# ComputationalRobotics/XM-code

Measured on AMD Instinct MI355X. Metric: BM iters/sec (tCG Hessian-vector iterations per second; ms_per_step = wall-clock-to-KKT of one staircase solve), higher is better.
Workload: dtype f64

## Files before the change

### include/xm_amd.h

```cpp
#ifndef XM_AMD_H
#define XM_AMD_H

#include <stddef.h>
#include <stdint.h>

#ifdef __cplusplus
extern "C" {
#endif

#define XM_OK              0
#define XM_ERR_IO         -1
#define XM_ERR_ARG        -2
#define XM_ERR_HIP        -3
#define XM_ERR_COMM       -4
#define XM_ERR_NOMEM      -5

#define XM_STATUS_NONE          0
#define XM_STATUS_CERTIFIED     1
#define XM_STATUS_MAX_RANK      2
#define XM_STATUS_LS_FAILED    -2

const char *xm_last_error(void);
const char *xm_version(void);
#define XM_ABI_REVISION 4
// ... 50 lines not shown
    uint32_t struct_size;
    int64_t n;
    int32_t storage;
    int32_t q_on_device;
    const double *q;
    int64_t ldq;
    int64_t nb;
    const int64_t *rowptr;
    const int32_t *colidx;
    const double *blocks;
    int64_t nobs, n_landmarks;
    const int32_t *obs_cam, *obs_lm;
    const double *obs_p, *obs_w;
    int64_t q_row0;
    int64_t ne;
    const int32_t *edge_i, *edge_j;
    const double *edge_w, *edge_M;
    int32_t n_gpus;
    int32_t gpu_map;
    const xm_tuning_t *tuning;
} xm_problem_t;

#define XM_MODE_SOLVE    0
#define XM_MODE_RANK3    1
#define XM_MODE_REBUTTLE 2

#define XM_FLAG_VERBOSE        1u
#define XM_FLAG_FIX_STALE_SR   2u
#define XM_FLAG_PROFILE_QW     4u
#define XM_FLAG_HOST_STEPPED   8u
#define XM_FLAG_MODEL_RECURRENCE 32u
#define XM_FLAG_HOST_OUTER    64u
#define XM_FLAG_DEVICE_OUTER 128u
#define XM_FLAG_WARM_R        16u

#define XM_RETRACT_QR    0
#define XM_RETRACT_POLAR 1

typedef struct {
    uint32_t struct_size;
    uint32_t max_rank;
    double tol, lam, max_time;
    int32_t mode;
    uint32_t flags;
    const double *s_ini;
    int32_t trace_cap;
    double *trace;
    const double *R_ini;
    int32_t retraction;
    int32_t sum_grouping;
} xm_options_t;

typedef struct {
    uint32_t struct_size;
    double *R;
    double *s;
    int32_t rank;
    int32_t status;
    double primal, dual, min_eig, gap;
    int64_t tcg_iters;
    int64_t outer_iters;
    int64_t qw_products;
    int64_t lanczos_iters;
    double seconds;
    double tr_seconds;
    double cert_seconds;
// ... 312 lines not shown
    int32_t irls_iterations;
    int32_t reserved;
    int64_t pcg_iterations;
    int64_t pcg_capped;
    int64_t pairs;
    int64_t registered;
    int64_t fixed_image;
    int64_t cams_heavy;
    int64_t max_incidences;
    double seconds_index;
    double seconds_kernels;
    double seconds_download;
} xm_vgr_result_t;
int xm_view_graph_rotations(int64_t n, const uint8_t *registered , const double *rot0, int64_t npairs, const int32_t *pi,
                            const int32_t *pj, const double *Rrel, const uint8_t *valid_in , const xm_vgr_options_t *opt,
                            double *rot_out, double *angle_axis_out, double *residual, double *weight, double *step_trace,
                            xm_vgr_result_t *res);
typedef struct {
    uint32_t struct_size;
    uint32_t reserved;
    const double *angle_axis, *x, *weight_in;
    double *rot, *residual, *gauge, *weight, *rhs, *diagonal, *product, *angle_axis_out, *step;
} xm_vgr_probe_t;
int xm_view_graph_rotations_probe(int64_t n, const uint8_t *registered, const double *rot0, int64_t npairs, const int32_t *pi,
                                  const int32_t *pj, const double *Rrel, const uint8_t *valid_in, const xm_vgr_options_t *opt,
                                  xm_vgr_probe_t *probe);
int xm_view_graph_rotations_limits(int64_t out[4]);
int xm_ctx_recover_tp(xm_ctx_t *ctx, const double *rot, const double *scale, double *t, double *p);
int xm_ctx_dense_q(xm_ctx_t *ctx, double *q, int64_t ldq);
int xm_create_matrix(int64_t n, int64_t m, int64_t nobs, const int32_t *cam, const int32_t *lm, const double *p, const double *w, double *Q,
                     int64_t ldq, double *Abar );
int xm_schur_dense_limits(int64_t out[3]);
int xm_ctx_schur_info(xm_ctx_t *ctx, int *uses_cg, int64_t stats[3], double *last_relres);
int xm_ctx_schur_precond_info(xm_ctx_t *ctx, int *kind, int64_t *aggregates, int *block);

#define XM_BA_FIX_ROTATIONS 1u
#define XM_BA_NONMONOTONIC  2u
#define XM_BA_DENSE_SCHUR   16u
#define XM_BA_PRECOND_TWO_LEVEL 32u
#define XM_BA_PRECOND_BLOCKS    64u
#define XM_BA_AGG_CAMS          16
#define XM_BA_MAX_AGGREGATES    4096
#define XM_BA_DENSE_MAX_ROWS 32768
#define XM_BA_LOSS_TRIVIAL  0
#define XM_BA_LOSS_HUBER    1
#define XM_BA_LOSS_SOFT_L1  2
#define XM_BA_LOSS_CAUCHY   3
#define XM_BA_LOSS_ARCTAN   4
#define XM_BA_OPTIONS_SIZE_V1 64u
#define XM_BA_NO_CONVERGENCE       0
#define XM_BA_CONVERGED_FUNCTION   1
#define XM_BA_CONVERGED_GRADIENT   2
#define XM_BA_CONVERGED_PARAMETER  3
#define XM_BA_MAX_ITERATIONS       4
#define XM_BA_TIME_LIMIT           5
#define XM_BA_NO_PROGRESS          6
typedef struct {
    uint32_t struct_size;
    int32_t max_iters;
    double max_time, eta, function_tol, gradient_tol, parameter_tol;
    uint32_t flags;
    int32_t trace_cap;
    double *trace;
    int32_t loss;
    int32_t max_nonmonotonic;
    double loss_scale;
// ... 312 lines not shown
```

### xm-code_amd/csrc/xm_capi.hip

```cpp
#include <algorithm>
#include <cmath>
#include <cstddef>
#include <cstdlib>
#include <cstring>
#include <fstream>
#include <mutex>
#include <vector>

#include "xm_ba.h"
#include "xm_gp.h"
#include "xm_clean.h"
#include "xm_trackfilter.h"
#include "xm_prune.h"
#include "xm_lift.h"
#include "xm_tracks.h"
#include "xm_tracks_split.h"
#include "xm_viewgraph.h"
#include "xm_vgcalib.h"
#include "xm_rotavg.h"
#include "xm_pair.h"
#include "xm_schur.h"
#include "xm_sell.h"
#include "xm_symw.h"
#include "xm_solver.h"
// ... 273 lines not shown
    XM_TRY
    if (!Q || ldq < 3 * n) throw xm::Error(XM_ERR_ARG, "xm_create_matrix: null Q or ldq < 3n");
    if (n > xm::kSchurDenseQMaxCams) throw xm::Error(XM_ERR_ARG, "xm_create_matrix: more than " + std::to_string(xm::kSchurDenseQMaxCams) + " cameras");
    require_device();
    hipStream_t st = nullptr;
    XM_HIP_CHECK(hipStreamCreateWithFlags(&st, hipStreamNonBlocking));
    double *dq = nullptr;
    try {
        xm::SchurSettings sc;
        sc.solver = 1;
        xm::SchurOp op(n, m, nobs, cam, lm, p, w, st, nullptr, sc);
        if (op.names_a_pair_twice()) throw xm::Error(XM_ERR_ARG, "xm_create_matrix: the observation list names a (camera, landmark) pair twice");
        const int64_t ld = xm_dense_ld(n);
        XM_HIP_CHECK(hipMalloc((void **)&dq, (size_t)3 * n * (size_t)ld * sizeof(double)));
        XM_HIP_CHECK(hipMemsetAsync(dq, 0, (size_t)3 * n * (size_t)ld * sizeof(double), st));
        op.build_dense_q(dq, ld, Abar, st);
        XM_HIP_CHECK(hipMemcpy2DAsync(Q, (size_t)ldq * sizeof(double), dq, (size_t)ld * sizeof(double), (size_t)3 * n * sizeof(double), (size_t)3 * n,
                                      hipMemcpyDeviceToHost, st));
        XM_HIP_CHECK(hipStreamSynchronize(st));
    } catch (...) {
        if (dq) (void)hipFree(dq);
        (void)hipStreamDestroy(st);
        throw;
    }
    (void)hipFree(dq);
    (void)hipStreamDestroy(st);
    return XM_OK;
    XM_CATCH
}
int xm_schur_dense_limits(int64_t out[3]) {
    XM_TRY
    if (!out) throw xm::Error(XM_ERR_ARG, "xm_schur_dense_limits: null output");
    out[0] = xm::kSchurDenseQWinCams; out[1] = xm::kSchurAbarPanel; out[2] = xm::kSchurDenseQMaxCams;
    return XM_OK;
    XM_CATCH
}
int xm_ctx_schur_info(xm_ctx_t *ctx, int *uses_cg, int64_t stats[3], double *last_relres) {
    XM_TRY
    if (!ctx || !ctx->impl || !uses_cg) throw xm::Error(XM_ERR_ARG, "xm_ctx_schur_info: single-GPU context and a non-null output needed");
    int64_t st[3] = {0, 0, 0};
    double rr = 0.0;
    *uses_cg = ctx->impl->schur_info(st, &rr) ? 1 : 0;
    if (stats) { stats[0] = st[0]; stats[1] = st[1]; stats[2] = st[2]; }
    if (last_relres) *last_relres = rr;
    return XM_OK;
    XM_CATCH
}
int xm_ctx_schur_precond_info(xm_ctx_t *ctx, int *kind, int64_t *aggregates, int *block) {
    XM_TRY
    if (!ctx || !ctx->impl || !kind) throw xm::Error(XM_ERR_ARG, "xm_ctx_schur_precond_info: single-GPU context and a non-null output needed");
    int64_t na = 0;
    int b = 0;
    *kind = ctx->impl->schur_precond(&na, &b);
    if (aggregates) *aggregates = na;
    if (block) *block = b;
    return XM_OK;
    XM_CATCH
}
int xm_ctx_bundle_adjust(xm_ctx_t *ctx, const xm_ba_options_t *opt, double *rot, double *t, double *p, xm_ba_result_t *res) {
    XM_TRY
    if (!ctx || !opt || !res || !rot || !t || !p) throw xm::Error(XM_ERR_ARG, "xm_ctx_bundle_adjust: null argument");
    static_assert(offsetof(xm_ba_options_t, loss) == XM_BA_OPTIONS_SIZE_V1, "the first version of xm_ba_options_t ends at trace");
    if (opt->struct_size != sizeof(xm_ba_options_t) && opt->struct_size != XM_BA_OPTIONS_SIZE_V1)
        throw xm::Error(XM_ERR_ARG, "xm_ctx_bundle_adjust: xm_ba_options_t.struct_size is neither sizeof(xm_ba_options_t) nor XM_BA_OPTIONS_SIZE_V1");
    if (res->struct_size != sizeof(xm_ba_result_t)) throw xm::Error(XM_ERR_ARG, "xm_ctx_bundle_adjust: xm_ba_result_t.struct_size is not sizeof(xm_ba_result_t)");
    if (ctx->team || !ctx->impl) throw xm::Error(XM_ERR_ARG, "xm_ctx_bundle_adjust: single-GPU contexts only (not n_gpus > 1)");
// ... 1611 lines not shown
```

### xm-code_amd/csrc/xm_common.h

```cpp
#pragma once

#include <hip/hip_runtime.h>

#include <algorithm>
#include <cstdint>
#include <cstdio>
#include <stdexcept>
#include <string>
#include <vector>

namespace xm {

struct Error : std::runtime_error {
    int code;
    Error(int c, const std::string &m) : std::runtime_error(m), code(c) {}
};

#define XM_HIP_CHECK(expr)                                                                            \
    do {                                                                                              \
        hipError_t _e = (expr);                                                                       \
        if (_e != hipSuccess)                                                                         \
            throw ::xm::Error(-3, std::string("HIP error: ") + hipGetErrorString(_e) + " at " +       \
                                      __FILE__ + ":" + std::to_string(__LINE__) + " (" #expr ")");    \
    } while (0)
// ... 147 lines not shown
    const OuterScal *os_cur;
    OuterScal *os_next;
    const double *parts;
    double *partsB_out;
    int nA, nB;
    const double *HpR, *Hps;
    double *R, *s;
    double *Rc, *sc;
    double *pR;
    const double *ps_cur;
    double *ps_next;
    double *vR, *vs, *HvR, *Hvs, *rR;
    const double *rs_cur;
    double *rs_next;
    double *Wloc, *Wpad;
    PointPtrs cur, cand;
    const double *partsA;
    double *partsM;
    int nM;
    double delta_bar, gradtol;
    int max_outer;
    double *trace;
    int trace_cap;
    const int *stop_req;
    unsigned long long *hprog;
    unsigned int run;
    int slot, grp;
};
void launch_outer_step(int o, int polar, const OuterStepArgs &A, int grid, hipStream_t st);

struct TcgParity {
    TcgScal *scal_cur, *scal_next;
    double *ps_cur, *ps_next, *rs_cur, *rs_next;
    size_t chunk, b_off;
    double *pcur;
    double *parts;
    double *Bout;
    double *partsB_out;
};

struct TcgInitArgs {
    int nloc;
    const double *rgR, *rgs, *R, *s;
    double *rR, *rs, *pR, *ps, *vR, *vs, *HvR, *Hvs;
    double *Wloc, *Wpad;
    TcgScal *scal0;
    double rr, delta;
    unsigned long long *hstat;
    int seq;
    const SpecCtl *spec;
};
struct CgStepArgs {
    int nloc;
    TcgParity v;
    int nA, nB, world;
    const double *HpR, *Hps, *R, *s;
    double *pR, *vR, *vs, *HvR, *Hvs, *rR;
    double *Wloc, *Wpad;
    unsigned long long *hstat;
    int64_t mat;
    double *Afull, *Wfull;
    int grouping;
    PeerXchg xchg;
};

void launch_qw_dense(int o, int epi, const double *Q, int64_t ld, const double *W, double alpha, const CamArgs &a,
                     hipStream_t st);
void launch_qw_bsr3(int o, int epi, const int64_t *rowptr, const int32_t *colidx, const double *blocks, const double *W,
                    double alpha, const CamArgs &a, hipStream_t st, int64_t nb = 0, const int4 *rowinfo = nullptr);
int64_t sell_resident_bytes(int64_t stream, int64_t other);
void bsr_build_rowinfo(const int64_t *rowptr_host, int nloc, std::vector<int4> &out);
int qw_grid(int nloc);
void launch_qw_dense_split(int o, int epi, const double *Q, int64_t ld, const double *W, double alpha, const CamArgs &a, hipStream_t st);
int qw_dense_tile_cols();
int qw_dense_split_k(int nloc, int64_t ld);
int bsr_grid(int nloc);
void qw_bench_nt(int nt);
void symv_bench_k(int k, int kf);
int symv_trace_slots();
struct SymvPlan { int K, Kf, ysplit, nchunks, gx, gy; };
void symv_plan_get(int nloc, int64_t ld, int out[4]);
struct SymvWork {
    int nloc = 0, o = 0;
    int64_t ld = 0;
    SymvPlan plan{};
    DevBuf<double> prow, pcol;
    void ensure(int nloc, int64_t ld, int o);
    void release();
    explicit operator bool() const { return pcol.p != nullptr; }
};
void launch_qw_sym_traced(int o, const double *Q, int64_t ld, const double *W, const CamArgs &a, SymvWork &work, unsigned long long *trace, hipStream_t st);
void launch_qw_sym(int o, int epi, const double *Q, int64_t ld, const double *W, double alpha, const CamArgs &a, SymvWork &work, hipStream_t st,
                   int rev = 0);
void launch_asym(const double *Q, int64_t ld, int64_t m, double *out, int grid, hipStream_t st);
void launch_dense_to_f32(const double *src, float *dst, int64_t rows, int64_t ld, unsigned int *bad, hipStream_t st);
void launch_qw_dense_f32(int o, int epi, const float *Qf, const double *Qd, int64_t ld, const double *W, double alpha, const CamArgs &a, hipStream_t st);
void launch_qw_sym_f32(int o, int epi, const float *Qf, const double *Qd, int64_t ld, const double *W, double alpha, const CamArgs &a, SymvWork &work,
                       hipStream_t st, int rev = 0);

void launch_symhash(const double *Q, int64_t ld, int64_t row0, int64_t nrows, int64_t m, unsigned long long *out, int grid, hipStream_t st);

void launch_transpose_pad(const double *src_colmajor, int64_t lds, int64_t rows, int64_t cols, double *dst, int64_t ldd,
                          hipStream_t st);
void launch_dense_from_bsr(const int64_t *rowptr, const int32_t *colidx, const double *blocks, int64_t nloc, int64_t cam0,
                           double *dst, int64_t ldd, hipStream_t st);

int flat_grid(int64_t elems);
void launch_scale_rows(int o, int nloc, const double *R, const double *s, double *Wloc, hipStream_t st);
void launch_tcg_init(int o, const TcgInitArgs &a, hipStream_t st);
void launch_cg_step(int o, const CgStepArgs &a, hipStream_t st);
struct OuterArgs { double loss, delta, delta_bar, gradtol; int shrink_count, last_iter; };
void launch_outer_finalize(const double *partsA, int nA_loc, int world, const double *partsM, int nM, const TcgScal *scal, double *hres,
                           unsigned long long seq, int grouping, hipStream_t st, const OuterArgs *oa = nullptr, SpecCtl *spec_out = nullptr);
void launch_retract(int o, int nloc, int cam0, const double *R, const double *s, const double *D, const double *ds, double t,
                    double *Rout, double *sout, double *Wloc, hipStream_t st, int polar = 0);
int retract_grid(int nloc);
void launch_retract_model(int o, int nloc, int cam0, const double *R, const double *s, const double *vR, const double *vs, double *Rout, double *sout,
                          double *Wloc, double *Wpad, const double *HvR, const double *Hvs, const double *rgR, const double *rgs, double *parts,
                          hipStream_t st, int polar);
void launch_cert_prepare(int o, int nloc, int cam0, double lam, const double *QsR, const double *R, const double *s,
                         double *Lam, double *dz, double *parts, hipStream_t st);
void launch_recover_gram(int64_t n, int r, const double *R, const double *s, double *parts, int grid, hipStream_t st);
void launch_recover_project(int64_t n, int r, const double *R, const double *s, const double *V, double *rot, double *scale, int *negcount,
                            hipStream_t st, int variant = 0);
void launch_negate(double *x, int64_t len, hipStream_t st);
int dots_multi_segments(int64_t len);
// ... 47 lines not shown
```

### xm-code_amd/csrc/xm_device.h

```cpp
#pragma once

#include "xm_common.h"

namespace xm {

template <int CTRL, int ROW_MASK>
__device__ __forceinline__ double dpp_mov(double v) {
    int lo = __double2loint(v), hi = __double2hiint(v);
    lo = __builtin_amdgcn_update_dpp(0, lo, CTRL, ROW_MASK, 0xf, false);
    hi = __builtin_amdgcn_update_dpp(0, hi, CTRL, ROW_MASK, 0xf, false);
    return __hiloint2double(hi, lo);
}
__device__ __forceinline__ double wave_sum(double v) {
    v += dpp_mov<0xb1, 0xf>(v);
    v += dpp_mov<0x4e, 0xf>(v);
    v += dpp_mov<0x124, 0xf>(v);
    v += dpp_mov<0x128, 0xf>(v);
    v += dpp_mov<0x142, 0xa>(v);
    v += dpp_mov<0x143, 0xc>(v);
    const int lo = __builtin_amdgcn_readlane(__double2loint(v), 63), hi = __builtin_amdgcn_readlane(__double2hiint(v), 63);
    return __hiloint2double(hi, lo);
}

template <int GW>
// ... 30 lines not shown
    __syncthreads();
    return (sh[0] + sh[1]) + (sh[2] + sh[3]);
}

__device__ __forceinline__ int sum_perm(int i, int count, int grp) {
    if (grp == 1) return count - 1 - i;
    if (grp == 2) { const int h = (count + 1) >> 1; return (i < h) ? 2 * i : 2 * (i - h) + 1; }
    return i;
}
__device__ __forceinline__ double sum_partials256(const double *p, int count, double *sh, int grp = 0) {
    double v = 0.0;
    for (int i = threadIdx.x; i < count; i += 256) v += p[sum_perm(i, count, grp)];
    return block_sum256(v, sh);
}

__device__ __forceinline__ void sum_partials256_x4(const double *p0, const double *p1, const double *p2, int count, const double *p3,
                                                   int count3, double *sh16, double (&out)[4], int grp = 0) {
    double v[4] = {0.0, 0.0, 0.0, 0.0};
    for (int i = threadIdx.x; i < count; i += 256) { const int j = sum_perm(i, count, grp); v[0] += p0[j]; v[1] += p1[j]; v[2] += p2[j]; }
    for (int i = threadIdx.x; i < count3; i += 256) v[3] += p3[sum_perm(i, count3, grp)];
#pragma unroll
    for (int k = 0; k < 4; ++k) v[k] = wave_sum(v[k]);
    __syncthreads();
    if ((threadIdx.x & 63) == 0) {
#pragma unroll
        for (int k = 0; k < 4; ++k) sh16[k * 4 + (threadIdx.x >> 6)] = v[k];
    }
    __syncthreads();
#pragma unroll
    for (int k = 0; k < 4; ++k) out[k] = (sh16[k * 4] + sh16[k * 4 + 1]) + (sh16[k * 4 + 2] + sh16[k * 4 + 3]);
}

constexpr int kPre = 4;
struct PartialsPre { double v[4][kPre]; };
__device__ __forceinline__ void sum_partials_prefetch(const double *p0, const double *p1, const double *p2, int count, const double *p3, int count3,
                                                      PartialsPre &pre, int grp) {
#pragma unroll
    for (int r = 0; r < kPre; ++r) {
        const int i = threadIdx.x + 256 * r;
        const int j = (i < count) ? sum_perm(i, count, grp) : 0, j3 = (i < count3) ? sum_perm(i, count3, grp) : 0;
        pre.v[0][r] = (i < count) ? p0[j] : 0.0; pre.v[1][r] = (i < count) ? p1[j] : 0.0; pre.v[2][r] = (i < count) ? p2[j] : 0.0;
        pre.v[3][r] = (i < count3) ? p3[j3] : 0.0;
    }
}
__device__ __forceinline__ void sum_partials256_x4_pre(const double *p0, const double *p1, const double *p2, int count, const double *p3,
                                                       int count3, bool use3, const PartialsPre &pre, double *sh16, double (&out)[4], int grp = 0) {
    double v[4] = {0.0, 0.0, 0.0, 0.0};
#pragma unroll
    for (int r = 0; r < kPre; ++r) {
        const int i = threadIdx.x + 256 * r;
        if (i < count) { v[0] += pre.v[0][r]; v[1] += pre.v[1][r]; v[2] += pre.v[2][r]; }
        if (use3 && i < count3) v[3] += pre.v[3][r];
    }
    for (int i = threadIdx.x + 256 * kPre; i < count; i += 256) { const int j = sum_perm(i, count, grp); v[0] += p0[j]; v[1] += p1[j]; v[2] += p2[j]; }
    if (use3)
        for (int i = threadIdx.x + 256 * kPre; i < count3; i += 256) v[3] += p3[sum_perm(i, count3, grp)];
#pragma unroll
    for (int k = 0; k < 4; ++k) v[k] = wave_sum(v[k]);
    __syncthreads();
    if ((threadIdx.x & 63) == 0) {
#pragma unroll
        for (int k = 0; k < 4; ++k) sh16[k * 4 + (threadIdx.x >> 6)] = v[k];
    }
    __syncthreads();
#pragma unroll
    for (int k = 0; k < 4; ++k) out[k] = (sh16[k * 4] + sh16[k * 4 + 1]) + (sh16[k * 4 + 2] + sh16[k * 4 + 3]);
}

#pragma clang fp contract(off)
struct Col3 {
    double v[3];
};
template <int O>
__device__ __forceinline__ Col3 load_col(const double *base, int cam, int lane) {
    constexpr int OP = pitch_of(O);
    Col3 c;
    const double *p = base + (size_t)cam * 3 * OP + lane;
#pragma unroll
    for (int a = 0; a < 3; ++a) c.v[a] = (lane < O) ? p[a * OP] : 0.0;
    return c;
}
template <int O>
__device__ __forceinline__ void store_col(const Col3 &c, double *base, int cam, int lane) {
    constexpr int OP = pitch_of(O);
    double *p = base + (size_t)cam * 3 * OP + lane;
    if (lane < O) {
#pragma unroll
        for (int a = 0; a < 3; ++a) p[a * OP] = c.v[a];
    }
// ... 198 lines not shown
```

### xm-code_amd/csrc/xm_kernels.hip

```cpp
#include <algorithm>
#include <cmath>
#include <cstdlib>
#include <cstring>
#include <type_traits>

#include "xm_common.h"
#include "xm_device.h"
#include "xm_symv_step.h"

namespace xm {

__device__ __forceinline__ double2 nt_load16(const double2 *p) {
    typedef double d2v __attribute__((ext_vector_type(2)));
    const d2v v = __builtin_nontemporal_load(reinterpret_cast<const d2v *>(p));
    return make_double2(v.x, v.y);
}

template <int O, int EPI, int NSUB, bool SPLIT = false>
__global__ __launch_bounds__(256) void qw_dense_kernel(const double *__restrict__ Q, int64_t ld,
                                                        const double *__restrict__ W, double alpha, CamArgs a) {
    constexpr int OP = pitch_of(O);
    int role = EPI;
    constexpr int TILE = NSUB * 128;
    constexpr int TILE2 = TILE * OP / 2;
// ... 229 lines not shown
            const double t = wave_sum(acc[r][k]);
            if (lane == k) h.v[r] = t;
        }
    if (active && lane < O) {
        double *ps = a.ksum + ((size_t)y * a.nloc + cam) * 3 * OP + lane;
#pragma unroll
        for (int r = 0; r < 3; ++r) __hip_atomic_store(ps + r * OP, h.v[r], __ATOMIC_RELAXED, __HIP_MEMORY_SCOPE_AGENT);
    }
    asm volatile("s_waitcnt vmcnt(0)" ::: "memory");
    __syncthreads();
    if (threadIdx.x == 0) {
        const unsigned int old = __hip_atomic_fetch_add(a.kcount + blockIdx.x, 1u, __ATOMIC_RELAXED, __HIP_MEMORY_SCOPE_AGENT);
        s_last = (old + 1 == (unsigned int)KS);
        if (s_last) __hip_atomic_store(a.kcount + blockIdx.x, 0u, __ATOMIC_RELAXED, __HIP_MEMORY_SCOPE_AGENT);
    }
    __syncthreads();
    if (!s_last) return;
    EpiOps eops;
    epi_prefetch<O, EPI>(eops, cam, lane, active, a);
    h.v[0] = h.v[1] = h.v[2] = 0.0;
    if (active && lane < O) {
        for (int s = 0; s < KS; ++s) {
            const double *ps = a.ksum + ((size_t)s * a.nloc + cam) * 3 * OP + lane;
#pragma unroll
            for (int r = 0; r < 3; ++r) h.v[r] += __hip_atomic_load(ps + r * OP, __ATOMIC_RELAXED, __HIP_MEMORY_SCOPE_AGENT);
        }
#pragma unroll
        for (int r = 0; r < 3; ++r) h.v[r] *= alpha;
    }
    qw_tail<O, EPI, 64, kQwWaves>(cam, lane, wave, active, h, a, eops, red);
}

constexpr int kSvTraceSlots = 24;
template <int O, bool TRACE = false>
__global__ __launch_bounds__(256) void qw_symv_kernel(const double *__restrict__ Q, int64_t ld, const double *__restrict__ W, int nloc, int Kc, int Kf, int ysplit, int nt_step0,
                                                        const TcgScal *__restrict__ scal, double *__restrict__ Prow,
                                                        double *__restrict__ Pcol, unsigned long long *__restrict__ trace, int rev, int by_phase) {
    constexpr int OP = pitch_of(O), V = 6 * O;
    __shared__ __attribute__((aligned(16))) double lds[4][V * 64];
    const int lane = threadIdx.x & 63, wave = __builtin_amdgcn_readfirstlane(threadIdx.x >> 6);
    unsigned long long *tr = nullptr;
    if constexpr (TRACE) {
        tr = trace + ((size_t)(blockIdx.y * gridDim.x + blockIdx.x) * 4 + wave) * kSvTraceSlots;
        if (lane == 0) {
            unsigned int hw, xcc;
            asm volatile("s_getreg_b32 %0, hwreg(HW_REG_HW_ID)" : "=s"(hw));
            asm volatile("s_getreg_b32 %0, hwreg(HW_REG_XCC_ID)" : "=s"(xcc));
            tr[0] = wall_clock64();
            tr[kSvTraceSlots - 1] = ((unsigned long long)xcc << 32) | hw;
        }
    }
    const SymvChunk ch = symv_chunk(blockIdx.x, blockIdx.y, nloc, ld, Kc, Kf, ysplit, wave);
    if (ch.empty) return;
    const int nrows = 3 * nloc, jb = ch.jb, je = ch.je;
    const bool half1 = ch.c0 + 128 < ld;
    double *L = lds[wave];
    const int64_t cA = ch.c0 + 2 * lane, cB = half1 ? cA + 128 : cA;

    double wc[2][2][O], ca[2][2][O];
    struct Slot { double2 q[6][2]; double wl; } slot[2];

    int nrun = 0;
    auto run = [&](int j, auto sl) __attribute__((always_inline)) {
        const Slot &b = slot[decltype(sl)::value];
        const int64_t r0 = (int64_t)6 * j;
        auto qat = [&](int r, int h, int e) __attribute__((always_inline)) { return e ? b.q[r][h].y : b.q[r][h].x; };
        auto wrow = [&](int r, double (&wr)[O]) __attribute__((always_inline)) { symv_wrow_read<O>(b.wl, r, r0 + r < nrows, wr); };
        double *prow = Prow + ((size_t)ch.s * (size_t)ch.R + (size_t)r0) * O;
        double mr[2] = {1.0, 1.0}, mc[2] = {1.0, 1.0};
        if (j < ch.jfull) symv_step<O, false>(qat, mr, mc, wrow, wc, ca, L, lane, prow);
        else {
#pragma unroll
            for (int h = 0; h < 2; ++h) {
                mr[h] = (cA + 128 * h >= r0) ? 1.0 : 0.0;
                mc[h] = (cA + 128 * h >= r0 + 6) ? 1.0 : 0.0;
            }
            symv_step<O, true>(qat, mr, mc, wrow, wc, ca, L, lane, prow);
        }
        if constexpr (TRACE) {
            if (lane == 0 && 2 + nrun < kSvTraceSlots - 3) tr[2 + nrun] = wall_clock64();
            ++nrun;
        }
    };
    auto sweep = [&](auto ntag) __attribute__((always_inline)) -> bool {
        constexpr bool NT = decltype(ntag)::value;
        auto load = [&](int j, auto sl) __attribute__((always_inline)) {
            Slot &b = slot[decltype(sl)::value];
            b.wl = symv_wrow_request<O>(W, j, nrows, lane);
            const int64_t r0 = (int64_t)6 * j;
#pragma unroll
            for (int r = 0; r < 6; ++r) {
                const int64_t rr = (r0 + r < nrows) ? r0 + r : nrows - 1;
                const double *row = Q + (size_t)rr * (size_t)ld;
#pragma unroll
                for (int h = 0; h < 2; ++h) {
                    const double2 *qp = reinterpret_cast<const double2 *>(row + (h ? cB : cA));
                    if (NT) b.q[r][h] = nt_load16(qp);
                    else b.q[r][h] = *qp;
                }
            }
        };
        if (jb < je) load(symv_walk_at(jb, je, rev, 0), std::integral_constant<int, 0>{});
#pragma unroll
        for (int h = 0; h < 2; ++h)
#pragma unroll
            for (int e = 0; e < 2; ++e)
#pragma unroll
                for (int k = 0; k < O; ++k) {
                    const double t = W[(size_t)((h ? cB : cA) + e) * OP + k];
                    wc[h][e][k] = (h == 0 || half1) ? t : 0.0;
                    ca[h][e][k] = 0.0;
                }
        if (scal != nullptr) {
            if (by_phase ? (scal->phase >= PH_STOP) : (scal->status != 0)) return false;
        }
        if constexpr (TRACE) { if (lane == 0) tr[1] = wall_clock64(); }
        symv_walk(jb, je, rev, load, run);
        return true;
    };
    const bool alive = (jb >= nt_step0) ? sweep(std::true_type{}) : sweep(std::false_type{});
    if (!alive) return;
    if constexpr (TRACE) { if (lane == 0) tr[kSvTraceSlots - 3] = wall_clock64(); }

    symv_colsum<O>(ca, lds, wave, lane, wave == 0 || half1, Pcol + ((size_t)ch.sc * (size_t)ld + (size_t)(cA + 128 * wave)) * O);
    if constexpr (TRACE) { if (lane == 0) tr[kSvTraceSlots - 2] = wall_clock64(); }
}

template <int O, int EPI>
__global__ __launch_bounds__(256) void symv_reduce_kernel(const double *__restrict__ Prow, const double *__restrict__ Pcol, int64_t ld,
                                                           int nstrips, int Kc, int Kf, int ysplit, double alpha, CamArgs a) {
    int role = (EPI == EPI_AUTO) ? (int)EPI_HESS : EPI;
    constexpr int NE = 3 * O;
    static_assert(NE <= 16, "a record must fit a 16-lane group");
    __shared__ double red[kQwWaves][3];
    const int lane = threadIdx.x & 63, wave = __builtin_amdgcn_readfirstlane(threadIdx.x >> 6);
    const int cam = blockIdx.x * kQwWaves + wave;
    const bool active = cam < a.nloc;
    EpiOps eops;
    epi_prefetch<O, EPI == EPI_AUTO ? EPI_HESS : EPI>(eops, cam, lane, active, a);
    const int e = lane & 15, g = lane >> 4;
    const bool eok = e < NE;
    const int camc = active ? cam : 0;
    const int64_t R = (int64_t)6 * ((a.nloc + 1) >> 1);
    const int s_lo = (6 * (camc >> 1)) / kSvStrip;
    const int nrow = nstrips - s_lo;
    auto ncol_of = [&](int c) -> int {
        const int sc_ = c / kSvStrip, row = min(sc_, nstrips - 1 - sc_);
        const int K = (row >= ysplit) ? Kf : Kc;
        return (c >= 6) ? (c - 6) / (6 * K) + 1 : 0;
    };
    const int ncol_l = ncol_of(3 * camc + (eok ? e / O : 0));
    const int ncol = max(ncol_of(3 * camc), ncol_of(3 * camc + 2));
    const int nrec = nrow + ncol;
    const int tot = active ? nrec : 0, tot_l = active ? nrow + ncol_l : 0;
    const size_t eo = (size_t)camc * 3 * O + (eok ? e : 0);
    auto fetch = [&](int i) -> double {
        const int ic = min(i, nrec - 1);
        const double *p = (ic < nrow) ? Prow + (size_t)(s_lo + ic) * (size_t)R * O : Pcol + (size_t)(ic - nrow) * (size_t)ld * O;
// ... 338 lines not shown
template <int O>
__global__ __launch_bounds__(256) void tcg_init_kernel(int nloc, const double *__restrict__ rgR, const double *__restrict__ rgs,
                                                        const double *__restrict__ R, const double *__restrict__ s,
                                                        double *rR, double *rs, double *pR, double *ps, double *vR, double *vs,
                                                        double *HvR, double *Hvs, double *Wloc, TcgScal *scal0, double rr,
                                                        double delta, unsigned long long *hstat, double *Wpad, int seq, const SpecCtl *spec) {
    constexpr int OP = pitch_of(O);
    const int64_t total = (int64_t)nloc * 3 * OP;
    if (spec != nullptr) {
        if (!spec->go) {
            if (blockIdx.x == 0 && threadIdx.x == 0) { TcgScal sc = *scal0; sc.status = 9; sc.seq = seq; *scal0 = sc; }
            return;
        }
        rr = spec->rr; delta = spec->delta;
    }
    for (int64_t i = (int64_t)blockIdx.x * 256 + threadIdx.x; i < total; i += (int64_t)gridDim.x * 256) {
        const int cam = (int)(i / (3 * OP));
        const double g = rgR[i], gs = rgs[cam];
        rR[i] = g; pR[i] = -g; vR[i] = 0.0; HvR[i] = 0.0;
        const double wv = s[cam] * (-g) + (-gs) * R[i];
        if (Wloc) Wloc[i] = wv;
        if (Wpad) Wpad[(size_t)cam * 16 + (i - (int64_t)cam * (3 * OP))] = wv;
        if (i % (3 * OP) == 0) { rs[cam] = gs; ps[cam] = -gs; vs[cam] = 0.0; Hvs[cam] = 0.0; }
    }
    if (blockIdx.x == 0 && threadIdx.x == 0) {
        TcgScal sc = {};
        sc.rr = rr; sc.vv = 0.0; sc.vp = 0.0; sc.pp = rr; sc.delta = delta; sc.gradnorm = sqrt(rr); sc.last_step = 0.0; sc.model = 0.0;
        sc.status = 0; sc.iter = 0; sc.seq = seq;
        *scal0 = sc;
        publish_host(hstat, pack_stat(seq, 0, 0));
    }
}

template <int O>
__global__ __launch_bounds__(256) void cg_step_kernel(int nloc, const TcgScal *__restrict__ scal_cur, TcgScal *scal_next,
                                                       const double *__restrict__ parts, int nA_loc, int nB_loc, int world,
                                                       const double *__restrict__ HpR,
                                                       const double *__restrict__ Hps, const double *__restrict__ R,
                                                       const double *__restrict__ s, double *pR, const double *__restrict__ ps_cur,
                                                       double *ps_next, double *vR, double *vs, double *HvR, double *Hvs, double *rR,
                                                       const double *__restrict__ rs_cur, double *rs_next, double *Wloc,
                                                       double *partsB_out, unsigned long long *hstat, int b_off, int64_t mat,
                                                       double *Afull, double *Wfull, int grp, PeerXchg x, double *Wpad) {
    constexpr int OP = pitch_of(O);
    __shared__ double sh[4];
    __shared__ double sh16[16];
    __shared__ int sh_flag;
    const int64_t total = (int64_t)nloc * 3 * OP;
    const int64_t stride = (int64_t)gridDim.x * 256;
    int64_t i = (int64_t)blockIdx.x * 256 + threadIdx.x;
    const bool in0 = i < total;
    const int camf = (int)(i / (3 * OP));
    const bool own0 = in0 && (i % (3 * OP) == 0);
    double hp = 0, pv = 0, vv0 = 0, hv = 0, rv = 0, Rv = 0, hs = 0, psv = 0, rsv = 0, sv = 1, vsv = 0, hvs = 0;
    const bool keep_hv = HvR != nullptr;
    if (in0) { hp = HpR[i]; pv = pR[i]; vv0 = vR[i]; if (keep_hv) hv = HvR[i]; rv = rR[i]; Rv = R[i]; hs = Hps[camf]; psv = ps_cur[camf]; rsv = rs_cur[camf]; sv = s[camf]; }
    if (own0) { vsv = vs[camf]; if (keep_hv) hvs = Hvs[camf]; }
    const bool can_pre = x.world <= 1;
    PartialsPre pre;
    if (can_pre) sum_partials_prefetch(parts + b_off, parts + b_off + nA_loc, parts + b_off + 2 * nA_loc, nA_loc, parts + b_off + 3 * nA_loc, nB_loc, pre, grp);
    const TcgScal sc0 = *scal_cur;
    const bool lead = (blockIdx.x == 0 && threadIdx.x == 0);
    if (sc0.status != 0) {
        if (lead) *scal_next = sc0;
        return;
    }
    if (x.world > 1) {
        const int par = sc0.iter & 1;
        const size_t chunk_d = (size_t)b_off + 3 * (size_t)nA_loc + nB_loc;
        const size_t off = ((size_t)par * x.world + x.rank) * chunk_d;
        const unsigned long long epoch = x.epoch_base + (unsigned long long)sc0.iter + 1ull;
        const double *src = x.buf[x.rank] + off;
        if (x.lite) {
            for (int p = 0; p < x.world; ++p) {
                if (p == x.rank) continue;
                double *dst = x.buf[p] + off;
                for (size_t j = (size_t)blockIdx.x * 256 + threadIdx.x; j < chunk_d; j += (size_t)stride)
                    __hip_atomic_store(dst + j, src[j], __ATOMIC_RELAXED, __HIP_MEMORY_SCOPE_SYSTEM);
            }
            asm volatile("s_waitcnt vmcnt(0)" ::: "memory");
            __syncthreads();
            if (threadIdx.x == 0) {
                const unsigned long long t = __hip_atomic_fetch_add(x.ticket + par, 1ull, __ATOMIC_RELAXED, __HIP_MEMORY_SCOPE_AGENT);
                sh_flag = (t + 1 == gridDim.x);
                if (sh_flag) __hip_atomic_store(x.ticket + par, 0ull, __ATOMIC_RELAXED, __HIP_MEMORY_SCOPE_AGENT);
            }
            __syncthreads();
            if (sh_flag && !x.mute && threadIdx.x < x.world && (int)threadIdx.x != x.rank)
                __hip_atomic_store(x.flag[threadIdx.x] + par * kMaxPeers + x.rank, epoch, __ATOMIC_RELAXED, __HIP_MEMORY_SCOPE_SYSTEM);
        } else {
            for (int p = 0; p < x.world; ++p) {
                if (p == x.rank) continue;
                double *dst = x.buf[p] + off;
                for (size_t j = (size_t)blockIdx.x * 256 + threadIdx.x; j < chunk_d; j += (size_t)stride) dst[j] = src[j];
            }
            __threadfence_system();
            asm volatile("s_waitcnt vmcnt(0)" ::: "memory");
            __syncthreads();
            if (threadIdx.x == 0) {
                const unsigned long long t = __hip_atomic_fetch_add(x.ticket + par, 1ull, __ATOMIC_ACQ_REL, __HIP_MEMORY_SCOPE_AGENT);
                sh_flag = (t + 1 == gridDim.x);
                if (sh_flag) __hip_atomic_store(x.ticket + par, 0ull, __ATOMIC_RELAXED, __HIP_MEMORY_SCOPE_AGENT);
            }
            __syncthreads();
            if (sh_flag && !x.mute && threadIdx.x < x.world && (int)threadIdx.x != x.rank) {
                __threadfence_system();
                asm volatile("s_waitcnt vmcnt(0)" ::: "memory");
                __hip_atomic_store(x.flag[threadIdx.x] + par * kMaxPeers + x.rank, epoch, __ATOMIC_RELEASE, __HIP_MEMORY_SCOPE_SYSTEM);
            }
        }
        __syncthreads();
        if (threadIdx.x == 0) {
            int good = 1;
            const long long t0 = wall_clock64();
            const unsigned long long *f = x.flag[x.rank] + par * kMaxPeers;
            for (int p = 0; p < x.world && good; ++p) {
                if (p == x.rank) continue;
                while (__hip_atomic_load(f + p, __ATOMIC_RELAXED, __HIP_MEMORY_SCOPE_SYSTEM) < epoch) {
                    if (wall_clock64() - t0 > x.spin_ticks) { good = 0; break; }
                    __builtin_amdgcn_s_sleep(1);
                }
            }
            if (!good) __hip_atomic_store(x.err, epoch | (1ull << 63), __ATOMIC_RELAXED, __HIP_MEMORY_SCOPE_SYSTEM);
            sh_flag = good;
            __atomic_thread_fence(__ATOMIC_ACQUIRE);
        }
        __syncthreads();
        if (!sh_flag) {
            if (lead) {
                TcgScal nx = sc0; nx.status = 7;
                *scal_next = nx;
                publish_host(hstat, pack_stat(nx.seq, nx.iter, nx.status));
            }
            return;
        }
        __builtin_amdgcn_fence(__ATOMIC_ACQUIRE, "");
    }
    const int chunk = b_off + 3 * nA_loc + nB_loc;
    double pHp = 0.0, rHp = 0.0, HpHp = 0.0, rr_prev = 0.0;
    for (int r = 0; r < world; ++r) {
        const double *pa = parts + (size_t)r * chunk + b_off;
        double t[4];
        if (r == 0 && can_pre) sum_partials256_x4_pre(pa, pa + nA_loc, pa + 2 * nA_loc, nA_loc, pa + 3 * nA_loc, nB_loc, sc0.iter > 0, pre, sh16, t, grp);
        else sum_partials256_x4(pa, pa + nA_loc, pa + 2 * nA_loc, nA_loc, pa + 3 * nA_loc, (sc0.iter > 0) ? nB_loc : 0, sh16, t, grp);
        pHp += t[0]; rHp += t[1]; HpHp += t[2];
        if (sc0.iter > 0) rr_prev += t[3];
    }
    TcgScal sc = sc0;
    if (sc0.iter > 0) sc.rr = rr_prev;
    const StepDecision d = tcg_decide(sc, pHp);
    if (d.mode == 5) {
        if (lead) {
            TcgScal nx = sc; nx.status = 5; nx.last_step = 0.0;
            *scal_next = nx;
            publish_host(hstat, pack_stat(nx.seq, nx.iter, nx.status));
        }
        return;
    }
    const double step = d.step;
    const bool cg = (d.mode == 0);
    double rr_est = sc.rr + 2.0 * step * rHp + step * step * HpHp;
    if (rr_est < 0.0) rr_est = 0.0;
    const bool conv = cg && (sqrt(rr_est) < sc.gradnorm * fmin(sc.gradnorm, 0.1));
    const double beta = rr_est / sc.rr;
    const bool newdir = cg && !conv;
    double acc = 0.0;
    if (in0) {
        vR[i] = vv0 + step * pv;
        if (keep_hv) HvR[i] = hv + step * hp;
        if (cg) {
            const double rn = rv + step * hp;
            const double rsn = rsv + step * hs;
            rR[i] = rn;
            acc += rn * rn;
            if (newdir) {
                const double pn = beta * pv - rn;
                const double psn = beta * psv - rsn;
                pR[i] = pn;
                if (!Afull) {
                    const double wv = sv * pn + psn * Rv;
                    if (Wloc) Wloc[i] = wv;
                    if (Wpad) Wpad[(size_t)camf * 16 + (i - (int64_t)camf * (3 * OP))] = wv;
                }
                if (own0) ps_next[camf] = psn;
            }
            if (own0) { rs_next[camf] = rsn; const double q = rsn / sv; acc += q * q; }
        }
        if (own0) { vs[camf] = vsv + step * psv; if (keep_hv) Hvs[camf] = hvs + step * hs; }
    }
    for (i += stride; i < total; i += stride) {
        const int cam = (int)(i / (3 * OP));
        const bool own = (i % (3 * OP) == 0);
        const double hpi = HpR[i], pi = pR[i], hsi = Hps[cam], psi = ps_cur[cam];
        vR[i] += step * pi;
        if (keep_hv) HvR[i] += step * hpi;
        if (cg) {
            const double rn = rR[i] + step * hpi;
            const double rsn = rs_cur[cam] + step * hsi;
            rR[i] = rn;
            acc += rn * rn;
            if (newdir) {
                const double pn = beta * pi - rn;
                const double psn = beta * psi - rsn;
                pR[i] = pn;
                if (!Afull) {
                    const double wv = s[cam] * pn + psn * R[i];
                    if (Wloc) Wloc[i] = wv;
                    if (Wpad) Wpad[(size_t)cam * 16 + (i - (int64_t)cam * (3 * OP))] = wv;
                }
                if (own) ps_next[cam] = psn;
            }
            if (own) { rs_next[cam] = rsn; const double q = rsn / s[cam]; acc += q * q; }
        }
        if (own) { vs[cam] += step * psi; if (keep_hv) Hvs[cam] += step * hsi; }
    }
    if (Afull && newdir) {
        const int64_t full = mat * world;
        const bool first = (sc0.iter == 0);
        for (int64_t j = (int64_t)blockIdx.x * 256 + threadIdx.x; j < full; j += stride) {
            const int64_t r = j / mat;
            const double b = parts[(size_t)r * chunk + (size_t)(j - r * mat)];
            const double w = Wfull[j];
            const double an = (first ? -w : Afull[j]) + step * b;
            Afull[j] = an;
            Wfull[j] = beta * w - an;
        }
    }
    if (cg) {
        const double tot = block_sum256(acc, sh);
        if (threadIdx.x == 0) partsB_out[blockIdx.x] = tot;
    }
    if (lead) {
        TcgScal nx = sc;
        nx.last_step = step;
        if (!keep_hv) nx.model = sc.model - step * sc.rr + 0.5 * step * step * pHp;
        if (!cg) {
            nx.status = d.mode;
        } else {
            nx.rr = rr_est;
            nx.vv = sc.vv + 2.0 * step * sc.vp + step * step * sc.pp;
            nx.vp = beta * (sc.vp + step * sc.pp);
            nx.pp = beta * beta * sc.pp + rr_est;
            if (conv) {
                nx.status = 3;
            } else {
                nx.iter = sc.iter + 1;
                nx.status = (nx.iter >= kMaxInner) ? 6 : 0;
            }
        }
        *scal_next = nx;
        publish_host(hstat, pack_stat(nx.seq, nx.iter, nx.status));
    }
}

__global__ __launch_bounds__(256) void outer_finalize_kernel(const double *__restrict__ partsA, int nA_loc, int world,
                                                              const double *__restrict__ partsM, int nM,
                                                              const TcgScal *__restrict__ scal, double *hres, unsigned long long seq, int grp,
                                                              OuterArgs oa, SpecCtl *spec_out) {
    __shared__ double sh[4];
    double f = 0.0, rr = 0.0;
    for (int r = 0; r < world; ++r) {
        f += sum_partials256(partsA + (size_t)r * 2 * nA_loc, nA_loc, sh, grp);
        rr += sum_partials256(partsA + (size_t)r * 2 * nA_loc + nA_loc, nA_loc, sh, grp);
    }
    const double m_vec = (nM > 0) ? sum_partials256(partsM, nM, sh, grp) : 0.0;
    if (threadIdx.x == 0) {
        const TcgScal sc = *scal;
        const double m = (nM > 0) ? m_vec : sc.model;
        __hip_atomic_store(hres + 0, f, __ATOMIC_RELAXED, __HIP_MEMORY_SCOPE_SYSTEM);
        __hip_atomic_store(hres + 1, rr, __ATOMIC_RELAXED, __HIP_MEMORY_SCOPE_SYSTEM);
        __hip_atomic_store(hres + 2, m, __ATOMIC_RELAXED, __HIP_MEMORY_SCOPE_SYSTEM);
        __hip_atomic_store(hres + 3, (double)sc.status, __ATOMIC_RELAXED, __HIP_MEMORY_SCOPE_SYSTEM);
        __hip_atomic_store(hres + 4, (double)sc.iter, __ATOMIC_RELAXED, __HIP_MEMORY_SCOPE_SYSTEM);
        if (spec_out != nullptr) {
            const int endreason = (sc.status == 0) ? 6 : sc.status;
            double delta = oa.delta;
            int shrink = oa.shrink_count;
            bool go = (m < 0.0) && endreason != 7;
            if (go) {
                const double rou = (f - oa.loss) / m;
                if (rou < 0.25) { delta *= 0.25; shrink++; }
                else if (rou > 0.75 && endreason <= 2) { delta = fmin(delta * 2, oa.delta_bar); shrink = 0; }
                else shrink = 0;
                bool stop_delta = false;
                if (shrink > 3) { delta *= 1e-3; shrink = 0; if (delta < 1e-20) stop_delta = true; }
// ... 1108 lines not shown
void symv_plan_get(int nloc, int64_t ld, int out[4]) {
    const SymvPlan p = symv_plan(nloc, ld);
    out[0] = p.K; out[1] = p.Kf; out[2] = p.ysplit; out[3] = p.nchunks;
}
void SymvWork::ensure(int nloc_new, int64_t ld_new, int o_new) {
    release();
    const SymvPlan p = symv_plan(nloc_new, ld_new);
    prow.alloc((size_t)((ld_new + kSvStrip - 1) / kSvStrip) * 6 * (size_t)((nloc_new + 1) / 2) * o_new);
    pcol.alloc((size_t)p.nchunks * (size_t)ld_new * o_new, false);
    nloc = nloc_new; ld = ld_new; o = o_new; plan = p;
}
void SymvWork::release() {
    prow.release(); pcol.release();
    nloc = 0; ld = 0; o = 0; plan = SymvPlan{};
}
struct SymvGeom { dim3 gs; int rK, rKf, ys, nstrips; };
static SymvGeom symv_geom(const SymvWork &w, int nloc, int64_t ld, int o) {
    if (!w || nloc != w.nloc || ld != w.ld || o > w.o) throw Error(-2, "symmetric product: the workspace was not made for this size and rank");
    return {dim3(w.plan.gx, w.plan.gy), 4 * w.plan.K, 4 * w.plan.Kf, w.plan.ysplit, (int)((ld + kSvStrip - 1) / kSvStrip)};
}

static int symv_nt_step0(int nloc, double elem_bytes) {
    const double m = 3.0 * nloc;
    const double tri = elem_bytes * m * (m + 6.0) / 2.0;
    const int64_t res = qw_resident_bytes((size_t)tri);
    const int nsteps = (nloc + 1) / 2;
    if ((double)res >= tri) return nsteps + 1;
    const double disc = m * m - 2.0 * (double)res / elem_bytes;
    const double r = m - std::sqrt(std::max(0.0, disc));
    return (int)std::min<double>(nsteps + 1, std::max(0.0, r / 6.0));
}
template <int O>
static void qw_symv_epi(int epi, const double *Q, int64_t ld, const double *W, double alpha, const CamArgs &a, SymvWork &work,
                        hipStream_t st, int rev, unsigned long long *trace = nullptr) {
    const auto [gs, rK, rKf, ys, nstrips] = symv_geom(work, a.nloc, ld, O);
    const SymvPlan &pl = work.plan;
    double *const Prow = work.prow.p, *const Pcol = work.pcol.p;
    const TcgScal *sc = (epi == EPI_HESS || epi == EPI_AUTO) ? a.scal : (const TcgScal *)nullptr;
    const int by_phase = (epi == EPI_AUTO) ? 1 : 0;
    const int nt0 = symv_nt_step0(a.nloc, sizeof(double));
    if (trace) {
        if constexpr (O == 3 || O == 4) hipLaunchKernelGGL((qw_symv_kernel<O, true>), gs, dim3(256), 0, st, Q, ld, W, a.nloc, pl.K, pl.Kf, ys, nt0, sc, Prow, Pcol, trace, rev, by_phase);
    } else hipLaunchKernelGGL((qw_symv_kernel<O>), gs, dim3(256), 0, st, Q, ld, W, a.nloc, pl.K, pl.Kf, ys, nt0, sc, Prow, Pcol, trace, rev, by_phase);
    const dim3 g(qw_grid(a.nloc)), b(256);
    switch (epi) {
        case EPI_PLAIN: hipLaunchKernelGGL((symv_reduce_kernel<O, EPI_PLAIN>), g, b, 0, st, Prow, Pcol, ld, nstrips, rK, rKf, ys, alpha, a); break;
        case EPI_GRAD: hipLaunchKernelGGL((symv_reduce_kernel<O, EPI_GRAD>), g, b, 0, st, Prow, Pcol, ld, nstrips, rK, rKf, ys, alpha, a); break;
        case EPI_HESS: hipLaunchKernelGGL((symv_reduce_kernel<O, EPI_HESS>), g, b, 0, st, Prow, Pcol, ld, nstrips, rK, rKf, ys, alpha, a); break;
        case EPI_AUTO:
            if constexpr (O >= 3) { hipLaunchKernelGGL((symv_reduce_kernel<O, EPI_AUTO>), g, b, 0, st, Prow, Pcol, ld, nstrips, rK, rKf, ys, alpha, a); break; }
            throw Error(-2, "bad epilogue");
        case EPI_CERT:
            if constexpr (O == 1) { hipLaunchKernelGGL((symv_reduce_kernel<1, EPI_CERT>), g, b, 0, st, Prow, Pcol, ld, nstrips, rK, rKf, ys, alpha, a); break; }
            throw Error(-2, "certificate operator needs o == 1");
        default: throw Error(-2, "bad epilogue");
    }
}
int symv_trace_slots() { return kSvTraceSlots; }
void launch_qw_sym_traced(int o, const double *Q, int64_t ld, const double *W, const CamArgs &a, SymvWork &work, unsigned long long *trace, hipStream_t st) {
    if (trace == nullptr) throw Error(-2, "traced symmetric product: no trace buffer");
    if (o == 3) qw_symv_epi<3>(EPI_PLAIN, Q, ld, W, 1.0, a, work, st, 0, trace);
    else if (o == 4) qw_symv_epi<4>(EPI_PLAIN, Q, ld, W, 1.0, a, work, st, 0, trace);
    else throw Error(-2, "traced symmetric product: o = 3 or 4");
    check_launch("qw_symv traced");
}

void launch_qw_sym(int o, int epi, const double *Q, int64_t ld, const double *W, double alpha, const CamArgs &a, SymvWork &work, hipStream_t st,
                   int rev) {
    if (a.nloc <= 0) return;
    switch (o) {
        case 1: qw_symv_epi<1>(epi, Q, ld, W, alpha, a, work, st, rev & 1); break;
        case 3: qw_symv_epi<3>(epi, Q, ld, W, alpha, a, work, st, rev & 1); break;
        case 4: qw_symv_epi<4>(epi, Q, ld, W, alpha, a, work, st, rev & 1); break;
        case 5: qw_symv_epi<5>(epi, Q, ld, W, alpha, a, work, st, rev & 1); break;
        default: throw Error(-2, "symmetric product is instantiated for o = 1, 3..5");
    }
    check_launch("qw_symv");
}
__global__ __launch_bounds__(256) void symhash_kernel(const double *__restrict__ Q, int64_t ld, int64_t row0, int64_t nrows, int64_t m,
                                                       unsigned long long *out) {
    __shared__ unsigned long long sh[2][4];
    unsigned long long acc = 0ull, bad = 0ull;
    const int64_t total = nrows * m;
    for (int64_t e = (int64_t)blockIdx.x * 256 + threadIdx.x; e < total; e += (int64_t)gridDim.x * 256) {
        const int64_t lr = e / m, c = e - lr * m, r = row0 + lr;
        if (r >= m || r == c) continue;
        const double v = Q[lr * ld + c];
        if (v != v) bad = 1ull;
        unsigned long long b = (v == 0.0) ? 0ull : (unsigned long long)__double_as_longlong(v);
        unsigned long long z = (unsigned long long)((r < c) ? r : c) * 0x9E3779B97F4A7C15ull + (unsigned long long)((r < c) ? c : r);
        z = (z ^ (z >> 30)) * 0xBF58476D1CE4E5B9ull; z = (z ^ (z >> 27)) * 0x94D049BB133111EBull; z ^= z >> 31;
        const unsigned long long t = (z | 1ull) * b;
        acc += (r < c) ? t : (0ull - t);
    }
    for (int off = 32; off > 0; off >>= 1) { acc += __shfl_xor(acc, off, 64); bad |= __shfl_xor(bad, off, 64); }
    if ((threadIdx.x & 63) == 0) { sh[0][threadIdx.x >> 6] = acc; sh[1][threadIdx.x >> 6] = bad; }
    __syncthreads();
    if (threadIdx.x == 0) {
        out[2 * blockIdx.x] = sh[0][0] + sh[0][1] + sh[0][2] + sh[0][3];
        out[2 * blockIdx.x + 1] = sh[1][0] | sh[1][1] | sh[1][2] | sh[1][3];
    }
}
void launch_symhash(const double *Q, int64_t ld, int64_t row0, int64_t nrows, int64_t m, unsigned long long *out, int grid, hipStream_t st) {
    hipLaunchKernelGGL(symhash_kernel, dim3(grid), dim3(256), 0, st, Q, ld, row0, nrows, m, out);
    check_launch("symhash");
}
void launch_asym(const double *Q, int64_t ld, int64_t m, double *out, int grid, hipStream_t st) {
// ... 55 lines not shown
            case 8: qw_bsr3_epi<8, 1>(epi, rp, ci, bl, W, ri, alpha, a, st); break;
            case 9: qw_bsr3_epi<9, 1>(epi, rp, ci, bl, W, ri, alpha, a, st); break;
            case 10: qw_bsr3_epi<10, 1>(epi, rp, ci, bl, W, ri, alpha, a, st); break;
            default: throw Error(-2, "rank o must be 1 or 3..10, got " + std::to_string(o));
        }
    }
    check_launch("qw_bsr3");
}

void launch_transpose_pad(const double *src, int64_t lds, int64_t rows, int64_t cols, double *dst, int64_t ldd, hipStream_t st) {
    const dim3 g((unsigned)((ldd + 31) / 32), (unsigned)((rows + 31) / 32));
    hipLaunchKernelGGL(transpose_pad_kernel, g, dim3(256), 0, st, src, lds, rows, cols, dst, ldd);
    check_launch("transpose_pad");
}
void launch_dense_from_bsr(const int64_t *rp, const int32_t *ci, const double *bl, int64_t nloc, int64_t cam0, double *dst,
                           int64_t ldd, hipStream_t st) {
    hipLaunchKernelGGL(dense_from_bsr_kernel, dim3((unsigned)nloc), dim3(252), 0, st, rp, ci, bl, nloc, cam0, dst, ldd);
    check_launch("dense_from_bsr");
}

void launch_scale_rows(int o, int nloc, const double *R, const double *s, double *Wloc, hipStream_t st) {
    XM_DISPATCH_O(o, hipLaunchKernelGGL((scale_rows_kernel<O_>), dim3(flat_grid((int64_t)nloc * 3 * pitch_of(O_))), dim3(256), 0, st,
                                        nloc, R, s, Wloc));
    check_launch("scale_rows");
}
void launch_tcg_init(int o, const TcgInitArgs &a, hipStream_t st) {
    XM_DISPATCH_O(o, hipLaunchKernelGGL((tcg_init_kernel<O_>), dim3(flat_grid((int64_t)a.nloc * 3 * pitch_of(O_))), dim3(256), 0, st,
                                        a.nloc, a.rgR, a.rgs, a.R, a.s, a.rR, a.rs, a.pR, a.ps, a.vR, a.vs, a.HvR, a.Hvs, a.Wloc, a.scal0, a.rr, a.delta,
                                        a.hstat, a.Wpad, a.seq, a.spec));
    check_launch("tcg_init");
}
void launch_cg_step(int o, const CgStepArgs &a, hipStream_t st) {
    XM_DISPATCH_O(o, hipLaunchKernelGGL((cg_step_kernel<O_>), dim3(a.nB), dim3(256), 0, st, a.nloc,
                                        a.v.scal_cur, a.v.scal_next, a.v.pcur, a.nA, a.nB, a.world, a.HpR, a.Hps, a.R, a.s, a.pR, a.v.ps_cur, a.v.ps_next, a.vR,
                                        a.vs, a.HvR, a.Hvs, a.rR, a.v.rs_cur, a.v.rs_next, a.Wloc, a.v.partsB_out, a.hstat, (int)a.v.b_off, a.mat, a.Afull,
                                        a.Wfull, a.grouping, a.xchg, a.Wpad));
    check_launch("cg_step");
}
void launch_outer_finalize(const double *partsA, int nA_loc, int world, const double *partsM, int nM, const TcgScal *scal, double *hres,
                           unsigned long long seq, int grouping, hipStream_t st, const OuterArgs *oa, SpecCtl *spec_out) {
    OuterArgs z;
    std::memset(&z, 0, sizeof(z));
    hipLaunchKernelGGL(outer_finalize_kernel, dim3(1), dim3(256), 0, st, partsA, nA_loc, world, partsM, nM, scal, hres, seq, grouping, oa ? *oa : z,
                       (oa != nullptr) ? spec_out : (SpecCtl *)nullptr);
    check_launch("outer_finalize");
}
void launch_outer_step(int o, int polar, const OuterStepArgs &A, int grid, hipStream_t st) {
    switch (o) {
#define XM_OS_CASE(OO) case OO: if (polar) hipLaunchKernelGGL((outer_step_kernel<OO, 1>), dim3(grid), dim3(256), 0, st, A); \
                                else hipLaunchKernelGGL((outer_step_kernel<OO, 0>), dim3(grid), dim3(256), 0, st, A); break;
        XM_OS_CASE(3) XM_OS_CASE(4) XM_OS_CASE(5) XM_OS_CASE(6) XM_OS_CASE(7) XM_OS_CASE(8) XM_OS_CASE(9) XM_OS_CASE(10)
#undef XM_OS_CASE
        default: throw Error(-2, "device-driven outer iteration: rank o must be 3..10, got " + std::to_string(o));
    }
    check_launch("outer_step");
}
int retract_grid(int nloc) { return (nloc + 255) / 256; }
void launch_retract_model(int o, int nloc, int cam0, const double *R, const double *s, const double *vR, const double *vs, double *Rout, double *sout,
                          double *Wloc, double *Wpad, const double *HvR, const double *Hvs, const double *rgR, const double *rgs, double *parts,
                          hipStream_t st, int polar) {
    const ModelArgs mv = {HvR, Hvs, rgR, rgs, parts};
    const dim3 g(retract_grid(nloc)), b(256);
    if (HvR == nullptr) {
        if (polar) { XM_DISPATCH_O(o, hipLaunchKernelGGL((retract_kernel<O_, 1, false>), g, b, 0, st, nloc, cam0, R, s, vR, vs, 1.0, Rout, sout, Wloc, Wpad, mv)); }
        else { XM_DISPATCH_O(o, hipLaunchKernelGGL((retract_kernel<O_, 0, false>), g, b, 0, st, nloc, cam0, R, s, vR, vs, 1.0, Rout, sout, Wloc, Wpad, mv)); }
        check_launch("retract");
        return;
    }
// ... 433 lines not shown
```

### xm-code_amd/csrc/xm_solver.h

```cpp
#pragma once

#include <chrono>
#include <cstdint>
#include <cstdio>
#include <memory>
#include <string>
#include <vector>

#include "../../include/xm_amd.h"
#include "xm_common.h"

namespace xm {

struct Settings {
    int sym = 0;
    int64_t sym_min_rows = 0;
    int64_t sym_rows(int world) const { return sym_min_rows > 0 ? sym_min_rows : (world <= 1 ? 4096 : 6144); }
    int sell = 0;
    int sell_slabs = 4, sell_lmax = 64, sell_gather = 1;
    int sell_codec = 0;
    int sell_wpad = 0;
    int overlap = 0;
    double overlap_min_mb = 64.0;
    int64_t cert_dense_rows = 384;
// ... 95 lines not shown
    int comm_kind() const { return comm_->active() ? comm_->kind() : 0; }
    int product_kind(int o) const;
    bool sell_wpad_on() const { return wpad_on_; }
    const std::string &fallback_note() const { return comm_->fallback_note; }
    int world() const { return comm_->world; }
    int64_t cameras() const { return n_; }
    int64_t edges() const { return ne_; }
    ~Context();
    void solve(const xm_options_t &opt, xm_result_t &res);
    void apply(int o, const double *W_host, double *out_host, double alpha);
    void attach_edges(int64_t ne, const int32_t *ei, const int32_t *ej, const double *M);
    void edge_residuals(double *res);
    void set_edge_weights(const double *w);
    void recover_tp(const double *rot, const double *scale, double *t, double *p);
    void bundle_adjust(const BaSettings &cfg, double *rot, double *t, double *p, BaOutcome &out);
    void ba_probe(const BaSettings &cfg, const double *rot, const double *t, const double *p, BaProbe &q);
    void global_positioning(const GpSettings &cfg, const double *rot, double *t, double *p, double *scales, GpOutcome &out);
    void gp_probe(const GpSettings &cfg, const double *rot, const double *t, const double *p, GpProbe &q);
    void outer_probe(xm_outer_probe_t &q);
    void rtr_probe(xm_rtr_probe_t &q);
    void schur_probe(xm_schur_probe_t &q);
    void cert_probe(xm_cert_probe_t &q);
    void reprojection_errors(const double *rot, const double *t, const double *p, double *sqerr);
    void filter_tracks(const TfSettings &cfg, const double *rot, const double *t, const double *p, uint8_t *keep, uint8_t *reason,
                       int32_t *lm_views, uint8_t *lm_status, TfOutcome &out);
    void prune_weakly_connected(const PruneSettings &cfg, int32_t *cluster_id, int32_t *obs_count, const PrunePairs *pairs, PruneOutcome &out);
    void clean_observations(const CleanSettings &cfg, uint8_t *keep, int32_t *cam_index, int32_t *lm_index, CleanOutcome &out);
    void edge_residuals_recovered(const double *rot, const double *scale, double *res);
    double xm2_filter(const double *rot, const double *scale, double pct, int64_t *removed, double *w_out);
    const std::vector<double> &weights() const { return w_cur_; }
    int64_t n_landmarks() const;
    int64_t n_observations() const;
    void dense_q(double *q, int64_t ldq);
    bool schur_info(int64_t out[3], double *relres) const;
    int schur_precond(int64_t *aggregates, int *block) const;

private:
    int64_t n_ = 0;
    int nloc_ = 0;
    int cam0_ = 0;
    int64_t g0_ = 0;
    int64_t true_loc_ = 0;
    int64_t ntot_ = 0;
    int64_t ld_ = 0;
    int storage_ = XM_STORAGE_DENSE;
    double *dQ_ = nullptr;
    bool ownQ_ = false;
    float *dQ32_ = nullptr;
    void refresh_q32();
    DevBuf<double> Afull_;
    DevBuf<int64_t> rowptr_;
    DevBuf<int32_t> colidx_;
    DevBuf<double> blocks_;
    int64_t nb_loc_ = 0;
    DevBuf<int4> rowinfo_;
    std::unique_ptr<SellMatrix> sell_;
    int sell_gm_ = 0;
    std::unique_ptr<SchurOp> schur_;
    bool schur_dense_ = false;
    int64_t ne_ = 0;
    DevBuf<int32_t> ei_, ej_, inc_edge_;
    DevBuf<int64_t> inc_ptr_, pos_ij_, pos_ji_, pos_d_;
    DevBuf<double> eM_, ew_, eres_;
    bool solved_ = false;
    std::vector<double> w_cur_;
    DevBuf<double> eerr_;
    const double *residuals_recovered_device(const double *rot, const double *scale);
    hipStream_t st_ = nullptr;
    hipStream_t st2_ = nullptr;
    hipEvent_t ev_w_ = nullptr, ev_p_ = nullptr;
    DevBuf<double> Pstrip_;
    bool w_pending_ = false;
    std::shared_ptr<Comm> comm_;
    Settings cfg_;
    PeerXchg xchg_;
    double *partsB_peer_ = nullptr;
    unsigned long long tcg_runs_ = 0;
    std::vector<int64_t> cam_cut_;
    int retraction_ = 0, grouping_ = 0;

    int o_ = 0, OP_ = 0;
    DevBuf<double> R_, s_, Rc_, sc_, W_, D_;
    DevBuf<double> wpad_;
    double *wpad() const { return (wpad_.p && wpad_on_) ? wpad_.p : nullptr; }
    bool wpad_on_ = false;
    const double *wpad_next_ = nullptr;
    PointState ps_[2];
    int cur_ = 0;
    DevBuf<double> rR_, rs_, rsB_, pR_, psA_, psB_, vR_, vs_, HvR_, Hvs_, HpR_, Hps_;
    DevBuf<double> partsA_, partsB_, partsM_;
    SymvWork symv_;
    DevBuf<double> ksum_;
    DevBuf<unsigned int> kcount_;
    int ks_ = 1;
    std::unique_ptr<SymwProduct> symw_;
    void product_symw(int epi, int o, double alpha, const CamArgs &a);
    bool sym_ok_ = false;
    int sym_max_o_ = 4;
    bool eig_exact_ = false;
    double q_asym_ = 0, q_max_ = 0;
    DevBuf<TcgScal> scal_;
    unsigned long long *hstat_ = nullptr;
    unsigned long long *hstat_dev_ = nullptr;
    double *hpin_ = nullptr;
    double *hpin_dev_ = nullptr;
    size_t hpin_count_ = 0;
    int nA_ = 0, nB_ = 0;
    unsigned long long outer_seq_ = 0;

    const xm_options_t *opt_ = nullptr;
    xm_result_t *res_ = nullptr;
    bool verbose_ = false;
    std::vector<std::pair<hipEvent_t, hipEvent_t>> ev_pool_;
    size_t ev_used_ = 0;
    int64_t hess_launches_ = 0;
    int sym_rev_ = 1;
    std::vector<float> qw_samples_;

    void init(const xm_problem_t &prob);
    void to_host(void *dst, const void *src_dev, size_t bytes);
    void to_dev(void *dst_dev, const void *src, size_t bytes);
    void ensure_pinned(size_t doubles);
    DevBuf<double> lzV_, lzc_, lzw_, lzc2_, lzab_, lzscr_;
    DevBuf<double> recW_;
    int64_t pos_of(int64_t g) const;
    void release_raw();
    void setup_rank(int o);
    void upload_point(const std::vector<double> &R_cm, int o, const std::vector<double> &s_ex);
    void download_point(std::vector<double> &R_cm, std::vector<double> &s_ex);
    CamArgs cam_args(int state) const;
    int prod_grid() const;
    int tcg_blocks() const;
    void product(int epi, int o, double alpha, const CamArgs &a);
    void gather_W();
    void flush_gather();
    bool overlap_applies() const;
    void eval_point(int state, const double *Rp, const double *sp, double &f, double &rr);
    double sum_parts(const double *dparts, int count);
    int run_tcg(double rr, double delta, int adopted = 0);
    int enqueue_spec_tcg();
    void tcg_enqueue_iteration(int i, bool profile);
    TcgParity tcg_parity(int par) const;
    void cand_role(CamArgs &a, const PointState &P, const double *R, const double *s) const;
    CamArgs tcg_cam_args(const TcgParity &v, bool cand) const;
    void tcg_product(int epi, const CamArgs &a, int par, bool profile);
    TcgInitArgs tcg_init_args(double rr, double delta, const SpecCtl *spec) const;
    CgStepArgs cg_step_args(int i) const;
    void probe_grad(bool aut, double &f, double &rr);
    bool spec_applies() const;
    DevBuf<SpecCtl> spec_;
    unsigned int tcg_seq_ = 0;
    volatile double *wait_outer_result();
    bool stream_idle(std::chrono::steady_clock::time_point t_wait, const char *what);
    bool agree_any(bool local);
    void drain_events();
    void finish_profile();
    TrResult trust_region(int o, double &gradtol, double linesearch_step, const std::vector<double> &v_dir, double max_time);
    bool device_outer_applies(int o) const;
    TrResult trust_region_device(int o, double &gradtol, double f, double rr, double delta, double delta_bar, double max_time);
    OuterStepArgs outer_step_args(int slot, bool model_rec, double delta_bar, double gradtol, unsigned int runid) const;
    void progress_line(int k, int inner, double loss, double gradnorm, int endreason, int trstatus) const;
    TrResult close_trust_region(int stop_reason, double &gradtol, long long totalite, int k, double loss, std::chrono::steady_clock::time_point start);
    DevBuf<double> trace_dev_;
    DevBuf<int> stop_req_;
    DevBuf<OuterScal> oscal_;
    unsigned int outer_run_ = 0;
    CertResult certificate(int o, double primal, std::vector<double> &v_out);
    int cert_multipliers(int o, double lam);
    int lanczos_min(std::vector<double> &x_out, double &theta, int &iters, double &resid);
    int lz_m_use_ = 0, lz_cycles_ = 0;
    bool lz_unfused_ = false;
    void cert_product(const double *vj, const CamArgs &a, int j);
    void log(const char *fmt, ...) const;
};
// ... 29 lines not shown
```

### xm-code_amd/csrc/xm_solver.hip

```cpp
#include "xm_solver.h"
#include "xm_sell.h"
#include "xm_symw.h"
#include "xm_schur.h"
#include "xm_ba.h"
#include "xm_gp.h"
#include "xm_clean.h"
#include "xm_trackfilter.h"
#include "xm_prune.h"

#include <algorithm>
#include <chrono>
#include <cmath>
#include <cstdarg>
#include <cstdlib>
#include <cstring>
#include <thread>

namespace xm {

using clk = std::chrono::steady_clock;
static double secs_since(clk::time_point t0) { return std::chrono::duration<double>(clk::now() - t0).count(); }

void Context::log(const char *fmt, ...) const {
    if (!verbose_ || (comm_ && comm_->rank != 0)) return;
// ... 380 lines not shown
            for (int b = 0; b < grid; ++b) { mine2[0] += hh[(size_t)2 * b]; mine2[1] |= hh[(size_t)2 * b + 1]; }
            static_assert(sizeof(unsigned long long) == sizeof(double), "checksums travel through the double all-gather");
            XM_HIP_CHECK(hipMemcpyAsync(repd.p + (size_t)rank * 2, mine2, sizeof(mine2), hipMemcpyHostToDevice, st_));
            comm_->allgather(repd.p, 2, st_);
            std::vector<unsigned long long> all((size_t)world * 2);
            XM_HIP_CHECK(hipMemcpyAsync(all.data(), repd.p, all.size() * sizeof(unsigned long long), hipMemcpyDeviceToHost, st_));
            XM_HIP_CHECK(hipStreamSynchronize(st_));
            unsigned long long tot = 0ull, bad2 = 0ull;
            for (int r = 0; r < world; ++r) { tot += all[(size_t)2 * r]; bad2 |= all[(size_t)2 * r + 1]; }
            if (tot != 0ull || bad2 != 0ull) symw_.reset();
        }
        comm_->host_barrier();
    }
    XM_HIP_CHECK(hipHostMalloc((void **)&hstat_, 256, hipHostMallocMapped | hipHostMallocCoherent));
    std::memset(hstat_, 0, 256);
    XM_HIP_CHECK(hipHostGetDevicePointer((void **)&hstat_dev_, hstat_, 0));
    ensure_pinned((size_t)1 << 17);
    if (viewgraph) {
        attach_edges(prob.ne, prob.edge_i, prob.edge_j, prob.edge_M);
        w_cur_.assign(prob.edge_w, prob.edge_w + prob.ne);
    }
}

Context::~Context() { release_raw(); }

void Context::setup_rank(int o) {
    if (comm_->active()) comm_->host_barrier();
    o_ = o;
    OP_ = pitch_of(o);
    const size_t mat = (size_t)nloc_ * 3 * OP_, vec = (size_t)nloc_;
    const int world = comm_->world;
    const int o_top = std::max(o, (int)std::min<unsigned>(opt_ ? opt_->max_rank : 0u, (unsigned)kMaxRank));
    const size_t mat_top = (size_t)nloc_ * 3 * pitch_of(o_top);
    for (DevBuf<double> *b : {&R_, &Rc_, &D_, &rR_, &pR_, &vR_, &HvR_, &HpR_}) b->ensure(mat, st_, mat_top);
    for (DevBuf<double> *b : {&s_, &sc_, &rs_, &rsB_, &psA_, &psB_, &vs_, &Hvs_, &Hps_}) b->ensure(vec, st_);
    for (int k = 0; k < 2; ++k) {
        ps_[k].G.ensure(mat, st_, mat_top); ps_[k].rgR.ensure(mat, st_, mat_top); ps_[k].egs.ensure(vec, st_); ps_[k].rgs.ensure(vec, st_); ps_[k].S0.ensure(vec * 9, st_);
    }
    cur_ = 0;
    wpad_on_ = sell_ && cfg_.sell_wpad >= 0 && !comm_->active() && sell_supports(o) && o >= 3 && 3 * OP_ <= 16 && (cfg_.sell_wpad == 1 || sell_->padded_pays(o));
    if (wpad_on_ && !wpad_.p) wpad_.alloc((size_t)ntot_ * 16 + 16);
    W_.ensure((size_t)ld_ * OP_ + 16, st_, (size_t)ld_ * pitch_of(o_top) + 16);
    const int nA_loc = prod_grid(), nB_loc = tcg_blocks();
    nA_ = nA_loc * world;
    nB_ = nB_loc * world;
    partsA_.ensure((size_t)3 * nA_, st_);
    const size_t b_off = comm_->active() ? mat : 0;
    const size_t pb = (size_t)2 * (b_off * world + 3 * nA_ + nB_);
    if (comm_->peer() && world > 1 && cfg_.exchange != 1 && !symw_ && storage_ != XM_STORAGE_SCHUR && comm_->device_waits()) {
        partsB_.release();
        comm_->xchg_setup(pb, xchg_);
        partsB_peer_ = xchg_.buf[comm_->rank];
        xchg_.mute = (cfg_.debug_peer_mute && comm_->rank == 1) ? 1 : 0;
        xchg_.lite = cfg_.exchange_lite;
    } else {
        xchg_ = PeerXchg();
        partsB_peer_ = nullptr;
        partsB_.ensure(pb, st_, (size_t)2 * ((comm_->active() ? mat_top : 0) * world + 3 * nA_ + nB_));
    }
    if (comm_->active()) Afull_.ensure(mat * world, st_, mat_top * world); else Afull_.release();
    partsM_.ensure((size_t)std::max(std::max(nB_, flat_grid((int64_t)mat_top) * world), 4 * ((nloc_ + 255) / 256) * world), st_);
    if (!(sym_ok_ && o >= 3 && o <= sym_max_o_)) symv_.release();
    else if (!symv_ || symv_.nloc != nloc_ || symv_.ld != ld_ || symv_.o != o) symv_.ensure(nloc_, ld_, o);
    ks_ = 1;
    if (storage_ == XM_STORAGE_DENSE && !sym_ok_ && cfg_.split_k >= 0) {
        if (cfg_.split_k >= 2) ks_ = std::min(cfg_.split_k, std::max(1, (int)((ld_ + 255) / 256)));
        else if (comm_->active()) ks_ = qw_dense_split_k(nloc_, ld_);
// ... 80 lines not shown
    a.partials = partsA_.p;
    a.scal = scal_.p;
    if (ks_ > 1) { a.ks = ks_; a.ksum = ksum_.p; a.kcount = kcount_.p; }
    return a;
}

void Context::product(int epi, int o, double alpha, const CamArgs &a) {
    if (w_pending_) {
        if (storage_ == XM_STORAGE_DENSE && (epi == EPI_PLAIN || epi == EPI_GRAD) && o == o_) {
            w_pending_ = false;
            const int tc = qw_dense_tile_cols();
            const int64_t c0 = 3 * (int64_t)cam0_, c1 = 3 * ((int64_t)cam0_ + nloc_);
            CamArgs s1 = a, s2 = a;
            s1.range_mode = 1; s1.t_lo = (int)((c0 + tc - 1) / tc); s1.t_hi = (int)(c1 / tc); s1.out = Pstrip_.p; s1.addend = nullptr;
            s2.range_mode = 2; s2.t_lo = s1.t_lo; s2.t_hi = s1.t_hi; s2.addend = Pstrip_.p;
            comm_->note("overlap_split", (double)s1.t_lo, (double)s1.t_hi);
            XM_HIP_CHECK(hipEventRecord(ev_w_, st_));
            XM_HIP_CHECK(hipStreamWaitEvent(st2_, ev_w_, 0));
            launch_qw_dense_split(o, EPI_PLAIN, dQ_, ld_, W_.p, 1.0, s1, st2_);
            XM_HIP_CHECK(hipEventRecord(ev_p_, st2_));
            comm_->allgather(W_.p, (size_t)nloc_ * 3 * OP_, st_);
            XM_HIP_CHECK(hipStreamWaitEvent(st_, ev_p_, 0));
            launch_qw_dense_split(o, epi, dQ_, ld_, W_.p, alpha, s2, st_);
            if (res_) res_->qw_products++;
            return;
        }
        flush_gather();
    }
    if (storage_ == XM_STORAGE_DENSE && dQ32_ && o == o_ && (epi == EPI_HESS || epi == EPI_AUTO)) {
        if (sym_ok_ && o >= 3 && o <= sym_max_o_ && symv_) launch_qw_sym_f32(o, epi, dQ32_, dQ_, ld_, W_.p, alpha, a, symv_, st_, sym_rev_);
        else { CamArgs ar = a; ar.rev = sym_rev_; launch_qw_dense_f32(o, epi, dQ32_, dQ_, ld_, W_.p, alpha, ar, st_); }
    } else if (storage_ == XM_STORAGE_DENSE) {
        if (symw_ && o == o_ && o >= 3 && o <= sym_max_o_ && epi != EPI_CERT) product_symw(epi, o, alpha, a);
        else if (sym_ok_ && o == o_ && o >= 3 && o <= sym_max_o_ && epi != EPI_CERT && symv_) launch_qw_sym(o, epi, dQ_, ld_, W_.p, alpha, a, symv_, st_, sym_rev_);
        else { CamArgs ar = a; ar.rev = sym_rev_; launch_qw_dense(o, epi, dQ_, ld_, W_.p, alpha, ar, st_); }
    } else if (storage_ == XM_STORAGE_SCHUR) {
        schur_->product(o, epi, W_.p, alpha, a, st_);
    } else if (sell_ && sell_supports(o)) {
        const double *wp = (epi == EPI_HESS && o == o_) ? wpad() : ((epi == EPI_GRAD && o == o_) ? wpad_next_ : nullptr);
        wpad_next_ = nullptr;
        launch_qw_sell(o, epi, *sell_, W_.p, alpha, a, sell_gm_, st_, wp);
    } else {
        launch_qw_bsr3(o, epi, rowptr_.p, colidx_.p, blocks_.p, W_.p, alpha, a, st_, nb_loc_, rowinfo_.p);
    }
    if (res_) res_->qw_products++;
}

int Context::product_kind(int o) const {
    if (storage_ == XM_STORAGE_SCHUR) return XM_PRODUCT_SCHUR;
    if (storage_ == XM_STORAGE_DENSE) return ((symw_ || sym_ok_) && o >= 3 && o <= sym_max_o_) ? XM_PRODUCT_DENSE_SYM : XM_PRODUCT_DENSE;
    if (sell_ && sell_supports(o)) return sell_->codec() == SELL_CODEC_QUAT ? XM_PRODUCT_SELL_QUAT : XM_PRODUCT_SELL;
    return XM_PRODUCT_BSR3;
}

void Context::product_symw(int epi, int o, double alpha, const CamArgs &a) {
    symw_->sweep(o, dQ_, W_.p, (epi == EPI_HESS) ? a.scal : (const TcgScal *)nullptr, comm_->rank, st_);
    comm_->allgather(symw_->csum_all(), symw_->csum_count(o), st_);
    symw_->reduce(o, epi, alpha, a, comm_->world, st_);
}

bool Context::overlap_applies() const {
    if (cfg_.overlap < 0 || !comm_->active() || storage_ != XM_STORAGE_DENSE || sym_ok_ || symw_) return false;
    if ((double)nloc_ * 3.0 * (double)ld_ * 8.0 < cfg_.overlap_min_mb * 1048576.0) return false;
    const int tc = qw_dense_tile_cols();
    const int64_t c0 = 3 * (int64_t)cam0_, c1 = 3 * ((int64_t)cam0_ + nloc_);
    return (c1 / tc) > ((c0 + tc - 1) / tc);
}
// ... 70 lines not shown
    while (*hseq != seq) {
        __builtin_ia32_pause();
        if (secs_since(t_check) > 500e-6) {
            if (stream_idle(t_wait, "the outer-iteration results")) {
                XM_HIP_CHECK(hipStreamSynchronize(st_));
                if (*hseq != seq) throw Error(XM_ERR_HIP, "outer-iteration results did not reach host-mapped memory");
            }
            t_check = clk::now();
        }
    }
    return reinterpret_cast<volatile double *>(hstat_) + 8;
}

void Context::drain_events() {
    for (size_t i = 0; i < ev_used_; ++i) {
        float ms = 0.f;
        if (hipEventElapsedTime(&ms, ev_pool_[i].first, ev_pool_[i].second) == hipSuccess) qw_samples_.push_back(ms);
    }
    ev_used_ = 0;
}

void Context::finish_profile() {
    drain_events();
    if (qw_samples_.empty()) return;
    std::vector<float> v = qw_samples_;
    std::sort(v.begin(), v.end());
    const float ref = v[(v.size() * 3) / 4];
    for (float x : v)
        if (x >= 0.5f * ref) { res_->qw_ms_sum += x; res_->qw_ms_count++; }
    qw_samples_.clear();
}

void Context::tcg_enqueue_iteration(int i, bool profile) {
    const CgStepArgs S = cg_step_args(i);
    tcg_product(EPI_HESS, tcg_cam_args(S.v, false), i & 1, profile);
    if (comm_->active() && xchg_.world <= 1) comm_->allgather(S.v.pcur, S.v.chunk, st_);
    launch_cg_step(o_, S, st_);
}

TcgParity Context::tcg_parity(int par) const {
    const size_t nA = (size_t)prod_grid(), world = (size_t)comm_->world, rank = (size_t)comm_->rank;
    TcgParity v;
    v.scal_cur = scal_.p + par; v.scal_next = scal_.p + (par ^ 1);
    v.ps_cur = par ? psB_.p : psA_.p; v.ps_next = par ? psA_.p : psB_.p;
    v.rs_cur = par ? rsB_.p : rs_.p; v.rs_next = par ? rs_.p : rsB_.p;
    v.b_off = comm_->active() ? (size_t)nloc_ * 3 * OP_ : 0;
    v.chunk = v.b_off + 3 * nA + (size_t)tcg_blocks();
    double *pB = xchg_.world > 1 ? partsB_peer_ : partsB_.p;
    v.pcur = pB + (size_t)par * v.chunk * world;
    v.parts = v.pcur + rank * v.chunk + v.b_off;
    v.Bout = comm_->active() ? v.pcur + rank * v.chunk : nullptr;
    v.partsB_out = pB + (size_t)(par ^ 1) * v.chunk * world + rank * v.chunk + v.b_off + 3 * nA;
    return v;
}

void Context::cand_role(CamArgs &a, const PointState &P, const double *R, const double *s) const {
    a.cand = {R, s, P.G.p, P.egs.p, P.S0.p, P.rgR.p, P.rgs.p, partsA_.p};
}

CamArgs Context::tcg_cam_args(const TcgParity &v, bool cand) const {
    CamArgs a = cam_args(cur_);
    a.scal = v.scal_cur; a.ps = v.ps_cur; a.rs = v.rs_cur;
    a.partials = v.parts; a.Bout = v.Bout;
    if (cand) cand_role(a, ps_[cur_ ^ 1], Rc_.p, sc_.p);
    return a;
}

void Context::tcg_product(int epi, const CamArgs &a, int par, bool profile) {
    const bool timed = profile && (hess_launches_ % kProfileStride == 0) && ev_used_ < ev_pool_.size();
    if (timed) XM_HIP_CHECK(hipEventRecord(ev_pool_[ev_used_].first, st_));
    sym_rev_ = par;
    product(epi, o_, 2.0, a);
    sym_rev_ = 1;
    if (timed) { XM_HIP_CHECK(hipEventRecord(ev_pool_[ev_used_].second, st_)); ev_used_++; }
    hess_launches_++;
}

TcgInitArgs Context::tcg_init_args(double rr, double delta, const SpecCtl *spec) const {
    const PointState &P = ps_[cur_];
    TcgInitArgs a;
    a.nloc = nloc_;
    a.rgR = P.rgR.p; a.rgs = P.rgs.p; a.R = R_.p; a.s = s_.p;
    a.rR = rR_.p; a.rs = rs_.p; a.pR = pR_.p; a.ps = psA_.p; a.vR = vR_.p; a.vs = vs_.p; a.HvR = HvR_.p; a.Hvs = Hvs_.p;
    a.Wloc = wpad() ? nullptr : W_.p + (size_t)cam0_ * 3 * OP_; a.Wpad = wpad();
    a.scal0 = scal_.p; a.rr = rr; a.delta = delta;
    a.hstat = hstat_dev_; a.seq = (int)tcg_seq_; a.spec = spec;
    return a;
}

CgStepArgs Context::cg_step_args(int i) const {
    const bool model_rec = opt_ && (opt_->flags & XM_FLAG_MODEL_RECURRENCE);
    CgStepArgs a;
    a.nloc = nloc_; a.v = tcg_parity(i & 1);
    a.nA = prod_grid(); a.nB = tcg_blocks(); a.world = comm_->world;
    a.HpR = HpR_.p; a.Hps = Hps_.p; a.R = R_.p; a.s = s_.p;
    a.pR = pR_.p; a.vR = vR_.p; a.vs = vs_.p; a.HvR = model_rec ? nullptr : HvR_.p; a.Hvs = model_rec ? nullptr : Hvs_.p; a.rR = rR_.p;
    a.Wloc = wpad() ? nullptr : W_.p + (size_t)cam0_ * 3 * OP_; a.Wpad = wpad();
    a.hstat = hstat_dev_; a.mat = (int64_t)nloc_ * 3 * OP_;
    a.Afull = comm_->active() ? Afull_.p : nullptr; a.Wfull = W_.p;
    a.grouping = grouping_; a.xchg = xchg_;
    return a;
}

bool Context::spec_applies() const {
    return !comm_->active() && opt_ && !(opt_->flags & XM_FLAG_HOST_STEPPED) && storage_ != XM_STORAGE_SCHUR && cfg_.debug_drop_finalize < 0;
}

int Context::enqueue_spec_tcg() {
    std::swap(R_.p, Rc_.p);
    std::swap(s_.p, sc_.p);
    cur_ ^= 1;
    ++tcg_seq_;
    launch_tcg_init(o_, tcg_init_args(0.0, 0.0, spec_.p), st_);
    const int n_spec = 1;
    for (int i = 0; i < n_spec; ++i) tcg_enqueue_iteration(i, false);
    std::swap(R_.p, Rc_.p);
    std::swap(s_.p, sc_.p);
    cur_ ^= 1;
    return n_spec;
}

int Context::run_tcg(double rr, double delta, int adopted) {
    const bool stepped = (opt_->flags & XM_FLAG_HOST_STEPPED) != 0;
    const bool profile = (opt_->flags & XM_FLAG_PROFILE_QW) != 0;
    if (comm_->active()) comm_->note("tcg_start", rr, delta);
    if (adopted == 0) {
        ++tcg_seq_;
        launch_tcg_init(o_, tcg_init_args(rr, delta, nullptr), st_);
        gather_W();
    }
    const bool fused = xchg_.world > 1;
    if (fused) xchg_.epoch_base = (++tcg_runs_) << 12;
    const bool lockstep = comm_->active() && !fused;
    const int run_ahead = (lockstep || prod_grid() >= 64) ? 2 : 3;
    int fin_status = 0, fin_iter = 0;
    int it = adopted;
    auto enqueue = [&](int i) { tcg_enqueue_iteration(i, profile); };
    auto read_scal = [&](int par) {
        TcgScal sc;
        to_host(&sc, scal_.p + par, sizeof(TcgScal));
        return sc;
    };
    if (stepped) {
        for (;;) {
            TcgScal sc = read_scal(it & 1);
            if (sc.status != 0 || it >= kMaxInner) break;
            enqueue(it++);
        }
    } else {
        volatile unsigned long long *hs = hstat_;
        auto last_progress = clk::now();
        auto last_change = last_progress;
        unsigned long long seen = ~0ull;
        for (;;) {
            const unsigned long long v = *hs;
            if (v != seen) { seen = v; last_progress = clk::now(); last_change = last_progress; }
            const bool valid = (unsigned int)(v >> 32) == tcg_seq_;
            const int status = valid ? (int)(v & 0xff) : 0;
            const int done = valid ? (int)((v >> 8) & 0xffffff) : 0;
            if (status != 0) { fin_status = status; fin_iter = done; break; }
            if (it < kMaxInner && it - done < run_ahead) { enqueue(it++); continue; }
            __builtin_ia32_pause();
            if (secs_since(last_progress) > 200e-6) {
                if (stream_idle(last_change, "the truncated-CG progress word")) {
                    TcgScal sc = read_scal(it & 1);
                    if (sc.status != 0) { fin_status = sc.status; fin_iter = sc.iter; break; }
                    if (it >= kMaxInner) { fin_status = 6; fin_iter = kMaxInner; break; }
                    *hstat_ = ((unsigned long long)tcg_seq_ << 32) | ((unsigned long long)(unsigned)sc.iter << 8);
                    if (it - sc.iter >= run_ahead) enqueue(it++);
                }
                last_progress = clk::now();
            }
        }
    }
    if (comm_->active()) comm_->note("tcg_end_before_topup", (double)it, (double)(fin_iter * 16 + fin_status));
    if (fin_status == 7) { comm_->check_device_error(); throw Error(XM_ERR_COMM, "peer exchange: a rank did not arrive inside the truncated CG"); }
    if (lockstep && !stepped) {
        const int T = (fin_status == 6) ? fin_iter - 1 : fin_iter;
        while (it < std::min(kMaxInner, T + 2)) enqueue(it++);
    }
    return it;
}

TrResult Context::trust_region(int o, double &gradtol, double linesearch_step, const std::vector<double> &v_dir, double max_time) {
    TrResult out;
    const double dim = (double)n_ * (3.0 * o - 6.0) + (double)n_ - 1.0;
    const double delta_bar = std::sqrt(dim);
    double delta = delta_bar / 8.0;
    double *Wloc = W_.p + (size_t)cam0_ * 3 * OP_;
    double f = 0, rr = 0;

    log("start linesearch\n");
    if (linesearch_step != 0) {
        launch_scale_rows(o, nloc_, R_.p, s_.p, Wloc, st_);
        gather_W();
        double f0, tmp;
        eval_point(cur_ ^ 1, R_.p, s_.p, f0, tmp);
        double alpha = linesearch_step;
        std::vector<double> D((size_t)nloc_ * 3 * OP_, 0.0);
        for (int c = 0; c < (int)true_loc_; ++c) {
            const int64_t g = g0_ + c;
            for (int a = 0; a < 3; ++a) D[((size_t)c * 3 + a) * OP_ + (o - 1)] = v_dir[(size_t)(3 * g + a)];
        }
        to_dev(D_.p, D.data(), D.size() * sizeof(double));
        double fn;
        for (;;) {
            launch_retract(o, nloc_, cam0_, R_.p, s_.p, D_.p, nullptr, -alpha, Rc_.p, nullptr, Wloc, st_, retraction_);
            gather_W();
            eval_point(cur_ ^ 1, Rc_.p, s_.p, fn, tmp);
            if (!(fn > f0)) break;
            alpha *= 0.5;
            if (alpha < 1e-20) { log("linesearch failed! BM stopped! \n"); out.primal = -1; out.ls_failed = true; out.stop_reason = -1; return out; }
        }
        if (f0 - fn > 0) {
            log("linesearch decrease %1.3e\n", f0 - fn);
            if (opt_->flags & XM_FLAG_FIX_STALE_SR) {
                std::swap(R_.p, Rc_.p);
                launch_scale_rows(o, nloc_, R_.p, s_.p, Wloc, st_);
            } else {
                launch_scale_rows(o, nloc_, R_.p, s_.p, Wloc, st_);
                std::swap(R_.p, Rc_.p);
            }
            gather_W();
        } else {
            log("linesearch failed! BM stopped! \n");
            out.primal = -1; out.ls_failed = true; out.stop_reason = -1;
            return out;
        }
    } else {
        launch_scale_rows(o, nloc_, R_.p, s_.p, Wloc, st_);
        gather_W();
    }
    eval_point(cur_, R_.p, s_.p, f, rr);
    if (device_outer_applies(o)) return trust_region_device(o, gradtol, f, rr, delta, delta_bar, max_time);
    double loss = f;

    int endreason = 6, trstatus = 4, shrink_count = 0, inner_print = 1, k = 0;
    int adopted = 0;
    long long totalite = 0;
    int stop_reason = 14;
    const auto start = clk::now();
    for (k = 0; k < kMaxOuter; ++k) {
        const double gradnorm = std::sqrt(rr);
        progress_line(k, inner_print, loss, gradnorm, endreason, trstatus);
        if (opt_->trace && res_->trace_len < opt_->trace_cap) {
            double *tr = opt_->trace + (size_t)res_->trace_len * 6;
            tr[0] = loss; tr[1] = gradnorm; tr[2] = inner_print; tr[3] = endreason; tr[4] = trstatus; tr[5] = delta;
            res_->trace_len++;
        }
        if (endreason == 5) { stop_reason = 5; break; }
        if (gradnorm < gradtol) { stop_reason = 10; break; }
        if (agree_any((double)(long long)secs_since(start) > max_time)) { stop_reason = 11; break; }
        endreason = 6; trstatus = 4;

        TcgScal fin;
        const int enq = run_tcg(rr, delta, adopted);
        adopted = 0;

        const int nA_loc = prod_grid();
        const PointState &P = ps_[cur_];
        const int nB_loc = retract_grid(nloc_);
        const bool model_rec = (opt_->flags & XM_FLAG_MODEL_RECURRENCE) != 0;
        launch_retract_model(o, nloc_, cam0_, R_.p, s_.p, vR_.p, vs_.p, Rc_.p, sc_.p, Wloc, wpad(), model_rec ? nullptr : HvR_.p, Hvs_.p, P.rgR.p, P.rgs.p,
                             partsM_.p + (size_t)comm_->rank * nB_loc, st_, retraction_ == XM_RETRACT_POLAR ? 1 : 0);
        if (comm_->active() && !model_rec) comm_->allgather(partsM_.p, (size_t)nB_loc, st_);
        gather_W();
        wpad_next_ = wpad();
// ... 624 lines not shown
    double *hres_dev = reinterpret_cast<double *>(hstat_dev_) + 8;
    double *Wloc = W_.p + (size_t)cam0_ * 3 * OP_;
    double *Wtcg = wpad() ? nullptr : Wloc;
    const PointState &P = ps_[cur_];

    upload_point(std::vector<double>(q.R, q.R + m3 * (size_t)o), o, std::vector<double>(q.s, q.s + n));
    double f = 0, rr = 0;
    probe_grad(aut, f, rr);
    q.f = f; q.rr = rr;
    down_mat(q.G, P.G.p); down_vec(q.egs, P.egs.p); down_vec(q.S0, P.S0.p, 9); down_mat(q.rgR, P.rgR.p); down_vec(q.rgs, P.rgs.p);

    if (want_init) {
        TcgInitArgs I = tcg_init_args(rr, q.scal_in.delta, nullptr);
        I.hstat = nullptr; I.seq = 0;
        launch_tcg_init(o, I, st_);
        down_mat(q.init_rR, rR_.p); down_vec(q.init_rs, rs_.p); down_mat(q.init_pR, pR_.p); down_vec(q.init_ps, psA_.p);
        down_mat(q.init_vR, vR_.p); down_vec(q.init_vs, vs_.p); down_mat(q.init_HvR, HvR_.p); down_vec(q.init_Hvs, Hvs_.p);
        if (Wtcg) down_mat(q.init_W, Wloc);
        if (wpad()) down_vec(q.init_Wpad, wpad(), 16);
        TcgScal sc;
        to_host(&sc, scal_.p, sizeof(sc));
        scal_out(sc, q.init_scal);
    }

    if (want_hess) {
        const int iter = want_step ? q.scal_in.iter : 0, par = iter & 1;
        const TcgParity v = tcg_parity(par);
        up_mat(D_.p, q.pR, -1.0);
        up_vec(sc_.p, q.ps, -1.0, true);
        TcgInitArgs I = tcg_init_args(0.0, 0.0, nullptr);
        I.rgR = D_.p; I.rgs = sc_.p;
        I.hstat = nullptr; I.seq = 0;
        launch_tcg_init(o, I, st_);
        up_mat(pR_.p, q.pR, 1.0); up_vec(v.ps_cur, q.ps, 1.0, false);
        up_mat(rR_.p, q.rR, 1.0); up_vec(v.rs_cur, q.rs, 1.0, false);
        TcgScal sc;
        std::memset(&sc, 0, sizeof(sc));
        if (want_step) {
            sc.rr = q.scal_in.rr; sc.vv = q.scal_in.vv; sc.vp = q.scal_in.vp; sc.pp = q.scal_in.pp; sc.delta = q.scal_in.delta; sc.gradnorm = q.scal_in.gradnorm;
            sc.model = q.scal_in.model; sc.iter = q.scal_in.iter;
        }
        sc.phase = PH_TCG;
        to_dev(v.scal_cur, &sc, sizeof(sc));
        tcg_product(aut ? EPI_AUTO : EPI_HESS, tcg_cam_args(v, aut), par, false);
        launch_outer_finalize(v.parts, nA, 1, v.parts + (size_t)2 * nA, nA, v.scal_cur, hres_dev, ++outer_seq_, 0, st_);
        volatile double *hres = wait_outer_result();
        q.pHp = hres[0]; q.rHp = hres[1]; q.HpHp = hres[2];
        down_mat(q.HpR, HpR_.p); down_vec(q.Hps, Hps_.p);

        if (want_step) {
            up_mat(vR_.p, q.vR, 1.0); up_vec(vs_.p, q.vs, 1.0, false);
            if (!model_rec) { up_mat(HvR_.p, q.HvR, 1.0); up_vec(Hvs_.p, q.Hvs, 1.0, false); }
            up_vec(v.ps_next, q.ps, 1.0, false); up_vec(v.rs_next, q.rs, 1.0, false);
            if (q.scal_in.iter > 0) to_dev(v.parts + (size_t)3 * nA, q.partsB_in, (size_t)nB * sizeof(double));
            XM_HIP_CHECK(hipMemsetAsync(v.partsB_out, 0, (size_t)nB * sizeof(double), st_));
            CgStepArgs S = cg_step_args(iter);
            S.hstat = nullptr;
            S.xchg = PeerXchg();
            S.grouping = 0;
            launch_cg_step(o_, S, st_);
            launch_outer_finalize(partsA_.p, 0, 1, v.partsB_out, nB, v.scal_next, hres_dev, ++outer_seq_, 0, st_);
            hres = wait_outer_result();
            q.rr_parts = hres[2];
            TcgScal nx;
            to_host(&nx, v.scal_next, sizeof(nx));
            scal_out(nx, q.scal_out);
            down_mat(q.out_vR, vR_.p); down_vec(q.out_vs, vs_.p);
            if (!model_rec) { down_mat(q.out_HvR, HvR_.p); down_vec(q.out_Hvs, Hvs_.p); }
            down_mat(q.out_rR, rR_.p); down_vec(q.out_rs, v.rs_next); down_mat(q.out_pR, pR_.p); down_vec(q.out_ps, v.ps_next);
            if (Wtcg) down_mat(q.out_W, Wloc);
            if (wpad()) down_vec(q.out_Wpad, wpad(), 16);
            if (q.partsB_out) to_host(q.partsB_out, v.partsB_out, (size_t)nB * sizeof(double));
        }
    }

    if (want_cert) {
        launch_scale_rows(o, nloc_, R_.p, s_.p, Wloc, st_);
        CamArgs a = cam_args(cur_);
        a.out = HpR_.p;
        product(EPI_PLAIN, o, 1.0, a);
        const int g = (nloc_ + 255) / 256;
        double *Lam = ps_[cur_ ^ 1].S0.p, *dz = ps_[cur_ ^ 1].egs.p;
        launch_cert_prepare(o, nloc_, cam0_, q.lam, HpR_.p, R_.p, s_.p, Lam, dz, partsM_.p, st_);
        std::vector<double> parts((size_t)2 * g);
        to_host(parts.data(), partsM_.p, parts.size() * sizeof(double));
        q.dual[0] = q.dual[1] = 0.0;
        for (int i = 0; i < g; ++i) { q.dual[0] += parts[(size_t)i]; q.dual[1] += parts[(size_t)g + i]; }
        down_vec(q.Lam, Lam, 9); down_vec(q.dz, dz);
        if (q.X && q.SX && q.k > 0) {
            CamArgs c = cam_args(cur_);
            c.Lam = Lam; c.dz = dz;
            std::vector<double> x((size_t)ld_), y(m3);
            for (int j = 0; j < q.k; ++j) {
                std::fill(x.begin(), x.end(), 0.0);
                std::copy(q.X + (size_t)j * m3, q.X + (size_t)(j + 1) * m3, x.begin());
                to_dev(W_.p, x.data(), x.size() * sizeof(double));
                c.Wloc = W_.p + (size_t)cam0_ * 3;
                c.out = HpR_.p;
                cert_product(W_.p, c, j);
                to_host(y.data(), HpR_.p, m3 * sizeof(double));
                std::copy(y.begin(), y.end(), q.SX + (size_t)j * m3);
            }
// ... 135 lines not shown
        if (q.ret_partsM) to_host(q.ret_partsM, partsM_.p, (size_t)nM * sizeof(double));
        q.ret_pad[0] = count_pad(Rc_.p); q.ret_pad[1] = count_pad(Wloc); q.ret_pad[2] = count_wpad();
    }

    if (want_ls) {
        up_mat(D_.p, q.D, 1.0);
        poison_mat(Rc_.p); poison_mat(Wloc);
        launch_retract(o, nloc_, cam0_, R_.p, s_.p, D_.p, nullptr, q.t, Rc_.p, nullptr, Wloc, st_, polar);
        down_mat(q.ls_Rc, Rc_.p); down_mat(q.ls_W, Wloc);
        q.ls_pad[0] = count_pad(Rc_.p); q.ls_pad[1] = count_pad(Wloc);
    }

    if (want_step) {
        const int par = q.slot & 1;
        const TcgParity v = tcg_parity(par);
        if (trace_dev_.count < (size_t)kMaxOuter * 6) trace_dev_.alloc((size_t)kMaxOuter * 6);
        if (stop_req_.count < 1) stop_req_.alloc(1);
        if (oscal_.count < 2) oscal_.alloc(2);
        const int stop_word = q.stop_req;
        to_dev(stop_req_.p, &stop_word, sizeof(int));
        const unsigned int runid = ++outer_run_;
        q.run = runid;
        volatile unsigned long long *hp = hstat_ + 24;
        *hp = 0;
        if (phase == PH_TCG) {
            up_mat(D_.p, q.pR, -1.0);
            up_vec(Hps_.p, q.ps, -1.0, true);
            TcgInitArgs I = tcg_init_args(0.0, 0.0, nullptr);
            I.rgR = D_.p; I.rgs = Hps_.p;
            I.hstat = nullptr; I.seq = 0;
            I.Wloc = Wloc; I.Wpad = nullptr;
            launch_tcg_init(o, I, st_);
        }
        up_mat(pR_.p, q.pR, 1.0); up_vec(v.ps_cur, q.ps, 1.0, false); up_vec(v.ps_next, q.ps, 1.0, false);
        up_mat(rR_.p, q.rR, 1.0); up_vec(v.rs_cur, q.rs, 1.0, false); up_vec(v.rs_next, q.rs, 1.0, false);
        up_mat(vR_.p, q.vR, 1.0); up_vec(vs_.p, q.vs, 1.0, false);
        up_mat(HvR_.p, q.HvR, 1.0); up_vec(Hvs_.p, q.Hvs, 1.0, false);
        if (q.Rc && q.sc) { up_mat(Rc_.p, q.Rc, 1.0); up_vec(sc_.p, q.sc, 1.0, false); }
        else {
            XM_HIP_CHECK(hipMemcpyAsync(Rc_.p, R_.p, mat * sizeof(double), hipMemcpyDeviceToDevice, st_));
            XM_HIP_CHECK(hipMemcpyAsync(sc_.p, s_.p, (size_t)nloc_ * sizeof(double), hipMemcpyDeviceToDevice, st_));
        }
        for (DevBuf<double> *b : {&ps_[cur_ ^ 1].G, &ps_[cur_ ^ 1].egs, &ps_[cur_ ^ 1].S0, &ps_[cur_ ^ 1].rgR, &ps_[cur_ ^ 1].rgs})
            XM_HIP_CHECK(hipMemsetAsync(b->p, 0, b->count * sizeof(double), st_));
        TcgScal sc = tcg_in(q.scal_in), sc_zero;
        std::memset(&sc_zero, 0, sizeof(sc_zero));
        to_dev(v.scal_cur, &sc, sizeof(sc));
        to_dev(v.scal_next, &sc_zero, sizeof(sc_zero));
        OuterScal os, os_zero;
        std::memset(&os, 0, sizeof(os));
        std::memset(&os_zero, 0, sizeof(os_zero));
        os.loss = q.os_in.loss; os.rr_point = q.os_in.rr_point; os.totalite = q.os_in.totalite; os.shrink_count = q.os_in.shrink_count; os.k = q.os_in.k;
        os.stop_reason = q.os_in.stop_reason; os.time_up = q.os_in.time_up; os.slots = q.os_in.slots;
        to_dev(oscal_.p + par, &os, sizeof(os));
        to_dev(oscal_.p + (par ^ 1), &os_zero, sizeof(os_zero));
        XM_HIP_CHECK(hipMemsetAsync(partsB_.p, 0, 2 * v.chunk * sizeof(double), st_));
        XM_HIP_CHECK(hipMemsetAsync(partsM_.p, 0, (size_t)std::max(nwave, nM) * sizeof(double), st_));
        if (q.partsM_in && q.partsM_in_count == nwave) to_dev(partsM_.p, q.partsM_in, (size_t)nwave * sizeof(double));
        const int krec = q.os_in.k + 1;
        const bool rec_ok = krec >= 1 && krec < kMaxOuter;
        if (rec_ok) XM_HIP_CHECK(hipMemsetAsync(trace_dev_.p + (size_t)krec * 6, 0xff, 6 * sizeof(double), st_));
        const CamArgs a = tcg_cam_args(v, true);
        if (phase == PH_TCG) {
            tcg_product(EPI_AUTO, a, par, false);
            launch_outer_finalize(v.parts, nA, 1, v.parts + (size_t)2 * nA, nA, v.scal_cur, hres_dev, ++outer_seq_, 0, st_);
            volatile double *hres = wait_outer_result();
            q.pHp = hres[0]; q.rHp = hres[1]; q.HpHp = hres[2];
            down_mat(q.HpR, HpR_.p); down_vec(q.Hps, Hps_.p);
// ... 2 lines not shown
        } else if (phase == PH_CAND) {
            launch_scale_rows(o, nloc_, Rc_.p, sc_.p, Wloc, st_);
            tcg_product(EPI_AUTO, a, par, false);
            std::vector<double> grouped((size_t)nM, 0.0);
            if (!model_rec)
                for (int i = 0; i < nM; ++i) {
                    auto w = [&](int j) { return j < nwave ? q.partsM_in[j] : 0.0; };
                    grouped[(size_t)i] = (w(4 * i) + w(4 * i + 1)) + (w(4 * i + 2) + w(4 * i + 3));
                }
            to_dev(D_.p, grouped.data(), grouped.size() * sizeof(double));
            launch_outer_finalize(partsA_.p, nA, 1, D_.p, model_rec ? 0 : nM, v.scal_cur, hres_dev, ++outer_seq_, grouping_, st_);
            volatile double *hres = wait_outer_result();
            q.f_cand = hres[0]; q.rr_cand = hres[1]; q.m_cand = hres[2];
            down_mat(q.cand_G, Pn.G.p); down_vec(q.cand_egs, Pn.egs.p); down_vec(q.cand_S0, Pn.S0.p, 9); down_mat(q.cand_rgR, Pn.rgR.p); down_vec(q.cand_rgs, Pn.rgs.p);
        }
        OuterStepArgs A = outer_step_args(q.slot, model_rec, q.delta_bar, q.gradtol, runid);
        if (q.max_outer > 0) A.max_outer = q.max_outer;
        launch_outer_step(o_, polar, A, nB, st_);
        XM_HIP_CHECK(hipStreamSynchronize(st_));
        q.progress = *hp;
        TcgScal nx;
        OuterScal on;
        to_host(&nx, v.scal_next, sizeof(nx));
        to_host(&on, oscal_.p + (par ^ 1), sizeof(on));
        tcg_out(nx, q.scal_out);
        q.os_out.loss = on.loss; q.os_out.rr_point = on.rr_point; q.os_out.totalite = on.totalite; q.os_out.shrink_count = on.shrink_count; q.os_out.k = on.k;
        q.os_out.stop_reason = on.stop_reason; q.os_out.time_up = on.time_up; q.os_out.slots = on.slots; q.os_out.pad = 0;
        if (rec_ok) {
            to_host(q.trace, trace_dev_.p + (size_t)krec * 6, 6 * sizeof(double));
            q.trace_written = std::isnan(q.trace[0]) ? 0 : 1;
        }
        down_mat(q.out_R, R_.p); down_vec(q.out_s, s_.p); down_mat(q.out_Rc, Rc_.p); down_vec(q.out_sc, sc_.p);
        down_mat(q.out_vR, vR_.p); down_vec(q.out_vs, vs_.p); down_mat(q.out_HvR, HvR_.p); down_vec(q.out_Hvs, Hvs_.p);
        down_mat(q.out_rR, rR_.p); down_vec(q.out_rs, v.rs_next); down_mat(q.out_pR, pR_.p); down_vec(q.out_ps, v.ps_next);
        down_mat(q.out_W, Wloc);
        if (wpad()) down_vec(q.out_Wpad, wpad(), 16);
        if (q.out_partsB) to_host(q.out_partsB, v.partsB_out, (size_t)nB * sizeof(double));
        if (q.out_partsM) to_host(q.out_partsM, partsM_.p, (size_t)nwave * sizeof(double));
        down_mat(q.out_G, P.G.p); down_vec(q.out_egs, P.egs.p); down_vec(q.out_S0, P.S0.p, 9); down_mat(q.out_rgR, P.rgR.p); down_vec(q.out_rgs, P.rgs.p);
        if (phase == PH_TCG) { q.out_pad[0] = count_pad(Rc_.p); q.out_pad[1] = count_pad(Wloc); }
    }
    XM_HIP_CHECK(hipStreamSynchronize(st_));
}

void Context::attach_edges(int64_t ne, const int32_t *ei, const int32_t *ej, const double *M) {
    if (ne < 0 || (ne > 0 && (!ei || !ej || !M))) throw Error(XM_ERR_ARG, "attach_edges: bad argument");
    validate_edges(n_, ne, ei, ej, "attach_edges");
    std::vector<int32_t> pi((size_t)std::max<int64_t>(ne, 1)), pj((size_t)std::max<int64_t>(ne, 1));
    for (int64_t e = 0; e < ne; ++e) { pi[(size_t)e] = (int32_t)pos_of(ei[e]); pj[(size_t)e] = (int32_t)pos_of(ej[e]); }
    ei = pi.data(); ej = pj.data();
    std::vector<int64_t> inc((size_t)ntot_ + 1, 0);
    for (int64_t e = 0; e < ne; ++e) { inc[(size_t)ei[e] + 1]++; inc[(size_t)ej[e] + 1]++; }
    for (int64_t c = 0; c < ntot_; ++c) inc[(size_t)c + 1] += inc[(size_t)c];
    std::vector<int32_t> ie((size_t)std::max<int64_t>(2 * ne, 1));
    {
        std::vector<int64_t> next(inc.begin(), inc.end() - 1);
        for (int64_t e = 0; e < ne; ++e) { ie[(size_t)next[(size_t)ei[e]]++] = (int32_t)e; ie[(size_t)next[(size_t)ej[e]]++] = (int32_t)e; }
    }
    const size_t m = (size_t)std::max<int64_t>(ne, 1);
    ei_.alloc(m, false); ej_.alloc(m, false); eM_.alloc(m * 9, false); ew_.alloc(m); eres_.alloc(m);
    inc_ptr_.alloc(inc.size(), false); inc_edge_.alloc(ie.size(), false);
    pos_ij_.alloc(m); pos_ji_.alloc(m); pos_d_.alloc((size_t)nloc_);
    if (ne > 0) {
        XM_HIP_CHECK(hipMemcpy(ei_.p, ei, (size_t)ne * sizeof(int32_t), hipMemcpyHostToDevice));
        XM_HIP_CHECK(hipMemcpy(ej_.p, ej, (size_t)ne * sizeof(int32_t), hipMemcpyHostToDevice));
        XM_HIP_CHECK(hipMemcpy(eM_.p, M, (size_t)ne * 9 * sizeof(double), hipMemcpyHostToDevice));
    }
// ... 251 lines not shown
    if (h) throw Error(XM_ERR_ARG, "xm_tuning_t.hess_f32: " + std::to_string(h) + " entries of Q are not finite in fp32");
}

void Context::set_edge_weights(const double *w) {
    if (schur_) {
        schur_->set_weights(w, st_);
        w_cur_.assign(w, w + schur_->nobs());
        if (schur_dense_) {
            schur_->build_dense_q(dQ_, ld_, nullptr, st_);
            if (dQ32_) refresh_q32();
        }
        return;
    }
    if (!ei_.p) throw Error(XM_ERR_ARG, "set_edge_weights: no edges attached");
    if (ne_ > 0 && !w) throw Error(XM_ERR_ARG, "set_edge_weights: null weights");
    w_cur_.assign(w, w + ne_);
    if (ne_ > 0) to_dev(ew_.p, w, (size_t)ne_ * sizeof(double));
    const bool dense = (storage_ == XM_STORAGE_DENSE);
    launch_edge_write(dense, ne_, ei_.p, ej_.p, eM_.p, ew_.p, cam0_, nloc_, inc_ptr_.p, inc_edge_.p, pos_ij_.p, pos_ji_.p, pos_d_.p,
                      dense ? nullptr : blocks_.p, dense ? dQ_ : nullptr, ld_, st_);
    if (sell_) sell_->refill(colidx_.p, blocks_.p, st_);
    if (dQ32_) refresh_q32();
    XM_HIP_CHECK(hipStreamSynchronize(st_));
}

void Context::solve(const xm_options_t &opt, xm_result_t &res) {
    opt_ = &opt;
    res_ = &res;
    verbose_ = (opt.flags & XM_FLAG_VERBOSE) != 0;
    if (opt.retraction != XM_RETRACT_QR && opt.retraction != XM_RETRACT_POLAR) throw Error(XM_ERR_ARG, "unknown retraction");
    if (opt.sum_grouping < 0 || opt.sum_grouping > 2) throw Error(XM_ERR_ARG, "sum_grouping must be 0, 1 or 2");
    retraction_ = opt.retraction;
    grouping_ = opt.sum_grouping;
    double *Rout = res.R, *sout = res.s;
    std::memset(&res, 0, sizeof(res));
    res.R = Rout; res.s = sout;
    if (!Rout || !sout) throw Error(XM_ERR_ARG, "result buffers missing");
    if (opt.max_rank > (unsigned)kMaxRank) throw Error(XM_ERR_ARG, "max_rank > 10 is not instantiated");
    if ((opt.flags & XM_FLAG_PROFILE_QW) && ev_pool_.empty()) {
        ev_pool_.resize(256);
        for (auto &e : ev_pool_) { XM_HIP_CHECK(hipEventCreate(&e.first)); XM_HIP_CHECK(hipEventCreate(&e.second)); }
    }
    ev_used_ = 0;
    hess_launches_ = 0;
    qw_samples_.clear();
    const auto t0 = clk::now();
    const size_t m = (size_t)3 * n_;
    log("+++++++++++++++++++++++++++++++++\nBegin XM\n+++++++++++++++++++++++++++++++++\n");
    unsigned o = 3;
    std::vector<double> v(m, 0.0), R0(m * 3, 0.0), Rk, s0((size_t)n_, 1.0), sk;
    if (opt.mode == XM_MODE_REBUTTLE && opt.s_ini) for (int64_t i = 0; i < n_; ++i) s0[(size_t)i] = opt.s_ini[i];
    const double s_anchor = s0[0];
    double gradtol = opt.tol, primal = 0;
    int status = XM_STATUS_NONE;
    auto identity_stack = [&]() {
        R0.assign(m * 3, 0.0);
        for (size_t i = 0; i < (size_t)n_; ++i) { R0[3 * i] = 1.0; R0[3 * i + m + 1] = 1.0; R0[3 * i + 2 * m + 2] = 1.0; }
    };
    int out_rank = 3;
    if (opt.mode == XM_MODE_RANK3) {
        log("+++++++++++++++++++++++++++++++++\nSolve TR with Rank   3\n+++++++++++++++++++++++++++++++++\n");
        identity_stack();
        setup_rank(3);
        upload_point(R0, 3, s0);
        TrResult tr = trust_region(3, gradtol, 0.0, v, opt.max_time);
        primal = tr.primal;
// ... 71 lines not shown
```

### xm-code_amd/csrc/xm_symv_step.h

```cpp
#pragma once

#include <type_traits>

#include "xm_device.h"

namespace xm {

constexpr int kSvStrip = 256;


struct SymvChunk {
    bool empty;
    int s, sc, jb, je, jfull;
    int64_t c0, R;
};
__device__ __forceinline__ SymvChunk symv_chunk(int bx, int by, int nloc, int64_t ld, int Kc, int Kf, int ysplit, int wave) {
    SymvChunk c{};
    c.empty = true;
    const int nsteps = (nloc + 1) >> 1;
    const int nstrips = (int)((ld + kSvStrip - 1) / kSvStrip);
    const int K = (by >= ysplit) ? Kf : Kc;
    c.s = by; c.sc = bx;
    {
        int jA = (int)(((int64_t)c.s * kSvStrip + kSvStrip + 5) / 6);
        if (jA > nsteps) jA = nsteps;
        const int nA = (jA + 4 * K - 1) / (4 * K);
        if (c.sc >= nA) {
            if (nstrips - 1 - c.s == c.s) return c;
            c.s = nstrips - 1 - c.s; c.sc -= nA;
        }
    }
    c.c0 = (int64_t)c.s * kSvStrip;
    int jend = (int)((c.c0 + kSvStrip + 5) / 6);
    if (jend > nsteps) jend = nsteps;
    if (c.sc * 4 * K >= jend) return c;
    c.jb = (c.sc * 4 + wave) * K;
    c.je = (c.jb + K < jend) ? c.jb + K : jend;
    c.jfull = (int)(c.c0 / 6);
    c.R = (int64_t)6 * nsteps;
    c.empty = false;
    return c;
}

template <int O>
__device__ __forceinline__ double symv_wrow_request(const double *__restrict__ W, int j, int nrows, int lane) {
    constexpr int OP = pitch_of(O);
    const int64_t wlim = (int64_t)nrows * OP - 1;
    const int64_t wi = (int64_t)6 * j * OP + (lane < 6 * OP ? lane : 0);
    return W[wi < wlim ? wi : wlim];
}
template <int O>
__device__ __forceinline__ void symv_wrow_read(double wl, int r, bool ok, double (&wr)[O]) {
    constexpr int OP = pitch_of(O);
#pragma unroll
    for (int k = 0; k < O; ++k) {
        const int lo = __builtin_amdgcn_readlane(__double2loint(wl), r * OP + k), hi = __builtin_amdgcn_readlane(__double2hiint(wl), r * OP + k);
        wr[k] = ok ? __hiloint2double(hi, lo) : 0.0;
    }
}

template <int O, bool MASK, class QAt, class WRow>
__device__ __forceinline__ void symv_step(QAt qat, const double (&mr)[2], const double (&mc)[2], WRow wrow, const double (&wc)[2][2][O],
                                          double (&ca)[2][2][O], double *L, int lane, double *prow) {
    constexpr int V = 6 * O;
#pragma unroll
    for (int r = 0; r < 6; ++r) {
        double wr[O];
        wrow(r, wr);
        double qr[2][2], qc[2][2];
#pragma unroll
        for (int h = 0; h < 2; ++h)
#pragma unroll
            for (int e = 0; e < 2; ++e) {
                const double x = qat(r, h, e);
                qr[h][e] = MASK ? x * mr[h] : x;
                qc[h][e] = MASK ? x * mc[h] : x;
            }
#pragma unroll
        for (int k = 0; k < O; ++k) {
            double t = qr[0][0] * wc[0][0][k];
            t = fma(qr[0][1], wc[0][1][k], t);
            t = fma(qr[1][0], wc[1][0][k], t);
            t = fma(qr[1][1], wc[1][1][k], t);
            L[(r * O + k) * 64 + lane] = t;
#pragma unroll
            for (int h = 0; h < 2; ++h)
// ... 69 lines not shown
```

### xm-code_amd/xmamd.py

```python
import ctypes as C
import os

import numpy as np

_HERE = os.path.dirname(os.path.abspath(__file__))
LIB_PATH = os.environ.get("XMAMD_LIB") or os.path.join(_HERE, "lib", "libxm_amd.so")
MODULE_DIR = os.path.join(_HERE, "build")

STORAGE_DENSE, STORAGE_BSR3 = 0, 1
STORAGE_BSR3_DENSE = 2
STORAGE_SCHUR = 3
STORAGE_VIEWGRAPH = 4
RETRACT_QR, RETRACT_POLAR = 0, 1
MODE_SOLVE, MODE_RANK3, MODE_REBUTTLE = 0, 1, 2
FLAG_VERBOSE, FLAG_FIX_STALE_SR, FLAG_PROFILE_QW, FLAG_HOST_STEPPED = 1, 2, 4, 8
CERT_EIG_NOT_CONVERGED = 1
CERT_EIG_EXACT = 2
FLAG_WARM_R = 16
FLAG_HOST_OUTER = 64
FLAG_DEVICE_OUTER = 128
FLAG_MODEL_RECURRENCE = 32

EXPORTS = [
    "xm_last_error", "xm_version", "xm_abi_revision", "xm_solve", "xm_solve_rank3", "xm_solve_rebuttle", "xm_ctx_create", "xm_ctx_solve",
    "xm_ctx_destroy", "xm_dense_ld", "xm_dev_count", "xm_dev_alloc", "xm_dev_free", "xm_dev_h2d", "xm_dev_d2h",
    "xm_dev_sync", "xm_dense_upload", "xm_dense_from_bsr3", "xm_qw_dense", "xm_qw_dense_sym", "xm_qw_bsr3", "xm_retract", "xm_retract_polar", "xm_recover_rotations",
    "xm_comm_unique_id", "xm_comm_init", "xm_comm_init_shm", "xm_comm_init_ipc", "xm_comm_finalize", "xm_partition", "xm_partition_blocks",
    "xm_symv_plan", "xm_sell_layout", "xm_sell_locality", "xm_sell_create", "xm_sell_create2", "xm_sell_quat_roundtrip", "xm_sell_destroy", "xm_qw_sell", "xm_qw_sell_padded",
    "xm_ctx_attach_edges", "xm_ctx_edge_residuals", "xm_ctx_edge_residuals_recovered", "xm_ctx_xm2_filter", "xm_ctx_xm2_round", "xm_ctx_set_edge_weights", "xm_ctx_recover_tp", "xm_ctx_schur_info", "xm_ctx_qw", "xm_spd_inverse", "xm_ctx_transport", "xm_ctx_sell_wpad", "xm_ctx_product_kind", "xm_symw_plan", "xm_symw_use",
    "xm_ctx_schur_precond_info", "xm_schur_aggregate_plan",
    "xm_dense_to_f32", "xm_qw_dense_f32", "xm_qw_dense_sym_f32",
    "xm_ctx_bundle_adjust", "xm_ctx_reprojection_errors", "xm_spd_solve", "xm_la_probe", "xm_ba_aggregate_plan", "xm_ctx_ba_probe",
    "xm_clean_observations", "xm_ctx_clean_observations", "xm_ctx_rtr_probe", "xm_ctx_outer_probe", "xm_ctx_cert_probe", "xm_tridiag_min", "xm_ctx_schur_probe",
    "xm_ctx_dense_q", "xm_create_matrix", "xm_schur_dense_limits",
    "xm_pair_filter", "xm_pair_filter_limits",
    "xm_lift_observations", "xm_lift_limits",
    "xm_build_tracks", "xm_tracks_limits", "xm_tracks_split_host", "xm_tracks_split_device", "xm_tracks_split_limits", "xm_tracks_split_stats",
    "xm_view_graph_filter", "xm_view_graph_limits",
    "xm_view_graph_calibrate", "xm_view_graph_calibrate_probe", "xm_view_graph_calibrate_limits",
    "xm_view_graph_rotations", "xm_view_graph_rotations_probe", "xm_view_graph_rotations_limits",
    "xm_ctx_filter_tracks", "xm_track_filter_limits",
    "xm_prune_weakly_connected", "xm_ctx_prune_weakly_connected", "xm_prune_limits",
    "xm_ctx_global_positioning", "xm_ctx_gp_probe", "xm_gp_limits",
]
BENCH_EXPORTS = ["xm_bench_last_error", "xm_qw_dense_time", "xm_qw_dense_sym_time", "xm_qw_dense_f32_time", "xm_qw_dense_sym_f32_time", "xm_bench_symv_k", "xm_bench_dense_policy", "xm_qw_dense_sym_trace", "xm_qw_dense_strip_time", "xm_qw_dense_strip_ks", "xm_qw_bsr3_time", "xm_bench_bsr_binned", "xm_qw_sell_time",
                 "xm_retract_variant", "xm_recover_rotations_variant", "xm_peer_allgather_bench", "xm_qw_symw_time", "xm_bench_grid_barrier"]
PRODUCT_KINDS = {0: "dense", 1: "dense_sym", 2: "bsr3", 3: "sell", 4: "sell_quat", 5: "schur"}


class XmError(RuntimeError):
    pass


class Tuning(C.Structure):
    _fields_ = [(k, C.c_int32) for k in ("sym", "sym_min_rows", "sell", "sell_slabs", "sell_lmax", "sell_gather", "sell_codec", "overlap",
                                         "overlap_min_mb", "cert_dense_rows", "lanczos_mmax", "lanczos_restarts", "watchdog_s", "balance",
                                         "exchange", "split_k", "sell_wpad", "exchange_fence", "schur_host_assembly", "schur_trace",
                                         "schur_solver", "schur_dense_max", "debug_drop_finalize", "debug_peer_mute", "schur_pcg_first",
                                         "schur_pcg_hess_digits", "hess_f32", "schur_dense_q")]


class Problem(C.Structure):
# ... 422 lines not shown
                                     [C.c_void_p] * 4 + [C.POINTER(C.c_int64), C.c_void_p, C.POINTER(TracksResult)]
        L.xm_tracks_limits.argtypes = [C.c_void_p]
        L.xm_view_graph_filter.argtypes = [C.c_int64] + [C.c_void_p] * 5 + [C.c_int64] + [C.c_void_p] * 12 + [C.POINTER(VgOptions)] + [C.c_void_p] * 7 + \
                                          [C.POINTER(VgResult)]
        L.xm_view_graph_limits.argtypes = [C.c_void_p]
        L.xm_view_graph_calibrate.argtypes = [C.c_int64] + [C.c_void_p] * 3 + [C.c_int64, C.c_void_p, C.c_int64] + [C.c_void_p] * 7 + \
                                             [C.POINTER(VgcOptions)] + [C.c_void_p] * 10 + [C.POINTER(VgcResult)]
        L.xm_view_graph_calibrate_probe.argtypes = [C.c_int64] + [C.c_void_p] * 3 + [C.c_int64, C.c_void_p, C.c_int64] + [C.c_void_p] * 5 + \
                                                   [C.POINTER(VgcOptions), C.POINTER(VgcProbe)]
        L.xm_view_graph_calibrate_limits.argtypes = [C.c_void_p]
        L.xm_view_graph_rotations.argtypes = [C.c_int64, C.c_void_p, C.c_void_p, C.c_int64] + [C.c_void_p] * 4 + [C.POINTER(VgrOptions)] + \
                                             [C.c_void_p] * 5 + [C.POINTER(VgrResult)]
        L.xm_view_graph_rotations_probe.argtypes = [C.c_int64, C.c_void_p, C.c_void_p, C.c_int64] + [C.c_void_p] * 4 + \
                                                   [C.POINTER(VgrOptions), C.POINTER(VgrProbe)]
        L.xm_view_graph_rotations_limits.argtypes = [C.c_void_p]
        L.xm_tracks_split_host.argtypes = [C.c_int64, C.c_void_p, C.c_int64, C.c_void_p, C.c_void_p, C.c_void_p, C.POINTER(C.c_int64), C.POINTER(C.c_int64)]
        L.xm_tracks_split_device.argtypes = L.xm_tracks_split_host.argtypes
        L.xm_tracks_split_limits.argtypes = [C.c_void_p]
        L.xm_tracks_split_stats.argtypes = [C.c_void_p]
        L.xm_ctx_filter_tracks.argtypes = [C.c_void_p, C.POINTER(TfOptions)] + [C.c_void_p] * 7 + [C.POINTER(TfResult)]
        L.xm_track_filter_limits.argtypes = [C.c_void_p]
        L.xm_ctx_global_positioning.argtypes = [C.c_void_p, C.POINTER(GpOptions), C.c_void_p, C.c_void_p, C.c_void_p, C.c_void_p, C.POINTER(GpResult)]
        L.xm_ctx_gp_probe.argtypes = [C.c_void_p, C.c_void_p, C.c_void_p, C.c_void_p, C.POINTER(GpProbe)]
        L.xm_gp_limits.argtypes = [C.c_void_p]
        L.xm_prune_weakly_connected.argtypes = [C.c_int64, C.c_int64, C.c_int64, C.c_void_p, C.c_void_p, C.c_void_p, C.POINTER(PruneOptions), C.c_void_p,
                                                C.c_void_p, C.c_void_p, C.POINTER(PruneResult)]
        L.xm_ctx_prune_weakly_connected.argtypes = [C.c_void_p, C.POINTER(PruneOptions), C.c_void_p, C.c_void_p, C.c_void_p, C.POINTER(PruneResult)]
        L.xm_prune_limits.argtypes = [C.c_void_p]
        L.xm_ctx_reprojection_errors.argtypes = [C.c_void_p, C.c_void_p, C.c_void_p, C.c_void_p, C.c_void_p]
        L.xm_ctx_transport.argtypes = [C.c_void_p, C.POINTER(C.c_int), C.c_char_p, C.c_size_t]
        L.xm_ctx_dense_q.argtypes = [C.c_void_p, C.c_void_p, C.c_int64]
        L.xm_create_matrix.argtypes = [C.c_int64, C.c_int64, C.c_int64, C.c_void_p, C.c_void_p, C.c_void_p, C.c_void_p, C.c_void_p, C.c_int64, C.c_void_p]
        L.xm_schur_dense_limits.argtypes = [C.c_void_p]
        L.xm_ctx_schur_info.argtypes = [C.c_void_p, C.POINTER(C.c_int), C.c_void_p, C.POINTER(C.c_double)]
        L.xm_ctx_schur_precond_info.argtypes = [C.c_void_p, C.POINTER(C.c_int), C.POINTER(C.c_int64), C.POINTER(C.c_int)]
        L.xm_schur_aggregate_plan.argtypes = [C.c_int64, C.c_int64, C.c_void_p, C.c_void_p, C.c_int, C.c_void_p]
        L.xm_ba_aggregate_plan.argtypes = [C.c_int64, C.c_int64, C.c_void_p, C.c_void_p, C.c_void_p, C.c_int, C.c_void_p]
        L.xm_ctx_sell_wpad.argtypes = [C.c_void_p, C.POINTER(C.c_int)]
        L.xm_ctx_product_kind.argtypes = [C.c_void_p, C.c_int, C.POINTER(C.c_int)]
        L.xm_bench_last_error.restype = C.c_char_p
        L.xm_symw_plan.argtypes = [C.c_int64, C.c_int, C.c_int, C.c_int, C.c_void_p, C.c_void_p]
        L.xm_symw_use.argtypes = [C.c_int, C.c_int, C.c_int]
        L.xm_qw_symw_time.argtypes = [C.c_int64, C.c_int, C.c_int, C.c_int, C.c_int, C.c_int, C.c_void_p, C.POINTER(C.c_int64)]
        L.xm_bench_grid_barrier.argtypes = [C.c_int, C.c_int, C.c_int, C.c_void_p]
        L.xm_dev_count.argtypes = [C.POINTER(C.c_int)]
        L.xm_dev_alloc.argtypes = [C.POINTER(C.c_void_p), C.c_size_t]
        L.xm_dev_free.argtypes = [C.c_void_p]
        L.xm_dev_h2d.argtypes = [C.c_void_p, C.c_void_p, C.c_size_t]
        L.xm_dev_d2h.argtypes = [C.c_void_p, C.c_void_p, C.c_size_t]
        L.xm_dense_upload.argtypes = [C.c_void_p, C.c_int64, C.c_int64, C.POINTER(C.c_void_p)]
        L.xm_dense_from_bsr3.argtypes = [C.c_void_p, C.c_void_p, C.c_void_p, C.c_int64, C.POINTER(C.c_void_p)]
        L.xm_qw_dense.argtypes = [C.c_void_p, C.c_int64, C.c_int, C.c_void_p, C.c_void_p, C.c_double, C.c_void_p]
        L.xm_qw_dense_sym.argtypes = L.xm_qw_dense.argtypes
        L.xm_dense_to_f32.argtypes = [C.c_void_p, C.c_int64, C.POINTER(C.c_void_p)]
        L.xm_qw_dense_f32.argtypes = L.xm_qw_dense.argtypes
        L.xm_qw_dense_sym_f32.argtypes = L.xm_qw_dense.argtypes
        L.xm_qw_dense_f32_time.argtypes = [C.c_void_p, C.c_int64, C.c_int, C.c_void_p, C.c_void_p, C.c_int, C.POINTER(C.c_double)]
        L.xm_qw_dense_sym_f32_time.argtypes = L.xm_qw_dense_f32_time.argtypes
        L.xm_qw_dense_sym_time.argtypes = [C.c_void_p, C.c_int64, C.c_int, C.c_void_p, C.c_void_p, C.c_int, C.POINTER(C.c_double)]
        L.xm_bench_symv_k.argtypes = [C.c_int, C.c_int, C.c_int]
        L.xm_qw_dense_sym_trace.argtypes = [C.c_void_p, C.c_int64, C.c_int, C.c_void_p, C.c_void_p, C.c_void_p, C.c_int64, C.c_void_p, C.POINTER(C.c_int)]
        L.xm_qw_bsr3.argtypes = [C.c_void_p, C.c_void_p, C.c_void_p, C.c_int64, C.c_int, C.c_void_p, C.c_void_p,
                                 C.c_double, C.c_void_p]
        L.xm_retract.argtypes = [C.c_int64, C.c_int, C.c_void_p, C.c_void_p, C.c_void_p, C.c_void_p, C.c_double,
                                 C.c_void_p, C.c_void_p, C.c_void_p]
        L.xm_retract_polar.argtypes = L.xm_retract.argtypes
# ... 1663 lines not shown
        info = {k: getattr(res, k) for k, _ in Result._fields_ if k not in ("R", "s", "struct_size")}
        x2 = {k: getattr(inf, k) for k, _ in Xm2Info._fields_ if k != "struct_size"}
        return np.ascontiguousarray(Ro[:, : res.rank]), so, info, x2

    def set_edge_weights(self, w):
        w = np.ascontiguousarray(w, dtype=np.float64)
        assert w.size == self.ne
        _chk(lib().xm_ctx_set_edge_weights(self.h, w.ctypes.data_as(C.c_void_p)))
        self._w = w.reshape(-1).copy()

    def solve(self, max_rank, tol, lam, max_time=1000.0, mode=MODE_SOLVE, flags=0, s_ini=None, trace=0, R_ini=None, retraction=RETRACT_QR,
              grouping=0):
        n = self.n
        rmax = max(int(max_rank), 3)
        R = np.zeros((3 * n, rmax + 1), order="F"); s = np.zeros(n)
        opt = Options(); res = Result()
        opt.struct_size, res.struct_size = C.sizeof(Options), C.sizeof(Result)
        opt.retraction, opt.sum_grouping = int(retraction), int(grouping)
        opt.max_rank, opt.tol, opt.lam, opt.max_time, opt.mode, opt.flags = int(max_rank), tol, lam, max_time, mode, flags
        si = None
        if s_ini is not None:
            si = np.ascontiguousarray(s_ini, dtype=np.float64).reshape(-1)
            opt.s_ini = si.ctypes.data_as(C.c_void_p)
        ri = None
        if R_ini is not None:
            ri = np.asfortranarray(np.asarray(R_ini, dtype=np.float64)[:, :3])
            opt.R_ini = ri.ctypes.data_as(C.c_void_p); opt.flags |= FLAG_WARM_R
        tr = None
        if trace:
            tr = np.zeros((trace, 6)); opt.trace_cap = trace; opt.trace = tr.ctypes.data_as(C.c_void_p)
        res.R = R.ctypes.data_as(C.c_void_p); res.s = s.ctypes.data_as(C.c_void_p)
        _chk(lib().xm_ctx_solve(self.h, C.byref(opt), C.byref(res)))
        info = {k: getattr(res, k) for k, _ in Result._fields_ if k not in ("R", "s", "struct_size")}
        if tr is not None:
            info["trace"] = tr[: res.trace_len].copy()
        return np.ascontiguousarray(R[:, : res.rank]), s, info

    def close(self):
        if self.h:
            lib().xm_ctx_destroy(self.h)
            self.h = C.c_void_p()

    def __del__(self):
        try:
            self.close()
        except Exception:
            pass


def solve_dense(Q, max_rank, tol, lam, tuning=None, **kw):
    ctx = Context(Q=Q, tuning=tuning)
    try:
        return ctx.solve(max_rank, tol, lam, **kw)
    finally:
        ctx.close()


def import_XM():
    import importlib
    import sys
    if MODULE_DIR not in sys.path:
        sys.path.insert(0, MODULE_DIR)
    return importlib.import_module("XM")
```

Measured before the change: 24350.

## Fuse tCG step direction update into symmetric QW sweep for two-launch iterations

Adds a fused symv kernel path in which each workgroup derives the next tCG search direction and W tile on the fly from the current p, r, Hp and R instead of reading a precomputed W, while extra grid rows run the cg-step body. The goal is to cut one kernel launch and one global round trip of W per inner iteration. To avoid races the p and r buffers are double-buffered by parity. The cost is redundant recomputation of partial-sum reductions and W entries per workgroup, plus fixed waves-per-EU occupancy. A three-launch flag keeps the old path.

Measured after the change: 25410, median of 6. +4.4%, better.

```diff
diff --git a/include/xm_amd.h b/include/xm_amd.h
--- a/include/xm_amd.h
+++ b/include/xm_amd.h
@@ -106,6 +106,7 @@
 #define XM_FLAG_MODEL_RECURRENCE 32u
 #define XM_FLAG_HOST_OUTER    64u
 #define XM_FLAG_DEVICE_OUTER 128u
+#define XM_FLAG_TCG_THREE_LAUNCH 256u
 #define XM_FLAG_WARM_R        16u
 
 #define XM_RETRACT_QR    0
@@ -484,6 +485,7 @@
                      int64_t ldq, double *Abar );
 int xm_schur_dense_limits(int64_t out[3]);
 int xm_ctx_schur_info(xm_ctx_t *ctx, int *uses_cg, int64_t stats[3], double *last_relres);
+int xm_ctx_tcg_two_launch(xm_ctx_t *ctx, int *count);
 int xm_ctx_schur_precond_info(xm_ctx_t *ctx, int *kind, int64_t *aggregates, int *block);
 
 #define XM_BA_FIX_ROTATIONS 1u
diff --git a/xm-code_amd/csrc/xm_capi.hip b/xm-code_amd/csrc/xm_capi.hip
--- a/xm-code_amd/csrc/xm_capi.hip
+++ b/xm-code_amd/csrc/xm_capi.hip
@@ -329,6 +329,13 @@
     XM_TRY
     if (!out) throw xm::Error(XM_ERR_ARG, "xm_schur_dense_limits: null output");
     out[0] = xm::kSchurDenseQWinCams; out[1] = xm::kSchurAbarPanel; out[2] = xm::kSchurDenseQMaxCams;
+    return XM_OK;
+    XM_CATCH
+}
+int xm_ctx_tcg_two_launch(xm_ctx_t *ctx, int *count) {
+    XM_TRY
+    if (!ctx || !ctx->impl || !count) throw xm::Error(XM_ERR_ARG, "xm_ctx_tcg_two_launch: single-GPU context and a non-null output needed");
+    *count = ctx->impl->tcg_two_launch_count();
     return XM_OK;
     XM_CATCH
 }
diff --git a/xm-code_amd/csrc/xm_common.h b/xm-code_amd/csrc/xm_common.h
--- a/xm-code_amd/csrc/xm_common.h
+++ b/xm-code_amd/csrc/xm_common.h
@@ -203,6 +203,7 @@
 struct TcgParity {
     TcgScal *scal_cur, *scal_next;
     double *ps_cur, *ps_next, *rs_cur, *rs_next;
+    double *pR_cur, *pR_next, *rR_cur, *rR_next;
     size_t chunk, b_off;
     double *pcur;
     double *parts;
@@ -226,7 +227,7 @@
     TcgParity v;
     int nA, nB, world;
     const double *HpR, *Hps, *R, *s;
-    double *pR, *vR, *vs, *HvR, *Hvs, *rR;
+    double *vR, *vs, *HvR, *Hvs;
     double *Wloc, *Wpad;
     unsigned long long *hstat;
     int64_t mat;
@@ -234,6 +235,17 @@
     int grouping;
     PeerXchg xchg;
 };
+
+struct TcgFuse {
+    int gy, nA, nB, grp;
+    const TcgScal *scal_cur;
+    TcgScal *scal_next;
+    const double *parts;
+    const double *HpR, *Hps, *R, *s, *pR_cur, *ps_cur, *rR_cur, *rs_cur;
+    double *pR_next, *ps_next, *rR_next, *rs_next, *vR, *vs, *HvR, *Hvs, *Wloc, *partsB_out;
+    unsigned long long *hstat;
+};
+constexpr int kSvDeriveRows = 768;
 
 void launch_qw_dense(int o, int epi, const double *Q, int64_t ld, const double *W, double alpha, const CamArgs &a,
                      hipStream_t st);
@@ -262,7 +274,8 @@
 };
 void launch_qw_sym_traced(int o, const double *Q, int64_t ld, const double *W, const CamArgs &a, SymvWork &work, unsigned long long *trace, hipStream_t st);
 void launch_qw_sym(int o, int epi, const double *Q, int64_t ld, const double *W, double alpha, const CamArgs &a, SymvWork &work, hipStream_t st,
-                   int rev = 0);
+                   int rev = 0, const CgStepArgs *step = nullptr);
+bool symv_derives(const SymvWork &work, int o);
 void launch_asym(const double *Q, int64_t ld, int64_t m, double *out, int grid, hipStream_t st);
 void launch_dense_to_f32(const double *src, float *dst, int64_t rows, int64_t ld, unsigned int *bad, hipStream_t st);
 void launch_qw_dense_f32(int o, int epi, const float *Qf, const double *Qd, int64_t ld, const double *W, double alpha, const CamArgs &a, hipStream_t st);
diff --git a/xm-code_amd/csrc/xm_device.h b/xm-code_amd/csrc/xm_device.h
--- a/xm-code_amd/csrc/xm_device.h
+++ b/xm-code_amd/csrc/xm_device.h
@@ -86,29 +86,32 @@
 }
 
 constexpr int kPre = 4;
-struct PartialsPre { double v[4][kPre]; };
+template <int KP> struct PartialsPreN { double v[4][KP]; };
+using PartialsPre = PartialsPreN<kPre>;
+template <int KP>
 __device__ __forceinline__ void sum_partials_prefetch(const double *p0, const double *p1, const double *p2, int count, const double *p3, int count3,
-                                                      PartialsPre &pre, int grp) {
-#pragma unroll
-    for (int r = 0; r < kPre; ++r) {
+                                                      PartialsPreN<KP> &pre, int grp) {
+#pragma unroll
+    for (int r = 0; r < KP; ++r) {
         const int i = threadIdx.x + 256 * r;
         const int j = (i < count) ? sum_perm(i, count, grp) : 0, j3 = (i < count3) ? sum_perm(i, count3, grp) : 0;
         pre.v[0][r] = (i < count) ? p0[j] : 0.0; pre.v[1][r] = (i < count) ? p1[j] : 0.0; pre.v[2][r] = (i < count) ? p2[j] : 0.0;
         pre.v[3][r] = (i < count3) ? p3[j3] : 0.0;
     }
 }
+template <int KP>
 __device__ __forceinline__ void sum_partials256_x4_pre(const double *p0, const double *p1, const double *p2, int count, const double *p3,
-                                                       int count3, bool use3, const PartialsPre &pre, double *sh16, double (&out)[4], int grp = 0) {
+                                                       int count3, bool use3, const PartialsPreN<KP> &pre, double *sh16, double (&out)[4], int grp = 0) {
     double v[4] = {0.0, 0.0, 0.0, 0.0};
 #pragma unroll
-    for (int r = 0; r < kPre; ++r) {
+    for (int r = 0; r < KP; ++r) {
         const int i = threadIdx.x + 256 * r;
         if (i < count) { v[0] += pre.v[0][r]; v[1] += pre.v[1][r]; v[2] += pre.v[2][r]; }
         if (use3 && i < count3) v[3] += pre.v[3][r];
     }
-    for (int i = threadIdx.x + 256 * kPre; i < count; i += 256) { const int j = sum_perm(i, count, grp); v[0] += p0[j]; v[1] += p1[j]; v[2] += p2[j]; }
+    for (int i = threadIdx.x + 256 * KP; i < count; i += 256) { const int j = sum_perm(i, count, grp); v[0] += p0[j]; v[1] += p1[j]; v[2] += p2[j]; }
     if (use3)
-        for (int i = threadIdx.x + 256 * kPre; i < count3; i += 256) v[3] += p3[sum_perm(i, count3, grp)];
+        for (int i = threadIdx.x + 256 * KP; i < count3; i += 256) v[3] += p3[sum_perm(i, count3, grp)];
 #pragma unroll
     for (int k = 0; k < 4; ++k) v[k] = wave_sum(v[k]);
     __syncthreads();
diff --git a/xm-code_amd/csrc/xm_kernels.hip b/xm-code_amd/csrc/xm_kernels.hip
--- a/xm-code_amd/csrc/xm_kernels.hip
+++ b/xm-code_amd/csrc/xm_kernels.hip
@@ -285,12 +285,41 @@
 }
 
 constexpr int kSvTraceSlots = 24;
-template <int O, bool TRACE = false>
-__global__ __launch_bounds__(256) void qw_symv_kernel(const double *__restrict__ Q, int64_t ld, const double *__restrict__ W, int nloc, int Kc, int Kf, int ysplit, int nt_step0,
-                                                        const TcgScal *__restrict__ scal, double *__restrict__ Prow,
-                                                        double *__restrict__ Pcol, unsigned long long *__restrict__ trace, int rev, int by_phase) {
+struct TcgNext;
+struct TcgSums { double pHp, rHp, HpHp, rr_prev; };
+__device__ __forceinline__ TcgNext tcg_next(const TcgScal &sc, double pHp, double rHp, double HpHp);
+__device__ __forceinline__ double tcg_w_next(double step, double beta, double pv, double rv, double hp, double psv, double rsv, double hs, double sv, double Rv);
+__device__ __forceinline__ double tcg_dir_next(double step, double beta, double pv, double rv, double hp);
+__device__ __forceinline__ double tcg_w_of(double sv, double pn, double psn, double Rv);
+constexpr int kSvDerivePre = 2;
+__device__ __forceinline__ bool tcg_derive_head(const TcgFuse &fu, const PartialsPreN<kSvDerivePre> &pre, double *sh16, bool lead, double &step, double &beta);
+template <int O, bool XCHG>
+__device__ __forceinline__ void cg_step_body(int bid, int nblk, int nloc, const TcgScal *__restrict__ scal_cur, TcgScal *scal_next, const double *__restrict__ parts,
+                                             int nA_loc, int nB_loc, int world, const double *__restrict__ HpR, const double *__restrict__ Hps,
+                                             const double *__restrict__ R, const double *__restrict__ s, const double *pR_cur, double *pR_next,
+                                             const double *__restrict__ ps_cur, double *ps_next, double *vR, double *vs, double *HvR, double *Hvs,
+                                             const double *rR_cur, double *rR_next, const double *__restrict__ rs_cur, double *rs_next, double *Wloc,
+                                             double *partsB_out, unsigned long long *hstat, int b_off, int64_t mat, double *Afull, double *Wfull, int grp,
+                                             const PeerXchg *xp, double *Wpad);
+template <int O, bool TRACE, bool DERIVE>
+__device__ __forceinline__ void qw_symv_body(const double *__restrict__ Q, int64_t ld, const double *__restrict__ W, int nloc, int Kc, int Kf, int ysplit, int nt_step0,
+                                             const TcgScal *__restrict__ scal, double *__restrict__ Prow,
+                                             double *__restrict__ Pcol, unsigned long long *__restrict__ trace, int rev, int by_phase, const TcgFuse &fu) {
     constexpr int OP = pitch_of(O), V = 6 * O;
+    static_assert(!(TRACE && DERIVE), "the traced sweep reads W");
     __shared__ __attribute__((aligned(16))) double lds[4][V * 64];
+    __shared__ double wcol[DERIVE ? kSvStrip * O : 1], wrws[DERIVE ? kSvDeriveRows : 1], shd[16];
+    __shared__ double cam_psn[DERIVE ? 256 : 1], cam_s[DERIVE ? 256 : 1];
+    if constexpr (DERIVE) {
+        if ((int)blockIdx.y >= fu.gy) {
+            const int bid = ((int)blockIdx.y - fu.gy) * (int)gridDim.x + (int)blockIdx.x;
+            if (bid < fu.nB)
+                cg_step_body<O, false>(bid, fu.nB, nloc, fu.scal_cur, fu.scal_next, fu.parts, fu.nA, fu.nB, 1, fu.HpR, fu.Hps, fu.R, fu.s, fu.pR_cur, fu.pR_next,
+                                       fu.ps_cur, fu.ps_next, fu.vR, fu.vs, fu.HvR, fu.Hvs, fu.rR_cur, fu.rR_next, fu.rs_cur, fu.rs_next, fu.Wloc,
+                                       fu.partsB_out, fu.hstat, 0, (int64_t)nloc * 3 * OP, nullptr, nullptr, fu.grp, nullptr, nullptr);
+            return;
+        }
+    }
     const int lane = threadIdx.x & 63, wave = __builtin_amdgcn_readfirstlane(threadIdx.x >> 6);
     unsigned long long *tr = nullptr;
     if constexpr (TRACE) {
@@ -318,7 +347,7 @@
         const Slot &b = slot[decltype(sl)::value];
         const int64_t r0 = (int64_t)6 * j;
         auto qat = [&](int r, int h, int e) __attribute__((always_inline)) { return e ? b.q[r][h].y : b.q[r][h].x; };
-        auto wrow = [&](int r, double (&wr)[O]) __attribute__((always_inline)) { symv_wrow_read<O>(b.wl, r, r0 + r < nrows, wr); };
+        auto wrow = [&](int r, double (&wr)[O]) __attribute__((always_inline)) { symv_wrow_read<O, DERIVE ? O : OP>(b.wl, r, r0 + r < nrows, wr); };
         double *prow = Prow + ((size_t)ch.s * (size_t)ch.R + (size_t)r0) * O;
         double mr[2] = {1.0, 1.0}, mc[2] = {1.0, 1.0};
         if (j < ch.jfull) symv_step<O, false>(qat, mr, mc, wrow, wc, ca, L, lane, prow);
@@ -335,11 +364,53 @@
             ++nrun;
         }
     };
+    const int j0 = jb - wave * ((int)blockIdx.y >= ysplit ? Kf : Kc);
+    auto derive_w = [&]() __attribute__((always_inline)) -> bool {
+        constexpr int NC = O, NR = kSvDeriveRows / 256, kColCams = kSvStrip / 3 + 2, kRowCams = kSvDeriveRows / (3 * O);
+        static_assert(!DERIVE || kColCams + kRowCams <= 256, "one thread per camera of the workgroup's W");
+        const int64_t wtot = (int64_t)nrows * OP;
+        const int ccam0 = (int)(ch.c0 / 3), rcam0 = 2 * j0;
+        auto windex = [&](int m) __attribute__((always_inline)) -> int64_t {
+            const int e = (m < NC ? 256 * m : 256 * (m - NC)) + (int)threadIdx.x;
+            return ((m < NC ? ch.c0 : (int64_t)6 * j0) + e / O) * OP + e % O;
+        };
+        double ops[NC + NR][4];
+#pragma unroll
+        for (int m = 0; m < NC + NR; ++m) {
+            const int64_t idx = windex(m);
+            const int64_t ic = idx < wtot ? idx : wtot - 1;
+            ops[m][0] = fu.pR_cur[ic]; ops[m][1] = fu.rR_cur[ic]; ops[m][2] = fu.HpR[ic]; ops[m][3] = fu.R[ic];
+        }
+        const int tcam = (int)threadIdx.x < kColCams ? ccam0 + (int)threadIdx.x : rcam0 + (int)threadIdx.x - kColCams;
+        const int tcc = tcam < nloc ? tcam : nloc - 1;
+        const double c_ps = fu.ps_cur[tcc], c_rs = fu.rs_cur[tcc], c_hs = fu.Hps[tcc], c_s = fu.s[tcc];
+        PartialsPreN<kSvDerivePre> pre;
+        sum_partials_prefetch(fu.parts, fu.parts + fu.nA, fu.parts + 2 * fu.nA, fu.nA, fu.parts + 3 * fu.nA, fu.nB, pre, fu.grp);
+        double step, beta;
+        if (!tcg_derive_head(fu, pre, shd, blockIdx.x == 0 && blockIdx.y == 0 && threadIdx.x == 0, step, beta)) return false;
+        if ((int)threadIdx.x < kColCams + kRowCams) { cam_psn[threadIdx.x] = tcg_dir_next(step, beta, c_ps, c_rs, c_hs); cam_s[threadIdx.x] = c_s; }
+        __syncthreads();
+#pragma unroll
+        for (int m = 0; m < NC + NR; ++m) {
+            const int64_t idx = windex(m);
+            const int64_t ic = idx < wtot ? idx : wtot - 1;
+            const int cam = (int)(ic / (3 * OP));
+            int ts = (m < NC) ? cam - ccam0 : kColCams + cam - rcam0;
+            ts = ts < 0 ? 0 : (ts < kColCams + kRowCams ? ts : kColCams + kRowCams - 1);
+            const double wv = tcg_w_of(cam_s[ts], tcg_dir_next(step, beta, ops[m][0], ops[m][1], ops[m][2]), cam_psn[ts], ops[m][3]);
+            (m < NC ? wcol : wrws)[threadIdx.x + 256 * (m < NC ? m : m - NC)] = idx < wtot ? wv : 0.0;
+        }
+        __syncthreads();
+        return true;
+    };
     auto sweep = [&](auto ntag) __attribute__((always_inline)) -> bool {
         constexpr bool NT = decltype(ntag)::value;
-        auto load = [&](int j, auto sl) __attribute__((always_inline)) {
+        auto loadw = [&](int j, auto sl) __attribute__((always_inline)) {
+            slot[decltype(sl)::value].wl = wrws[(j - j0) * 6 * O + (lane < 6 * O ? lane : 0)];
+        };
+        auto loadq = [&](int j, auto sl) __attribute__((always_inline)) {
             Slot &b = slot[decltype(sl)::value];
-            b.wl = symv_wrow_request<O>(W, j, nrows, lane);
+            if constexpr (!DERIVE) b.wl = symv_wrow_request<O>(W, j, nrows, lane);
             const int64_t r0 = (int64_t)6 * j;
 #pragma unroll
             for (int r = 0; r < 6; ++r) {
@@ -353,30 +424,56 @@
                 }
             }
         };
-        if (jb < je) load(symv_walk_at(jb, je, rev, 0), std::integral_constant<int, 0>{});
+        auto load = [&](int j, auto sl) __attribute__((always_inline)) {
+            if constexpr (DERIVE) loadw(j, sl);
+            loadq(j, sl);
+        };
+        if (jb < je) loadq(symv_walk_at(jb, je, rev, 0), std::integral_constant<int, 0>{});
+        if constexpr (DERIVE) {
+            if (!derive_w()) return false;
+            if (jb < je) loadw(symv_walk_at(jb, je, rev, 0), std::integral_constant<int, 0>{});
+        }
 #pragma unroll
         for (int h = 0; h < 2; ++h)
 #pragma unroll
             for (int e = 0; e < 2; ++e)
 #pragma unroll
                 for (int k = 0; k < O; ++k) {
-                    const double t = W[(size_t)((h ? cB : cA) + e) * OP + k];
-                    wc[h][e][k] = (h == 0 || half1) ? t : 0.0;
+                    if constexpr (DERIVE) {
+                        wc[h][e][k] = wcol[(128 * h + 2 * lane + e) * O + k];
+                    } else {
+                        const double t = W[(size_t)((h ? cB : cA) + e) * OP + k];
+                        wc[h][e][k] = (h == 0 || half1) ? t : 0.0;
+                    }
                     ca[h][e][k] = 0.0;
                 }
-        if (scal != nullptr) {
-            if (by_phase ? (scal->phase >= PH_STOP) : (scal->status != 0)) return false;
+        if constexpr (!DERIVE) {
+            if (scal != nullptr) {
+                if (by_phase ? (scal->phase >= PH_STOP) : (scal->status != 0)) return false;
+            }
         }
         if constexpr (TRACE) { if (lane == 0) tr[1] = wall_clock64(); }
         symv_walk(jb, je, rev, load, run);
         return true;
     };
-    const bool alive = (jb >= nt_step0) ? sweep(std::true_type{}) : sweep(std::false_type{});
+    const bool alive = DERIVE ? sweep(std::false_type{}) : ((jb >= nt_step0) ? sweep(std::true_type{}) : sweep(std::false_type{}));
     if (!alive) return;
     if constexpr (TRACE) { if (lane == 0) tr[kSvTraceSlots - 3] = wall_clock64(); }
 
     symv_colsum<O>(ca, lds, wave, lane, wave == 0 || half1, Pcol + ((size_t)ch.sc * (size_t)ld + (size_t)(cA + 128 * wave)) * O);
     if constexpr (TRACE) { if (lane == 0) tr[kSvTraceSlots - 2] = wall_clock64(); }
+}
+template <int O, bool TRACE = false>
+__global__ __launch_bounds__(256) void qw_symv_kernel(const double *__restrict__ Q, int64_t ld, const double *__restrict__ W, int nloc, int Kc, int Kf, int ysplit, int nt_step0,
+                                                        const TcgScal *__restrict__ scal, double *__restrict__ Prow,
+                                                        double *__restrict__ Pcol, unsigned long long *__restrict__ trace, int rev, int by_phase) {
+    qw_symv_body<O, TRACE, false>(Q, ld, W, nloc, Kc, Kf, ysplit, nt_step0, scal, Prow, Pcol, trace, rev, by_phase, TcgFuse{});
+}
+template <int O>
+__global__ __launch_bounds__(256) __attribute__((amdgpu_waves_per_eu(2, 2)))
+void qw_symv_step_kernel(const double *__restrict__ Q, int64_t ld, int nloc, int Kc, int Kf, int ysplit, int nt_step0, double *__restrict__ Prow,
+                         double *__restrict__ Pcol, int rev, TcgFuse fu) {
+    qw_symv_body<O, false, true>(Q, ld, nullptr, nloc, Kc, Kf, ysplit, nt_step0, nullptr, Prow, Pcol, nullptr, rev, 0, fu);
 }
 
 template <int O, int EPI>
@@ -781,40 +878,106 @@
     }
 }
 
-template <int O>
-__global__ __launch_bounds__(256) void cg_step_kernel(int nloc, const TcgScal *__restrict__ scal_cur, TcgScal *scal_next,
-                                                       const double *__restrict__ parts, int nA_loc, int nB_loc, int world,
-                                                       const double *__restrict__ HpR,
-                                                       const double *__restrict__ Hps, const double *__restrict__ R,
-                                                       const double *__restrict__ s, double *pR, const double *__restrict__ ps_cur,
-                                                       double *ps_next, double *vR, double *vs, double *HvR, double *Hvs, double *rR,
-                                                       const double *__restrict__ rs_cur, double *rs_next, double *Wloc,
-                                                       double *partsB_out, unsigned long long *hstat, int b_off, int64_t mat,
-                                                       double *Afull, double *Wfull, int grp, PeerXchg x, double *Wpad) {
+struct TcgNext {
+    int mode;
+    bool cg, conv, newdir;
+    double step, beta, rr_est;
+    int status, iter;
+};
+__device__ __forceinline__ TcgNext tcg_next(const TcgScal &sc, double pHp, double rHp, double HpHp) {
+    TcgNext n;
+    const StepDecision d = tcg_decide(sc, pHp);
+    n.mode = d.mode; n.step = d.step; n.cg = (d.mode == 0);
+    n.conv = false; n.newdir = false; n.beta = 0.0; n.rr_est = 0.0; n.status = d.mode; n.iter = sc.iter;
+    if (d.mode == 5) { n.cg = false; return n; }
+    const double step = d.step;
+    double rr_est = sc.rr + 2.0 * step * rHp + step * step * HpHp;
+    if (rr_est < 0.0) rr_est = 0.0;
+    n.rr_est = rr_est;
+    n.conv = n.cg && (sqrt(rr_est) < sc.gradnorm * fmin(sc.gradnorm, 0.1));
+    n.beta = rr_est / sc.rr;
+    n.newdir = n.cg && !n.conv;
+    if (n.cg) {
+        if (n.conv) n.status = 3;
+        else { n.iter = sc.iter + 1; n.status = (n.iter >= kMaxInner) ? 6 : 0; }
+    }
+    return n;
+}
+__device__ __forceinline__ TcgScal tcg_scal_next(const TcgScal &sc, const TcgNext &n, double pHp, bool keep_hv) {
+    TcgScal nx = sc;
+    const double step = n.step, beta = n.beta, rr_est = n.rr_est;
+    nx.last_step = step;
+    if (!keep_hv) nx.model = sc.model - step * sc.rr + 0.5 * step * step * pHp;
+    if (!n.cg) {
+        nx.status = n.mode;
+    } else {
+        nx.rr = rr_est;
+        nx.vv = sc.vv + 2.0 * step * sc.vp + step * step * sc.pp;
+        nx.vp = beta * (sc.vp + step * sc.pp);
+        nx.pp = beta * beta * sc.pp + rr_est;
+        nx.status = n.status; nx.iter = n.iter;
+    }
+    return nx;
+}
+__device__ __forceinline__ double tcg_dir_next(double step, double beta, double pv, double rv, double hp) {
+    const double rn = rv + step * hp;
+    return beta * pv - rn;
+}
+__device__ __forceinline__ double tcg_w_of(double sv, double pn, double psn, double Rv) { return sv * pn + psn * Rv; }
+__device__ __forceinline__ double tcg_w_next(double step, double beta, double pv, double rv, double hp, double psv, double rsv, double hs, double sv, double Rv) {
+    return tcg_w_of(sv, tcg_dir_next(step, beta, pv, rv, hp), tcg_dir_next(step, beta, psv, rsv, hs), Rv);
+}
+__device__ __forceinline__ bool tcg_derive_head(const TcgFuse &fu, const PartialsPreN<kSvDerivePre> &pre, double *sh16, bool lead, double &step, double &beta) {
+    const TcgScal sc0 = *fu.scal_cur;
+    step = 0.0; beta = 0.0;
+    if (sc0.status != 0) return false;
+    double t[4];
+    sum_partials256_x4_pre(fu.parts, fu.parts + fu.nA, fu.parts + 2 * fu.nA, fu.nA, fu.parts + 3 * fu.nA, fu.nB, sc0.iter > 0, pre, sh16, t, fu.grp);
+    double pHp = 0.0, rHp = 0.0, HpHp = 0.0, rr_prev = 0.0;
+    pHp += t[0]; rHp += t[1]; HpHp += t[2];
+    if (sc0.iter > 0) rr_prev += t[3];
+    TcgScal sc = sc0;
+    if (sc0.iter > 0) sc.rr = rr_prev;
+    const TcgNext n = tcg_next(sc, pHp, rHp, HpHp);
+    if (lead) publish_host(fu.hstat, pack_stat(sc.seq, n.iter, n.status));
+    step = n.step; beta = n.beta;
+    return n.status == 0;
+}
+
+template <int O, bool XCHG>
+__device__ __forceinline__ void cg_step_body(int bid, int nblk, int nloc, const TcgScal *__restrict__ scal_cur, TcgScal *scal_next, const double *__restrict__ parts,
+                                             int nA_loc, int nB_loc, int world, const double *__restrict__ HpR, const double *__restrict__ Hps,
+                                             const double *__restrict__ R, const double *__restrict__ s, const double *pR_cur, double *pR_next,
+                                             const double *__restrict__ ps_cur, double *ps_next, double *vR, double *vs, double *HvR, double *Hvs,
+                                             const double *rR_cur, double *rR_next, const double *__restrict__ rs_cur, double *rs_next, double *Wloc,
+                                             double *partsB_out, unsigned long long *hstat, int b_off, int64_t mat, double *Afull, double *Wfull, int grp,
+                                             const PeerXchg *xp, double *Wpad) {
     constexpr int OP = pitch_of(O);
     __shared__ double sh[4];
     __shared__ double sh16[16];
     __shared__ int sh_flag;
     const int64_t total = (int64_t)nloc * 3 * OP;
-    const int64_t stride = (int64_t)gridDim.x * 256;
-    int64_t i = (int64_t)blockIdx.x * 256 + threadIdx.x;
+    const int64_t stride = (int64_t)nblk * 256;
+    int64_t i = (int64_t)bid * 256 + threadIdx.x;
     const bool in0 = i < total;
     const int camf = (int)(i / (3 * OP));
     const bool own0 = in0 && (i % (3 * OP) == 0);
     double hp = 0, pv = 0, vv0 = 0, hv = 0, rv = 0, Rv = 0, hs = 0, psv = 0, rsv = 0, sv = 1, vsv = 0, hvs = 0;
     const bool keep_hv = HvR != nullptr;
-    if (in0) { hp = HpR[i]; pv = pR[i]; vv0 = vR[i]; if (keep_hv) hv = HvR[i]; rv = rR[i]; Rv = R[i]; hs = Hps[camf]; psv = ps_cur[camf]; rsv = rs_cur[camf]; sv = s[camf]; }
+    if (in0) { hp = HpR[i]; pv = pR_cur[i]; vv0 = vR[i]; if (keep_hv) hv = HvR[i]; rv = rR_cur[i]; Rv = R[i]; hs = Hps[camf]; psv = ps_cur[camf]; rsv = rs_cur[camf]; sv = s[camf]; }
     if (own0) { vsv = vs[camf]; if (keep_hv) hvs = Hvs[camf]; }
-    const bool can_pre = x.world <= 1;
+    const bool can_pre = !XCHG || xp->world <= 1;
     PartialsPre pre;
     if (can_pre) sum_partials_prefetch(parts + b_off, parts + b_off + nA_loc, parts + b_off + 2 * nA_loc, nA_loc, parts + b_off + 3 * nA_loc, nB_loc, pre, grp);
     const TcgScal sc0 = *scal_cur;
-    const bool lead = (blockIdx.x == 0 && threadIdx.x == 0);
+    const bool lead = (bid == 0 && threadIdx.x == 0);
     if (sc0.status != 0) {
         if (lead) *scal_next = sc0;
         return;
     }
-    if (x.world > 1) {
+    if constexpr (XCHG) {
+    if (xp->world > 1) {
+        const PeerXchg &x = *xp;
         const int par = sc0.iter & 1;
         const size_t chunk_d = (size_t)b_off + 3 * (size_t)nA_loc + nB_loc;
         const size_t off = ((size_t)par * x.world + x.rank) * chunk_d;
@@ -824,14 +987,14 @@
             for (int p = 0; p < x.world; ++p) {
                 if (p == x.rank) continue;
                 double *dst = x.buf[p] + off;
-                for (size_t j = (size_t)blockIdx.x * 256 + threadIdx.x; j < chunk_d; j += (size_t)stride)
+                for (size_t j = (size_t)bid * 256 + threadIdx.x; j < chunk_d; j += (size_t)stride)
                     __hip_atomic_store(dst + j, src[j], __ATOMIC_RELAXED, __HIP_MEMORY_SCOPE_SYSTEM);
             }
             asm volatile("s_waitcnt vmcnt(0)" ::: "memory");
             __syncthreads();
             if (threadIdx.x == 0) {
                 const unsigned long long t = __hip_atomic_fetch_add(x.ticket + par, 1ull, __ATOMIC_RELAXED, __HIP_MEMORY_SCOPE_AGENT);
-                sh_flag = (t + 1 == gridDim.x);
+                sh_flag = (t + 1 == (unsigned)nblk);
                 if (sh_flag) __hip_atomic_store(x.ticket + par, 0ull, __ATOMIC_RELAXED, __HIP_MEMORY_SCOPE_AGENT);
             }
             __syncthreads();
@@ -841,14 +1004,14 @@
             for (int p = 0; p < x.world; ++p) {
                 if (p == x.rank) continue;
                 double *dst = x.buf[p] + off;
-                for (size_t j = (size_t)blockIdx.x * 256 + threadIdx.x; j < chunk_d; j += (size_t)stride) dst[j] = src[j];
+                for (size_t j = (size_t)bid * 256 + threadIdx.x; j < chunk_d; j += (size_t)stride) dst[j] = src[j];
             }
             __threadfence_system();
             asm volatile("s_waitcnt vmcnt(0)" ::: "memory");
             __syncthreads();
             if (threadIdx.x == 0) {
                 const unsigned long long t = __hip_atomic_fetch_add(x.ticket + par, 1ull, __ATOMIC_ACQ_REL, __HIP_MEMORY_SCOPE_AGENT);
-                sh_flag = (t + 1 == gridDim.x);
+                sh_flag = (t + 1 == (unsigned)nblk);
                 if (sh_flag) __hip_atomic_store(x.ticket + par, 0ull, __ATOMIC_RELAXED, __HIP_MEMORY_SCOPE_AGENT);
             }
             __syncthreads();
@@ -885,6 +1048,7 @@
         }
         __builtin_amdgcn_fence(__ATOMIC_ACQUIRE, "");
     }
+    }
     const int chunk = b_off + 3 * nA_loc + nB_loc;
     double pHp = 0.0, rHp = 0.0, HpHp = 0.0, rr_prev = 0.0;
     for (int r = 0; r < world; ++r) {
@@ -897,8 +1061,8 @@
     }
     TcgScal sc = sc0;
     if (sc0.iter > 0) sc.rr = rr_prev;
-    const StepDecision d = tcg_decide(sc, pHp);
-    if (d.mode == 5) {
+    const TcgNext nx_ = tcg_next(sc, pHp, rHp, HpHp);
+    if (nx_.mode == 5) {
         if (lead) {
             TcgScal nx = sc; nx.status = 5; nx.last_step = 0.0;
             *scal_next = nx;
@@ -906,13 +1070,10 @@
         }
         return;
     }
-    const double step = d.step;
-    const bool cg = (d.mode == 0);
-    double rr_est = sc.rr + 2.0 * step * rHp + step * step * HpHp;
-    if (rr_est < 0.0) rr_est = 0.0;
-    const bool conv = cg && (sqrt(rr_est) < sc.gradnorm * fmin(sc.gradnorm, 0.1));
-    const double beta = rr_est / sc.rr;
-    const bool newdir = cg && !conv;
+    const double step = nx_.step;
+    const bool cg = nx_.cg;
+    const double beta = nx_.beta;
+    const bool newdir = nx_.newdir;
     double acc = 0.0;
     if (in0) {
         vR[i] = vv0 + step * pv;
@@ -920,14 +1081,14 @@
         if (cg) {
             const double rn = rv + step * hp;
             const double rsn = rsv + step * hs;
-            rR[i] = rn;
+            rR_next[i] = rn;
             acc += rn * rn;
             if (newdir) {
                 const double pn = beta * pv - rn;
                 const double psn = beta * psv - rsn;
-                pR[i] = pn;
+                pR_next[i] = pn;
                 if (!Afull) {
-                    const double wv = sv * pn + psn * Rv;
+                    const double wv = tcg_w_next(step, beta, pv, rv, hp, psv, rsv, hs, sv, Rv);
                     if (Wloc) Wloc[i] = wv;
                     if (Wpad) Wpad[(size_t)camf * 16 + (i - (int64_t)camf * (3 * OP))] = wv;
                 }
@@ -940,20 +1101,21 @@
     for (i += stride; i < total; i += stride) {
         const int cam = (int)(i / (3 * OP));
         const bool own = (i % (3 * OP) == 0);
-        const double hpi = HpR[i], pi = pR[i], hsi = Hps[cam], psi = ps_cur[cam];
+        const double hpi = HpR[i], pi = pR_cur[i], hsi = Hps[cam], psi = ps_cur[cam];
         vR[i] += step * pi;
         if (keep_hv) HvR[i] += step * hpi;
         if (cg) {
-            const double rn = rR[i] + step * hpi;
-            const double rsn = rs_cur[cam] + step * hsi;
-            rR[i] = rn;
+            const double rri = rR_cur[i], rsi = rs_cur[cam];
+            const double rn = rri + step * hpi;
+            const double rsn = rsi + step * hsi;
+            rR_next[i] = rn;
             acc += rn * rn;
             if (newdir) {
                 const double pn = beta * pi - rn;
                 const double psn = beta * psi - rsn;
-                pR[i] = pn;
+                pR_next[i] = pn;
                 if (!Afull) {
-                    const double wv = s[cam] * pn + psn * R[i];
+                    const double wv = tcg_w_next(step, beta, pi, rri, hpi, psi, rsi, hsi, s[cam], R[i]);
                     if (Wloc) Wloc[i] = wv;
                     if (Wpad) Wpad[(size_t)cam * 16 + (i - (int64_t)cam * (3 * OP))] = wv;
                 }
@@ -966,7 +1128,7 @@
     if (Afull && newdir) {
         const int64_t full = mat * world;
         const bool first = (sc0.iter == 0);
-        for (int64_t j = (int64_t)blockIdx.x * 256 + threadIdx.x; j < full; j += stride) {
+        for (int64_t j = (int64_t)bid * 256 + threadIdx.x; j < full; j += stride) {
             const int64_t r = j / mat;
             const double b = parts[(size_t)r * chunk + (size_t)(j - r * mat)];
             const double w = Wfull[j];
@@ -977,29 +1139,27 @@
     }
     if (cg) {
         const double tot = block_sum256(acc, sh);
-        if (threadIdx.x == 0) partsB_out[blockIdx.x] = tot;
+        if (threadIdx.x == 0) partsB_out[bid] = tot;
     }
     if (lead) {
-        TcgScal nx = sc;
-        nx.last_step = step;
-        if (!keep_hv) nx.model = sc.model - step * sc.rr + 0.5 * step * step * pHp;
-        if (!cg) {
-            nx.status = d.mode;
-        } else {
-            nx.rr = rr_est;
-            nx.vv = sc.vv + 2.0 * step * sc.vp + step * step * sc.pp;
-            nx.vp = beta * (sc.vp + step * sc.pp);
-            nx.pp = beta * beta * sc.pp + rr_est;
-            if (conv) {
-                nx.status = 3;
-            } else {
-                nx.iter = sc.iter + 1;
-                nx.status = (nx.iter >= kMaxInner) ? 6 : 0;
-            }
-        }
+        const TcgScal nx = tcg_scal_next(sc, nx_, pHp, keep_hv);
         *scal_next = nx;
         publish_host(hstat, pack_stat(nx.seq, nx.iter, nx.status));
     }
+}
+
+template <int O>
+__global__ __launch_bounds__(256) void cg_step_kernel(int nloc, const TcgScal *__restrict__ scal_cur, TcgScal *scal_next,
+                                                       const double *__restrict__ parts, int nA_loc, int nB_loc, int world,
+                                                       const double *__restrict__ HpR,
+                                                       const double *__restrict__ Hps, const double *__restrict__ R,
+                                                       const double *__restrict__ s, const double *pR_cur, double *pR_next, const double *__restrict__ ps_cur,
+                                                       double *ps_next, double *vR, double *vs, double *HvR, double *Hvs, const double *rR_cur, double *rR_next,
+                                                       const double *__restrict__ rs_cur, double *rs_next, double *Wloc,
+                                                       double *partsB_out, unsigned long long *hstat, int b_off, int64_t mat,
+                                                       double *Afull, double *Wfull, int grp, PeerXchg x, double *Wpad) {
+    cg_step_body<O, true>(blockIdx.x, gridDim.x, nloc, scal_cur, scal_next, parts, nA_loc, nB_loc, world, HpR, Hps, R, s, pR_cur, pR_next, ps_cur, ps_next, vR, vs,
+                          HvR, Hvs, rR_cur, rR_next, rs_cur, rs_next, Wloc, partsB_out, hstat, b_off, mat, Afull, Wfull, grp, &x, Wpad);
 }
 
 __global__ __launch_bounds__(256) void outer_finalize_kernel(const double *__restrict__ partsA, int nA_loc, int world,
@@ -2174,14 +2334,29 @@
 }
 template <int O>
 static void qw_symv_epi(int epi, const double *Q, int64_t ld, const double *W, double alpha, const CamArgs &a, SymvWork &work,
-                        hipStream_t st, int rev, unsigned long long *trace = nullptr) {
+                        hipStream_t st, int rev, unsigned long long *trace = nullptr, const CgStepArgs *step = nullptr) {
     const auto [gs, rK, rKf, ys, nstrips] = symv_geom(work, a.nloc, ld, O);
     const SymvPlan &pl = work.plan;
     double *const Prow = work.prow.p, *const Pcol = work.pcol.p;
     const TcgScal *sc = (epi == EPI_HESS || epi == EPI_AUTO) ? a.scal : (const TcgScal *)nullptr;
     const int by_phase = (epi == EPI_AUTO) ? 1 : 0;
     const int nt0 = symv_nt_step0(a.nloc, sizeof(double));
-    if (trace) {
+    if (step) {
+        if constexpr (O == 3 || O == 4) {
+            if (epi != EPI_HESS || trace || !symv_derives(work, O) || step->world > 1 || step->Afull || step->Wpad || step->v.b_off != 0)
+                throw Error(-2, "symmetric product: this launch cannot carry the tCG step");
+            const CgStepArgs &S = *step;
+            TcgFuse fu;
+            fu.gy = (int)gs.y; fu.nA = S.nA; fu.nB = S.nB; fu.grp = S.grouping;
+            fu.scal_cur = S.v.scal_cur; fu.scal_next = S.v.scal_next; fu.parts = S.v.pcur;
+            fu.HpR = S.HpR; fu.Hps = S.Hps; fu.R = S.R; fu.s = S.s;
+            fu.pR_cur = S.v.pR_cur; fu.ps_cur = S.v.ps_cur; fu.rR_cur = S.v.rR_cur; fu.rs_cur = S.v.rs_cur;
+            fu.pR_next = S.v.pR_next; fu.ps_next = S.v.ps_next; fu.rR_next = S.v.rR_next; fu.rs_next = S.v.rs_next;
+            fu.vR = S.vR; fu.vs = S.vs; fu.HvR = S.HvR; fu.Hvs = S.Hvs; fu.Wloc = S.Wloc; fu.partsB_out = S.v.partsB_out; fu.hstat = S.hstat;
+            const dim3 gf(gs.x, gs.y + (S.nB + gs.x - 1) / gs.x);
+            hipLaunchKernelGGL((qw_symv_step_kernel<O>), gf, dim3(256), 0, st, Q, ld, a.nloc, pl.K, pl.Kf, ys, nt0, Prow, Pcol, rev, fu);
+        } else throw Error(-2, "symmetric product: the tCG step travels with the sweep at o = 3 and 4 only");
+    } else if (trace) {
         if constexpr (O == 3 || O == 4) hipLaunchKernelGGL((qw_symv_kernel<O, true>), gs, dim3(256), 0, st, Q, ld, W, a.nloc, pl.K, pl.Kf, ys, nt0, sc, Prow, Pcol, trace, rev, by_phase);
     } else hipLaunchKernelGGL((qw_symv_kernel<O>), gs, dim3(256), 0, st, Q, ld, W, a.nloc, pl.K, pl.Kf, ys, nt0, sc, Prow, Pcol, trace, rev, by_phase);
     const dim3 g(qw_grid(a.nloc)), b(256);
@@ -2198,6 +2373,9 @@
         default: throw Error(-2, "bad epilogue");
     }
 }
+bool symv_derives(const SymvWork &work, int o) {
+    return work && (o == 3 || o == 4) && o <= work.o && 4 * std::max(work.plan.K, work.plan.Kf) * 6 * o <= kSvDeriveRows;
+}
 int symv_trace_slots() { return kSvTraceSlots; }
 void launch_qw_sym_traced(int o, const double *Q, int64_t ld, const double *W, const CamArgs &a, SymvWork &work, unsigned long long *trace, hipStream_t st) {
     if (trace == nullptr) throw Error(-2, "traced symmetric product: no trace buffer");
@@ -2208,13 +2386,13 @@
 }
 
 void launch_qw_sym(int o, int epi, const double *Q, int64_t ld, const double *W, double alpha, const CamArgs &a, SymvWork &work, hipStream_t st,
-                   int rev) {
+                   int rev, const CgStepArgs *step) {
     if (a.nloc <= 0) return;
     switch (o) {
-        case 1: qw_symv_epi<1>(epi, Q, ld, W, alpha, a, work, st, rev & 1); break;
-        case 3: qw_symv_epi<3>(epi, Q, ld, W, alpha, a, work, st, rev & 1); break;
-        case 4: qw_symv_epi<4>(epi, Q, ld, W, alpha, a, work, st, rev & 1); break;
-        case 5: qw_symv_epi<5>(epi, Q, ld, W, alpha, a, work, st, rev & 1); break;
+        case 1: qw_symv_epi<1>(epi, Q, ld, W, alpha, a, work, st, rev & 1, nullptr, step); break;
+        case 3: qw_symv_epi<3>(epi, Q, ld, W, alpha, a, work, st, rev & 1, nullptr, step); break;
+        case 4: qw_symv_epi<4>(epi, Q, ld, W, alpha, a, work, st, rev & 1, nullptr, step); break;
+        case 5: qw_symv_epi<5>(epi, Q, ld, W, alpha, a, work, st, rev & 1, nullptr, step); break;
         default: throw Error(-2, "symmetric product is instantiated for o = 1, 3..5");
     }
     check_launch("qw_symv");
@@ -2336,8 +2514,8 @@
 }
 void launch_cg_step(int o, const CgStepArgs &a, hipStream_t st) {
     XM_DISPATCH_O(o, hipLaunchKernelGGL((cg_step_kernel<O_>), dim3(a.nB), dim3(256), 0, st, a.nloc,
-                                        a.v.scal_cur, a.v.scal_next, a.v.pcur, a.nA, a.nB, a.world, a.HpR, a.Hps, a.R, a.s, a.pR, a.v.ps_cur, a.v.ps_next, a.vR,
-                                        a.vs, a.HvR, a.Hvs, a.rR, a.v.rs_cur, a.v.rs_next, a.Wloc, a.v.partsB_out, a.hstat, (int)a.v.b_off, a.mat, a.Afull,
+                                        a.v.scal_cur, a.v.scal_next, a.v.pcur, a.nA, a.nB, a.world, a.HpR, a.Hps, a.R, a.s, a.v.pR_cur, a.v.pR_next, a.v.ps_cur, a.v.ps_next, a.vR,
+                                        a.vs, a.HvR, a.Hvs, a.v.rR_cur, a.v.rR_next, a.v.rs_cur, a.v.rs_next, a.Wloc, a.v.partsB_out, a.hstat, (int)a.v.b_off, a.mat, a.Afull,
                                         a.Wfull, a.grouping, a.xchg, a.Wpad));
     check_launch("cg_step");
 }
diff --git a/xm-code_amd/csrc/xm_solver.h b/xm-code_amd/csrc/xm_solver.h
--- a/xm-code_amd/csrc/xm_solver.h
+++ b/xm-code_amd/csrc/xm_solver.h
@@ -151,6 +151,7 @@
     int64_t n_landmarks() const;
     int64_t n_observations() const;
     void dense_q(double *q, int64_t ldq);
+    int tcg_two_launch_count() const { return tcg_two_launch_count_; }
     bool schur_info(int64_t out[3], double *relres) const;
     int schur_precond(int64_t *aggregates, int *block) const;
 
@@ -206,7 +207,7 @@
     const double *wpad_next_ = nullptr;
     PointState ps_[2];
     int cur_ = 0;
-    DevBuf<double> rR_, rs_, rsB_, pR_, psA_, psB_, vR_, vs_, HvR_, Hvs_, HpR_, Hps_;
+    DevBuf<double> rR_, rRB_, rs_, rsB_, pR_, pRB_, psA_, psB_, vR_, vs_, HvR_, Hvs_, HpR_, Hps_;
     DevBuf<double> partsA_, partsB_, partsM_;
     SymvWork symv_;
     DevBuf<double> ksum_;
@@ -259,6 +260,9 @@
     int run_tcg(double rr, double delta, int adopted = 0);
     int enqueue_spec_tcg();
     void tcg_enqueue_iteration(int i, bool profile);
+    bool tcg_two_launch() const;
+    const CgStepArgs *fuse_step_ = nullptr;
+    int tcg_two_launch_count_ = 0;
     TcgParity tcg_parity(int par) const;
     void cand_role(CamArgs &a, const PointState &P, const double *R, const double *s) const;
     CamArgs tcg_cam_args(const TcgParity &v, bool cand) const;
diff --git a/xm-code_amd/csrc/xm_solver.hip b/xm-code_amd/csrc/xm_solver.hip
--- a/xm-code_amd/csrc/xm_solver.hip
+++ b/xm-code_amd/csrc/xm_solver.hip
@@ -436,7 +436,7 @@
     const int world = comm_->world;
     const int o_top = std::max(o, (int)std::min<unsigned>(opt_ ? opt_->max_rank : 0u, (unsigned)kMaxRank));
     const size_t mat_top = (size_t)nloc_ * 3 * pitch_of(o_top);
-    for (DevBuf<double> *b : {&R_, &Rc_, &D_, &rR_, &pR_, &vR_, &HvR_, &HpR_}) b->ensure(mat, st_, mat_top);
+    for (DevBuf<double> *b : {&R_, &Rc_, &D_, &rR_, &rRB_, &pR_, &pRB_, &vR_, &HvR_, &HpR_}) b->ensure(mat, st_, mat_top);
     for (DevBuf<double> *b : {&s_, &sc_, &rs_, &rsB_, &psA_, &psB_, &vs_, &Hvs_, &Hps_}) b->ensure(vec, st_);
     for (int k = 0; k < 2; ++k) {
         ps_[k].G.ensure(mat, st_, mat_top); ps_[k].rgR.ensure(mat, st_, mat_top); ps_[k].egs.ensure(vec, st_); ps_[k].rgs.ensure(vec, st_); ps_[k].S0.ensure(vec * 9, st_);
@@ -583,7 +583,7 @@
         else { CamArgs ar = a; ar.rev = sym_rev_; launch_qw_dense_f32(o, epi, dQ32_, dQ_, ld_, W_.p, alpha, ar, st_); }
     } else if (storage_ == XM_STORAGE_DENSE) {
         if (symw_ && o == o_ && o >= 3 && o <= sym_max_o_ && epi != EPI_CERT) product_symw(epi, o, alpha, a);
-        else if (sym_ok_ && o == o_ && o >= 3 && o <= sym_max_o_ && epi != EPI_CERT && symv_) launch_qw_sym(o, epi, dQ_, ld_, W_.p, alpha, a, symv_, st_, sym_rev_);
+        else if (sym_ok_ && o == o_ && o >= 3 && o <= sym_max_o_ && epi != EPI_CERT && symv_) launch_qw_sym(o, epi, dQ_, ld_, W_.p, alpha, a, symv_, st_, sym_rev_, fuse_step_);
         else { CamArgs ar = a; ar.rev = sym_rev_; launch_qw_dense(o, epi, dQ_, ld_, W_.p, alpha, ar, st_); }
     } else if (storage_ == XM_STORAGE_SCHUR) {
         schur_->product(o, epi, W_.p, alpha, a, st_);
@@ -720,10 +720,24 @@
 }
 
 void Context::tcg_enqueue_iteration(int i, bool profile) {
+    if (tcg_two_launch()) {
+        const CgStepArgs P = (i > 0) ? cg_step_args(i - 1) : CgStepArgs();
+        fuse_step_ = (i > 0) ? &P : nullptr;
+        struct Clear { const CgStepArgs *&p; ~Clear() { p = nullptr; } } clear{fuse_step_};
+        tcg_product(EPI_HESS, tcg_cam_args(tcg_parity(i & 1), false), i & 1, profile);
+        return;
+    }
     const CgStepArgs S = cg_step_args(i);
     tcg_product(EPI_HESS, tcg_cam_args(S.v, false), i & 1, profile);
     if (comm_->active() && xchg_.world <= 1) comm_->allgather(S.v.pcur, S.v.chunk, st_);
     launch_cg_step(o_, S, st_);
+}
+
+bool Context::tcg_two_launch() const {
+    if (!opt_ || (opt_->flags & (XM_FLAG_HOST_STEPPED | XM_FLAG_TCG_THREE_LAUNCH))) return false;
+    if (comm_->active() || comm_->world > 1 || storage_ != XM_STORAGE_DENSE || dQ32_ || symw_ || !sym_ok_ || !symv_ || wpad()) return false;
+    if (o_ < 3 || o_ > sym_max_o_ || !symv_derives(symv_, o_)) return false;
+    return !device_outer_applies(o_);
 }
 
 TcgParity Context::tcg_parity(int par) const {
@@ -732,6 +746,9 @@
     v.scal_cur = scal_.p + par; v.scal_next = scal_.p + (par ^ 1);
     v.ps_cur = par ? psB_.p : psA_.p; v.ps_next = par ? psA_.p : psB_.p;
     v.rs_cur = par ? rsB_.p : rs_.p; v.rs_next = par ? rs_.p : rsB_.p;
+    const bool one = opt_ && device_outer_applies(o_);
+    v.pR_cur = (par && !one) ? pRB_.p : pR_.p; v.pR_next = (par || one) ? pR_.p : pRB_.p;
+    v.rR_cur = (par && !one) ? rRB_.p : rR_.p; v.rR_next = (par || one) ? rR_.p : rRB_.p;
     v.b_off = comm_->active() ? (size_t)nloc_ * 3 * OP_ : 0;
     v.chunk = v.b_off + 3 * nA + (size_t)tcg_blocks();
     double *pB = xchg_.world > 1 ? partsB_peer_ : partsB_.p;
@@ -748,7 +765,7 @@
 
 CamArgs Context::tcg_cam_args(const TcgParity &v, bool cand) const {
     CamArgs a = cam_args(cur_);
-    a.scal = v.scal_cur; a.ps = v.ps_cur; a.rs = v.rs_cur;
+    a.scal = v.scal_cur; a.pR = v.pR_cur; a.ps = v.ps_cur; a.rR = v.rR_cur; a.rs = v.rs_cur;
     a.partials = v.parts; a.Bout = v.Bout;
     if (cand) cand_role(a, ps_[cur_ ^ 1], Rc_.p, sc_.p);
     return a;
@@ -782,7 +799,7 @@
     a.nloc = nloc_; a.v = tcg_parity(i & 1);
     a.nA = prod_grid(); a.nB = tcg_blocks(); a.world = comm_->world;
     a.HpR = HpR_.p; a.Hps = Hps_.p; a.R = R_.p; a.s = s_.p;
-    a.pR = pR_.p; a.vR = vR_.p; a.vs = vs_.p; a.HvR = model_rec ? nullptr : HvR_.p; a.Hvs = model_rec ? nullptr : Hvs_.p; a.rR = rR_.p;
+    a.vR = vR_.p; a.vs = vs_.p; a.HvR = model_rec ? nullptr : HvR_.p; a.Hvs = model_rec ? nullptr : Hvs_.p;
     a.Wloc = wpad() ? nullptr : W_.p + (size_t)cam0_ * 3 * OP_; a.Wpad = wpad();
     a.hstat = hstat_dev_; a.mat = (int64_t)nloc_ * 3 * OP_;
     a.Afull = comm_->active() ? Afull_.p : nullptr; a.Wfull = W_.p;
@@ -808,6 +825,10 @@
     return n_spec;
 }
 
+#ifndef XM_TCG_PAIRS_AHEAD
+#define XM_TCG_PAIRS_AHEAD 3
+#endif
+constexpr int kTcgPairsAhead = XM_TCG_PAIRS_AHEAD;
 int Context::run_tcg(double rr, double delta, int adopted) {
     const bool stepped = (opt_->flags & XM_FLAG_HOST_STEPPED) != 0;
     const bool profile = (opt_->flags & XM_FLAG_PROFILE_QW) != 0;
@@ -820,9 +841,12 @@
     const bool fused = xchg_.world > 1;
     if (fused) xchg_.epoch_base = (++tcg_runs_) << 12;
     const bool lockstep = comm_->active() && !fused;
-    const int run_ahead = (lockstep || prod_grid() >= 64) ? 2 : 3;
+    const bool two = tcg_two_launch();
+    const int cap = two ? kMaxInner + 1 : kMaxInner;
+    const int run_ahead = two ? kTcgPairsAhead : ((lockstep || prod_grid() >= 64) ? 2 : 3);
     int fin_status = 0, fin_iter = 0;
     int it = adopted;
+    auto fin_par = [&]() { return (two ? std::max(it - 1, 0) : it) & 1; };
     auto enqueue = [&](int i) { tcg_enqueue_iteration(i, profile); };
     auto read_scal = [&](int par) {
         TcgScal sc;
@@ -847,13 +871,13 @@
             const int status = valid ? (int)(v & 0xff) : 0;
             const int done = valid ? (int)((v >> 8) & 0xffffff) : 0;
             if (status != 0) { fin_status = status; fin_iter = done; break; }
-            if (it < kMaxInner && it - done < run_ahead) { enqueue(it++); continue; }
+            if (it < cap && it - done < run_ahead) { enqueue(it++); continue; }
             __builtin_ia32_pause();
             if (secs_since(last_progress) > 200e-6) {
                 if (stream_idle(last_change, "the truncated-CG progress word")) {
-                    TcgScal sc = read_scal(it & 1);
+                    TcgScal sc = read_scal(fin_par());
                     if (sc.status != 0) { fin_status = sc.status; fin_iter = sc.iter; break; }
-                    if (it >= kMaxInner) { fin_status = 6; fin_iter = kMaxInner; break; }
+                    if (it >= cap) { fin_status = 6; fin_iter = kMaxInner; break; }
                     *hstat_ = ((unsigned long long)tcg_seq_ << 32) | ((unsigned long long)(unsigned)sc.iter << 8);
                     if (it - sc.iter >= run_ahead) enqueue(it++);
                 }
@@ -867,7 +891,7 @@
         const int T = (fin_status == 6) ? fin_iter - 1 : fin_iter;
         while (it < std::min(kMaxInner, T + 2)) enqueue(it++);
     }
-    return it;
+    return two ? std::max(it - 1, 0) : it;
 }
 
 TrResult Context::trust_region(int o, double &gradtol, double linesearch_step, const std::vector<double> &v_dir, double max_time) {
@@ -921,6 +945,7 @@
     }
     eval_point(cur_, R_.p, s_.p, f, rr);
     if (device_outer_applies(o)) return trust_region_device(o, gradtol, f, rr, delta, delta_bar, max_time);
+    if (tcg_two_launch()) tcg_two_launch_count_++;
     double loss = f;
 
     int endreason = 6, trstatus = 4, shrink_count = 0, inner_print = 1, k = 0;
@@ -1611,8 +1636,8 @@
         I.rgR = D_.p; I.rgs = sc_.p;
         I.hstat = nullptr; I.seq = 0;
         launch_tcg_init(o, I, st_);
-        up_mat(pR_.p, q.pR, 1.0); up_vec(v.ps_cur, q.ps, 1.0, false);
-        up_mat(rR_.p, q.rR, 1.0); up_vec(v.rs_cur, q.rs, 1.0, false);
+        up_mat(v.pR_cur, q.pR, 1.0); up_vec(v.ps_cur, q.ps, 1.0, false);
+        up_mat(v.rR_cur, q.rR, 1.0); up_vec(v.rs_cur, q.rs, 1.0, false);
         TcgScal sc;
         std::memset(&sc, 0, sizeof(sc));
         if (want_step) {
@@ -1631,6 +1656,7 @@
             up_mat(vR_.p, q.vR, 1.0); up_vec(vs_.p, q.vs, 1.0, false);
             if (!model_rec) { up_mat(HvR_.p, q.HvR, 1.0); up_vec(Hvs_.p, q.Hvs, 1.0, false); }
             up_vec(v.ps_next, q.ps, 1.0, false); up_vec(v.rs_next, q.rs, 1.0, false);
+            if (v.pR_next != v.pR_cur) { up_mat(v.pR_next, q.pR, 1.0); up_mat(v.rR_next, q.rR, 1.0); }
             if (q.scal_in.iter > 0) to_dev(v.parts + (size_t)3 * nA, q.partsB_in, (size_t)nB * sizeof(double));
             XM_HIP_CHECK(hipMemsetAsync(v.partsB_out, 0, (size_t)nB * sizeof(double), st_));
             CgStepArgs S = cg_step_args(iter);
@@ -1646,7 +1672,7 @@
             scal_out(nx, q.scal_out);
             down_mat(q.out_vR, vR_.p); down_vec(q.out_vs, vs_.p);
             if (!model_rec) { down_mat(q.out_HvR, HvR_.p); down_vec(q.out_Hvs, Hvs_.p); }
-            down_mat(q.out_rR, rR_.p); down_vec(q.out_rs, v.rs_next); down_mat(q.out_pR, pR_.p); down_vec(q.out_ps, v.ps_next);
+            down_mat(q.out_rR, v.rR_next); down_vec(q.out_rs, v.rs_next); down_mat(q.out_pR, v.pR_next); down_vec(q.out_ps, v.ps_next);
             if (Wtcg) down_mat(q.out_W, Wloc);
             if (wpad()) down_vec(q.out_Wpad, wpad(), 16);
             if (q.partsB_out) to_host(q.partsB_out, v.partsB_out, (size_t)nB * sizeof(double));
@@ -1848,8 +1874,8 @@
             I.Wloc = Wloc; I.Wpad = nullptr;
             launch_tcg_init(o, I, st_);
         }
-        up_mat(pR_.p, q.pR, 1.0); up_vec(v.ps_cur, q.ps, 1.0, false); up_vec(v.ps_next, q.ps, 1.0, false);
-        up_mat(rR_.p, q.rR, 1.0); up_vec(v.rs_cur, q.rs, 1.0, false); up_vec(v.rs_next, q.rs, 1.0, false);
+        up_mat(v.pR_cur, q.pR, 1.0); up_vec(v.ps_cur, q.ps, 1.0, false); up_vec(v.ps_next, q.ps, 1.0, false);
+        up_mat(v.rR_cur, q.rR, 1.0); up_vec(v.rs_cur, q.rs, 1.0, false); up_vec(v.rs_next, q.rs, 1.0, false);
         up_mat(vR_.p, q.vR, 1.0); up_vec(vs_.p, q.vs, 1.0, false);
         up_mat(HvR_.p, q.HvR, 1.0); up_vec(Hvs_.p, q.Hvs, 1.0, false);
         if (q.Rc && q.sc) { up_mat(Rc_.p, q.Rc, 1.0); up_vec(sc_.p, q.sc, 1.0, false); }
@@ -1918,7 +1944,7 @@
         }
         down_mat(q.out_R, R_.p); down_vec(q.out_s, s_.p); down_mat(q.out_Rc, Rc_.p); down_vec(q.out_sc, sc_.p);
         down_mat(q.out_vR, vR_.p); down_vec(q.out_vs, vs_.p); down_mat(q.out_HvR, HvR_.p); down_vec(q.out_Hvs, Hvs_.p);
-        down_mat(q.out_rR, rR_.p); down_vec(q.out_rs, v.rs_next); down_mat(q.out_pR, pR_.p); down_vec(q.out_ps, v.ps_next);
+        down_mat(q.out_rR, v.rR_next); down_vec(q.out_rs, v.rs_next); down_mat(q.out_pR, v.pR_next); down_vec(q.out_ps, v.ps_next);
         down_mat(q.out_W, Wloc);
         if (wpad()) down_vec(q.out_Wpad, wpad(), 16);
         if (q.out_partsB) to_host(q.out_partsB, v.partsB_out, (size_t)nB * sizeof(double));
@@ -2236,6 +2262,7 @@
     if (opt.sum_grouping < 0 || opt.sum_grouping > 2) throw Error(XM_ERR_ARG, "sum_grouping must be 0, 1 or 2");
     retraction_ = opt.retraction;
     grouping_ = opt.sum_grouping;
+    tcg_two_launch_count_ = 0;
     double *Rout = res.R, *sout = res.s;
     std::memset(&res, 0, sizeof(res));
     res.R = Rout; res.s = sout;
diff --git a/xm-code_amd/csrc/xm_symv_step.h b/xm-code_amd/csrc/xm_symv_step.h
--- a/xm-code_amd/csrc/xm_symv_step.h
+++ b/xm-code_amd/csrc/xm_symv_step.h
@@ -49,9 +49,9 @@
     const int64_t wi = (int64_t)6 * j * OP + (lane < 6 * OP ? lane : 0);
     return W[wi < wlim ? wi : wlim];
 }
-template <int O>
+template <int O, int P = pitch_of(O)>
 __device__ __forceinline__ void symv_wrow_read(double wl, int r, bool ok, double (&wr)[O]) {
-    constexpr int OP = pitch_of(O);
+    constexpr int OP = P;
 #pragma unroll
     for (int k = 0; k < O; ++k) {
         const int lo = __builtin_amdgcn_readlane(__double2loint(wl), r * OP + k), hi = __builtin_amdgcn_readlane(__double2hiint(wl), r * OP + k);
diff --git a/xm-code_amd/xmamd.py b/xm-code_amd/xmamd.py
--- a/xm-code_amd/xmamd.py
+++ b/xm-code_amd/xmamd.py
@@ -20,6 +20,7 @@
 FLAG_HOST_OUTER = 64
 FLAG_DEVICE_OUTER = 128
 FLAG_MODEL_RECURRENCE = 32
+FLAG_TCG_THREE_LAUNCH = 256
 
 EXPORTS = [
     "xm_last_error", "xm_version", "xm_abi_revision", "xm_solve", "xm_solve_rank3", "xm_solve_rebuttle", "xm_ctx_create", "xm_ctx_solve",
@@ -27,7 +28,7 @@
     "xm_dev_sync", "xm_dense_upload", "xm_dense_from_bsr3", "xm_qw_dense", "xm_qw_dense_sym", "xm_qw_bsr3", "xm_retract", "xm_retract_polar", "xm_recover_rotations",
     "xm_comm_unique_id", "xm_comm_init", "xm_comm_init_shm", "xm_comm_init_ipc", "xm_comm_finalize", "xm_partition", "xm_partition_blocks",
     "xm_symv_plan", "xm_sell_layout", "xm_sell_locality", "xm_sell_create", "xm_sell_create2", "xm_sell_quat_roundtrip", "xm_sell_destroy", "xm_qw_sell", "xm_qw_sell_padded",
-    "xm_ctx_attach_edges", "xm_ctx_edge_residuals", "xm_ctx_edge_residuals_recovered", "xm_ctx_xm2_filter", "xm_ctx_xm2_round", "xm_ctx_set_edge_weights", "xm_ctx_recover_tp", "xm_ctx_schur_info", "xm_ctx_qw", "xm_spd_inverse", "xm_ctx_transport", "xm_ctx_sell_wpad", "xm_ctx_product_kind", "xm_symw_plan", "xm_symw_use",
+    "xm_ctx_attach_edges", "xm_ctx_edge_residuals", "xm_ctx_edge_residuals_recovered", "xm_ctx_xm2_filter", "xm_ctx_xm2_round", "xm_ctx_set_edge_weights", "xm_ctx_recover_tp", "xm_ctx_schur_info", "xm_ctx_tcg_two_launch", "xm_ctx_qw", "xm_spd_inverse", "xm_ctx_transport", "xm_ctx_sell_wpad", "xm_ctx_product_kind", "xm_symw_plan", "xm_symw_use",
     "xm_ctx_schur_precond_info", "xm_schur_aggregate_plan",
     "xm_dense_to_f32", "xm_qw_dense_f32", "xm_qw_dense_sym_f32",
     "xm_ctx_bundle_adjust", "xm_ctx_reprojection_errors", "xm_spd_solve", "xm_la_probe", "xm_ba_aggregate_plan", "xm_ctx_ba_probe",
@@ -516,6 +517,7 @@
         L.xm_ctx_dense_q.argtypes = [C.c_void_p, C.c_void_p, C.c_int64]
         L.xm_create_matrix.argtypes = [C.c_int64, C.c_int64, C.c_int64, C.c_void_p, C.c_void_p, C.c_void_p, C.c_void_p, C.c_void_p, C.c_int64, C.c_void_p]
         L.xm_schur_dense_limits.argtypes = [C.c_void_p]
+        L.xm_ctx_tcg_two_launch.argtypes = [C.c_void_p, C.POINTER(C.c_int)]
         L.xm_ctx_schur_info.argtypes = [C.c_void_p, C.POINTER(C.c_int), C.c_void_p, C.POINTER(C.c_double)]
         L.xm_ctx_schur_precond_info.argtypes = [C.c_void_p, C.POINTER(C.c_int), C.POINTER(C.c_int64), C.POINTER(C.c_int)]
         L.xm_schur_aggregate_plan.argtypes = [C.c_int64, C.c_int64, C.c_void_p, C.c_void_p, C.c_int, C.c_void_p]
@@ -2245,6 +2247,8 @@
         res.R = R.ctypes.data_as(C.c_void_p); res.s = s.ctypes.data_as(C.c_void_p)
         _chk(lib().xm_ctx_solve(self.h, C.byref(opt), C.byref(res)))
         info = {k: getattr(res, k) for k, _ in Result._fields_ if k not in ("R", "s", "struct_size")}
+        cnt = C.c_int(0)
+        info["tcg_two_launch"] = cnt.value if lib().xm_ctx_tcg_two_launch(self.h, C.byref(cnt)) == 0 else 0
         if tr is not None:
             info["trace"] = tr[: res.trace_len].copy()
         return np.ascontiguousarray(R[:, : res.rank]), s, info
```
